# SamsungLabs/fcaf3d

Hardware: AMD Instinct MI355X
Metric: scenes/sec fwd+bwd, ScanNet 100k-pt 2cm voxels, 1/2/4/8 MI355X (higher is better)
Workload: dtype f32

## Files before the change

fcaf3d_amd/_lib.py:

```python
import ctypes
import os
import re
import threading
import time

import torch

_HERE = os.path.dirname(os.path.abspath(__file__))
LIB_PATH = os.environ.get('FC_LIB') or os.path.join(_HERE, 'libfcaf3d_hip.so')
HEADER = os.path.join(os.path.dirname(_HERE), 'include', 'fcaf3d_hip.h')

_SCALARS = {'int': ctypes.c_int, 'int64_t': ctypes.c_int64, 'float': ctypes.c_float,
            'hipStream_t': ctypes.c_void_p}


def parse_header(path=HEADER):
    txt = open(path).read()
    txt = re.sub(r'/\*.*?\*/', '', txt, flags=re.S)
    protos = {}
    for m in re.finditer(r'\b(int64_t|int)\s+(fc_\w+)\s*\(([^)]*)\)\s*;', txt):
        ret, name, args = m.group(1), m.group(2), m.group(3)
        argl = []
        for a in args.split(','):
            a = ' '.join(a.split())
            if not a or a == 'void':
                continue
            if '*' in a:
                argl.append((a.split('*')[-1].strip(), ctypes.c_void_p))
            else:
                ty, nm = a.rsplit(' ', 1)
                argl.append((nm, _SCALARS[ty.replace('const ', '')]))
        protos[name] = (_SCALARS[ret], argl)
    return protos


EXEC_OPS = os.path.join(_HERE, 'csrc', 'exec_ops.h')


def parse_enums(path=EXEC_OPS):
    txt = re.sub(r'//[^\n]*', '', open(path).read())
    known, blocks = {}, []
    for m in re.finditer(r'\benum\s*\{([^}]*)\}', txt):
        block, nxt = {}, 0
        for item in filter(None, (s.strip() for s in m.group(1).split(','))):
            name, _, expr = (s.strip() for s in item.partition('='))
            if expr:
                nxt = sum(known[t] if t in known else int(t, 0) for t in (s.strip() for s in expr.split('+')))
            assert re.fullmatch(r'[A-Z]\w*', name) and name not in known, item
            block[name] = known[name] = nxt
            nxt += 1
        blocks.append(block)
    return blocks


ABI_VERSION = 14
_lib = None
_protos = None


def lib():
    global _lib, _protos
    if _lib is None:
        if not os.path.exists(LIB_PATH):
            raise RuntimeError(
                f'{LIB_PATH} is missing: build it with `python -m fcaf3d_amd.build` '
                '(hipcc --offload-arch=gfx950).  There is no CPU fallback.')
        l = ctypes.CDLL(LIB_PATH)
        _protos = parse_header()
        for name, (ret, args) in _protos.items():
            fn = getattr(l, name)
            fn.restype = ret
            fn.argtypes = [t for _, t in args]
        if l.fc_abi_version() != ABI_VERSION:
            raise RuntimeError(f'{LIB_PATH} speaks ABI version {l.fc_abi_version()}, this host code was written for {ABI_VERSION}: rebuild '
                               'with `python -m fcaf3d_amd.build`')
        _lib = l
    return _lib


def ptr(t):
    if t is None:
        return None
    assert t.is_contiguous(), 'C ABI takes contiguous buffers'
    return t.data_ptr()


_raw_stream = getattr(torch._C, '_cuda_getCurrentRawStream', None)


def stream():
    if _raw_stream is not None:
        return _raw_stream(torch.cuda.current_device())
    return torch.cuda.current_stream().cuda_stream


_fns = {}


def call(name, *args):
    fn = _fns.get(name)
    if fn is None:
        fn = _fns[name] = getattr(lib(), name)
    rc = fn(*args)
    if rc != 0:
        kind = 'invalid argument' if rc == -1 else 'workspace too small' if rc == -2 else f'hipError {rc}'
        raise RuntimeError(f'{name} failed: {kind}')


_header_enums = {}


def header_enums():
    if not _header_enums:
        _header_enums.update({k: v for block in parse_enums(HEADER) for k, v in block.items()})
    return _header_enums


_ROUTE_FIELDS = {'fc_conv_fwd_route': 'FC_ROUTE_', 'fc_conv_wgrad_route': 'FC_WROUTE_', 'fc_bn_train_fwd_route': 'FC_NROUTE_',
                 'fc_bn_train_bwd_route': 'FC_NROUTE_'}


def route(name, *args):
    out = (ctypes.c_int * 16)()
    rc = getattr(lib(), name)(*args, out)
    prefix = _ROUTE_FIELDS[name]
    return rc, {k[len(prefix):].lower(): out[v] for k, v in header_enums().items() if k.startswith(prefix)}


_query_cache = {}


def query(name, *args):
    key = (name,) + args
    v = _query_cache.get(key)
    if v is None:
        if len(_query_cache) > 65536:
            _query_cache.clear()
        v = _query_cache[key] = int(getattr(lib(), name)(*args))
    return v


_ws_cache = {}


def workspace(nbytes, device):
    key = (device, stream())
    buf = _ws_cache.get(key)
    if buf is None or buf.numel() < nbytes:
        buf = torch.empty(max(int(nbytes), 1 << 20), dtype=torch.uint8, device=device)
        _ws_cache[key] = buf
    return buf


HOST_WAIT = [0.0]


class _PinnedRing:

    def __init__(self, n=16):
        self.bufs, self.evts, self.i = [None] * n, [None] * n, 0
        self.lock = threading.Lock()

    def upload(self, arr, device):
        with self.lock:
            i = self.i
            self.i = (i + 1) % len(self.bufs)
        if self.evts[i] is not None and not self.evts[i].query():
            t0 = time.perf_counter()
            self.evts[i].synchronize()
            HOST_WAIT[0] += time.perf_counter() - t0
        nb = max(int(arr.nbytes), 1)
        if self.bufs[i] is None or self.bufs[i].numel() < nb:
            self.bufs[i] = torch.empty(max(nb, 4096), dtype=torch.uint8).pin_memory()
        src = torch.from_numpy(arr)
        stage = self.bufs[i][:arr.nbytes].view(src.dtype).reshape(src.shape)
        stage.copy_(src)
        out = stage.to(device, non_blocking=True)
        e = torch.cuda.Event()
        e.record(torch.cuda.current_stream(out.device))
        self.evts[i] = e
        return out


_ring = _PinnedRing()


def upload(arr, device):
    return _ring.upload(arr, device)
```

fcaf3d_amd/csrc/exec.hip:

```cpp
#include "fc_common.h"
#include "../../include/fcaf3d_hip.h"
#include "exec_ops.h"
#include <vector>

namespace {

constexpr int MAX_EVENTS = 64;

constexpr int MAX_DEVICES = 16;
hipEvent_t g_events_dev[MAX_DEVICES][MAX_EVENTS];
bool g_events_ready[MAX_DEVICES] = {};
thread_local hipEvent_t* g_events = nullptr;

int ensure_events() {
  int dev = 0;
  FC_HIP(hipGetDevice(&dev));
  if (dev < 0 || dev >= MAX_DEVICES) return FC_EINVAL;
  if (!g_events_ready[dev]) {
    for (int i = 0; i < MAX_EVENTS; ++i) FC_HIP(hipEventCreateWithFlags(&g_events_dev[dev][i], hipEventDisableTiming));
    g_events_ready[dev] = true;
  }
  g_events = g_events_dev[dev];
  return 0;
}
// ... 94 lines not shown
  int64_t bn_small_elems;
  int flags;
};

int run_op_impl(Ctx& c, const int64_t* op);

int run_op(Ctx& c, const int64_t* op) {
  if (c.dry || !c.probe || (op[ROW_OP] != OP_CONV && op[ROW_OP] != OP_AMAX)) return run_op_impl(c, op);
  ProbeRec r;
  r.a = probe_event(); r.b = probe_event();
  if (!r.a || !r.b) return run_op_impl(c, op);
  hipStream_t st = c.streams[op[ROW_STREAM]];
  if (op[ROW_OP] == OP_AMAX) {
    const int64_t meta[8] = {-2, 0, c.dims[op[AMAX_N]], 0, 0, op[AMAX_C], 0, 0};
    __builtin_memcpy(r.meta, meta, sizeof meta);
  } else if (op[CONV_MAP] < 0) {
    const int64_t n = c.dims[op[CONV_N]];
    const int64_t meta[8] = {-1, op[CONV_DIR], n, n, 1, op[CONV_CIN], op[CONV_COUT], 0};
    __builtin_memcpy(r.meta, meta, sizeof meta);
  } else {
    const int64_t* mp = c.maps + op[CONV_MAP] * MAPW;
    const bool bwd = op[CONV_DIR] != 0;
    const int64_t meta[8] = {op[CONV_MAP], op[CONV_DIR], bwd ? mp[MAP_N_OUT] : mp[MAP_N_IN], bwd ? mp[MAP_N_IN] : mp[MAP_N_OUT], mp[MAP_K],
                             op[CONV_CIN], op[CONV_COUT], (mp[MAP_FLAGS] & (bwd ? MAP_ROUTE_BWD_PAIRS : MAP_ROUTE_FWD_PAIRS)) ? 1 : 0};
    __builtin_memcpy(r.meta, meta, sizeof meta);
  }
  FC_HIP(hipEventRecord(r.a, st));
  const int rc = run_op_impl(c, op);
  FC_HIP(hipEventRecord(r.b, st));
  g_probe.push_back(r);
  return rc;
}

template <class T>
inline T* P(const Ctx& c, int64_t idx) { return idx < 0 ? nullptr : reinterpret_cast<T*>(c.addr[idx]); }
template <class T>
inline T* P1(const Ctx& c, int64_t idx1) { return P<T>(c, idx1 - 1); }

int64_t stats_blocks_of(const Ctx& c, const int64_t* conv) {
  const int Cin = (int)conv[CONV_CIN], Cout = (int)conv[CONV_COUT];
  const int fl = c.flags | FC_CONV_SPLIT | FC_CONV_IMAGE;
  if (conv[CONV_MAP] < 0) return fc_conv_stats_blocks(c.dims[conv[CONV_N]], 1, Cin, Cout, fl, 0);
  const int64_t* m = c.maps + conv[CONV_MAP] * MAPW;
  const bool bwd = conv[CONV_DIR] != 0;
  return fc_conv_stats_blocks(bwd ? m[MAP_N_IN] : m[MAP_N_OUT], (int)m[MAP_K], Cin, Cout, fl,
                              (m[MAP_FLAGS] & (bwd ? MAP_ROUTE_BWD_PAIRS : MAP_ROUTE_FWD_PAIRS)) ? 1 : 0);
}

inline bool want_ws(Ctx& c, int s, int64_t bytes) {
  if (bytes > c.need[s]) c.need[s] = bytes;
  return !c.dry;
}

int run_op_impl(Ctx& c, const int64_t* op) {
  const int s = (int)op[ROW_STREAM];
  hipStream_t st = c.streams[s];
#ifdef FC_KO_EXEC
  {
    static const int ko = getenv("FC_KO_OPS") ? atoi(getenv("FC_KO_OPS")) : 0;
    const int64_t o = op[ROW_OP];
    if (!c.dry && (((ko & 1) && (o == OP_WGRAD || o == OP_STEM_WGRAD)) || ((ko & 2) && o == OP_CONV) ||
                   ((ko & 4) && (o == OP_BN_FWD || o == OP_BN_BWD || o == OP_COL_STATS || o == OP_NORM_POOL_FWD || o == OP_POOL_NORM_BWD))))
      return 0;
  }
#endif
  switch (op[ROW_OP]) {
    case OP_STEM_FWD: {
      const int64_t* m = c.maps + op[STEM_FWD_MAP] * MAPW;
      if (c.dry) return 0;
      return fc_stem_conv_fwd(P<const float>(c, op[STEM_FWD_X]), P<const float>(c, op[STEM_FWD_W]), reinterpret_cast<const int*>(m[MAP_NBR]),
                              P<float>(c, op[STEM_FWD_OUT]), P<float>(c, op[STEM_FWD_COL]), m[MAP_N_IN], m[MAP_N_OUT], (int)m[MAP_K], st);
    }
    case OP_COL_STATS: {
      const int64_t n = c.dims[op[COL_STATS_N]];
      const int C = (int)op[COL_STATS_C], nseg = (int)c.dims[op[COL_STATS_NSEG]];
      if (!want_ws(c, s, fc_col_stats_ws_bytes(n, C, nseg))) return 0;
      return fc_col_stats(P<const float>(c, op[COL_STATS_X]), P<const int>(c, op[COL_STATS_SEG]), op[COL_STATS_SEG] >= 0 ? 4 : 0, n, C, nseg,
                          P<float>(c, op[COL_STATS_MEAN]), P<float>(c, op[COL_STATS_VAR]), P<float>(c, op[COL_STATS_CNT]), c.ws[s],
                          c.ws_bytes[s], st);
    }
    case OP_CONV: {
      const int Cin = (int)op[CONV_CIN], Cout = (int)op[CONV_COUT];
      const int fl = c.flags | FC_CONV_SPLIT | FC_CONV_IMAGE;
      float* stats = (op[CONV_STATS_P1] > 0 && stats_blocks_of(c, op) > 0) ? P1<float>(c, op[CONV_STATS_P1]) : nullptr;
      const float* bnx = stats ? P1<const float>(c, op[CONV_BN_X_P1]) : nullptr;
      const float *bmean = P<const float>(c, op[CONV_BN_MEAN]), *bvar = P<const float>(c, op[CONV_BN_VAR]),
                  *bga = P<const float>(c, op[CONV_BN_GAMMA]), *bbe = P<const float>(c, op[CONV_BN_BETA]);
      const float beps = (float)as_double(op[CONV_BN_EPS]);
      const int bact = (int)op[CONV_BN_ACT];
      const float* badd = P1<const float>(c, op[CONV_BN_ADD_P1]);
      const float* bny = P1<const float>(c, op[CONV_BN_Y_P1]);
      const float* in = P<const float>(c, op[CONV_X]);
      const float* img = P<const float>(c, op[CONV_IMG]);
      float* out = P<float>(c, op[CONV_OUT]);
      if (!c.dry && op[CONV_AMAX_X_P1] > 0) fc_conv_amax_hint(P1<const unsigned>(c, op[CONV_AMAX_X_P1]), nullptr);
      if (op[CONV_MAP] < 0) {
        const int64_t n = c.dims[op[CONV_N]];
        if (!want_ws(c, s, fc_conv_fwd_ws_bytes(n, 1, Cin, Cout, fl))) return 0;
        if (bnx)
          return fc_conv_fwd_bn_bwd_stats(in, img, nullptr, nullptr, out, n, n, 1, Cin, Cout, fl, c.ws[s], c.ws_bytes[s], stats, bnx, bmean, bvar,
                                          bga, bbe, beps, bact, badd, bny, st);
        return fc_conv_fwd_stats(in, img, nullptr, nullptr, out, n, n, 1, Cin, Cout, fl, c.ws[s], c.ws_bytes[s], stats, st);
      }
      const int64_t* m = c.maps + op[CONV_MAP] * MAPW;
      const bool bwd = op[CONV_DIR] != 0;
      const int64_t n_in = bwd ? m[MAP_N_OUT] : m[MAP_N_IN], n_out = bwd ? m[MAP_N_IN] : m[MAP_N_OUT];
      const int K = (int)m[MAP_K];
      if (m[MAP_FLAGS] & (bwd ? MAP_ROUTE_BWD_PAIRS : MAP_ROUTE_FWD_PAIRS)) {
        const int64_t* pr = m + (bwd ? MAP_PAIRS_T : MAP_PAIRS);
        const int *pi = reinterpret_cast<const int*>(pr[PAIR_IN]), *pc = reinterpret_cast<const int*>(pr[PAIR_CNT]),
                  *pp = reinterpret_cast<const int*>(pr[PAIR_POS]);
        if (!want_ws(c, s, fc_conv_fwd_pairs_ws_bytes(n_out, K, Cout))) return 0;
        if (bnx)
          return fc_conv_fwd_pairs_tiles_bn_bwd_stats(in, img, pi, pc, pp, out, n_in, n_out, K, Cin, Cout, pr[PAIR_TILES], fl, c.ws[s],
                                                      c.ws_bytes[s], stats, bnx, bmean, bvar, bga, bbe, beps, bact, badd, bny, st);
        return fc_conv_fwd_pairs_tiles_stats(in, img, pi, pc, pp, out, n_in, n_out, K, Cin, Cout, pr[PAIR_TILES], fl, c.ws[s], c.ws_bytes[s],
                                             stats, st);
      }
      const int *tab = reinterpret_cast<const int*>(bwd ? m[MAP_BWD_TAB] : m[MAP_FWD_TAB]),
                *oidx = reinterpret_cast<const int*>(bwd ? m[MAP_BWD_IDX] : m[MAP_FWD_IDX]);
      if (!want_ws(c, s, fc_conv_fwd_ws_bytes(n_out, K, Cin, Cout, fl))) return 0;
      if (bnx)
        return fc_conv_fwd_bn_bwd_stats(in, img, tab, oidx, out, n_in, n_out, K, Cin, Cout, fl, c.ws[s], c.ws_bytes[s], stats, bnx, bmean, bvar,
                                        bga, bbe, beps, bact, badd, bny, st);
      return fc_conv_fwd_stats(in, img, tab, oidx, out, n_in, n_out, K, Cin, Cout, fl, c.ws[s], c.ws_bytes[s], stats, st);
    }
    case OP_BN_FWD: {
      const int64_t n = c.dims[op[BN_FWD_N]];
      const int C = (int)op[BN_FWD_C];
      const float eps = (float)as_double(op[BN_FWD_EPS]), mom = (float)as_double(op[BN_FWD_MOMENTUM]);
      const int* add_inv = P1<const int>(c, op[BN_FWD_ADD_INV_P1]);
      const float* add_src = op[BN_FWD_ADD_INV_P1] > 0 ? P1<const float>(c, op[BN_FWD_ADD_SRC_P1]) : nullptr;
      if (!op[BN_FWD_TRAIN]) {
        if (c.dry) return 0;
        if (op[BN_FWD_AMAX_Y_P1] > 0) fc_amax_out_hint(P1<unsigned>(c, op[BN_FWD_AMAX_Y_P1]));
        return fc_norm_act_add_fwd(P<const float>(c, op[BN_FWD_X]), nullptr, 0, n, C, P<const float>(c, op[BN_FWD_RMEAN]),
                                   P<const float>(c, op[BN_FWD_RVAR]), eps, P<const float>(c, op[BN_FWD_GAMMA]),
                                   P<const float>(c, op[BN_FWD_BETA]), P<const float>(c, op[BN_FWD_RES]), (int)op[BN_FWD_ACT], add_inv, add_src,
                                   P<float>(c, op[BN_FWD_Y]), st);
      }
      const float* part = nullptr;
      int64_t nbp = 0;
      if (op[BN_FWD_PRODUCER_P1] > 0) {
        const int64_t* conv = c.ops + (op[BN_FWD_PRODUCER_P1] - 1) * OPW;
        nbp = conv[CONV_STATS_P1] > 0 ? stats_blocks_of(c, conv) : 0;
        if (nbp > 0) part = P1<const float>(c, conv[CONV_STATS_P1]);
      }
      if (!want_ws(c, s, fc_bn_train_ws_bytes(n, C))) return 0;
      if (op[BN_FWD_AMAX_Y_P1] > 0) fc_amax_out_hint(P1<unsigned>(c, op[BN_FWD_AMAX_Y_P1]));
      return fc_bn_train_add_fwd(P<const float>(c, op[BN_FWD_X]), n, C, eps, P<const float>(c, op[BN_FWD_GAMMA]),
                                 P<const float>(c, op[BN_FWD_BETA]), P<const float>(c, op[BN_FWD_RES]), (int)op[BN_FWD_ACT], mom,
                                 P<float>(c, op[BN_FWD_Y]), P<float>(c, op[BN_FWD_MEAN]), P<float>(c, op[BN_FWD_VAR]),
                                 P<float>(c, op[BN_FWD_CNT]), P<float>(c, op[BN_FWD_RMEAN]), P<float>(c, op[BN_FWD_RVAR]),
                                 P<long long>(c, op[BN_FWD_NBT]), part, nbp, op[BN_FWD_GROUPS] > 0 ? (int)op[BN_FWD_GROUPS] : 1,
                                 c.bn_small_elems, add_inv, add_src, c.ws[s], c.ws_bytes[s], st);
    }
    case OP_HEAD_FWD: {
      if (c.dry) return 0;
      return fc_head_split_fwd(P<const float>(c, op[HEAD_FWD_Y]), (int)op[HEAD_FWD_LD], P<const float>(c, op[HEAD_FWD_BIAS]),
                               P<const float>(c, op[HEAD_FWD_SCALE]), c.dims[op[HEAD_FWD_N]], (int)op[HEAD_FWD_N_REG], (int)op[HEAD_FWD_N_CLS],
                               P<float>(c, op[HEAD_FWD_CENT]), P<float>(c, op[HEAD_FWD_BBOX]), P<float>(c, op[HEAD_FWD_CLS]),
                               P<float>(c, op[HEAD_FWD_CMAX]), st);
    }
    case OP_RECORD:
      if (c.dry) return 0;
      FC_HIP(hipEventRecord(g_events[op[RECORD_EVENT]], st));
      return 0;
    case OP_WAIT:
      if (c.dry) return 0;
      FC_HIP(hipStreamWaitEvent(st, g_events[op[WAIT_EVENT]], 0));
      return 0;
    case OP_HEAD_BWD: {
      const float *y = P<const float>(c, op[HEAD_BWD_Y]), *scale = P<const float>(c, op[HEAD_BWD_SCALE]),
                  *bbox = P<const float>(c, op[HEAD_BWD_BBOX]), *g_cent = P<const float>(c, op[HEAD_BWD_G_CENT]),
                  *g_bbox = P<const float>(c, op[HEAD_BWD_G_BBOX]), *g_cls = P<const float>(c, op[HEAD_BWD_G_CLS]);
      const int64_t n = c.dims[op[HEAD_BWD_N]];
      const int ld = (int)op[HEAD_BWD_LD], n_reg = (int)op[HEAD_BWD_N_REG], n_cls = (int)op[HEAD_BWD_N_CLS];
      if (op[HEAD_BWD_GS_ROW] < 0) {
        if (!want_ws(c, s, fc_head_split_bwd_sums_ws_bytes(n))) return 0;
        if (op[HEAD_BWD_AMAX_GY_P1] > 0) fc_amax_out_hint(P1<unsigned>(c, op[HEAD_BWD_AMAX_GY_P1]));
        return fc_head_split_bwd_sums(y, ld, scale, bbox, g_cent, g_bbox, g_cls, n, n_reg, n_cls, P<float>(c, op[HEAD_BWD_GY]),
                                      P<float>(c, op[HEAD_BWD_BIAS_PART]), P<float>(c, op[HEAD_BWD_G_SCALE]), c.ws[s], c.ws_bytes[s], st);
      }
      if (c.dry) return 0;
      return fc_head_split_bwd(y, ld, scale, bbox, g_cent, g_bbox, g_cls, n, n_reg, n_cls, P<float>(c, op[HEAD_BWD_GY]),
                               P<float>(c, op[HEAD_BWD_GS_ROW]), st);
    }
    case OP_WGRAD: {
      const int Cin = (int)op[WGRAD_CIN], Cout = (int)op[WGRAD_COUT];
      const int fl = c.flags | FC_CONV_SPLIT;
      const float *in = P<const float>(c, op[WGRAD_X]), *gout = P<const float>(c, op[WGRAD_GOUT]);
      float* gw = P<float>(c, op[WGRAD_GW]);
      if (!c.dry && (op[WGRAD_AMAX_X_P1] > 0 || op[WGRAD_AMAX_GOUT_P1] > 0))
        fc_conv_amax_hint(P1<const unsigned>(c, op[WGRAD_AMAX_X_P1]), P1<const unsigned>(c, op[WGRAD_AMAX_GOUT_P1]));
      if (op[WGRAD_MAP] < 0) {
        const int64_t n = c.dims[op[WGRAD_N]];
        if (!want_ws(c, s, fc_conv_wgrad_ws_bytes(n, 1, Cin, Cout, fl))) return 0;
        return fc_conv_wgrad(in, gout, nullptr, nullptr, gw, n, n, 1, Cin, Cout, fl, c.ws[s], c.ws_bytes[s], st);
      }
      const int64_t* m = c.maps + op[WGRAD_MAP] * MAPW;
      const int K = (int)m[MAP_K];
      if (!want_ws(c, s, fc_conv_wgrad_ws_bytes(m[MAP_N_OUT], K, Cin, Cout, fl))) return 0;
      if ((m[MAP_FLAGS] & MAP_ROUTE_WGRAD_PAIRS) && Cin % 64 == 0 && Cout % 64 == 0) {
        const int64_t* pr = m + MAP_PAIRS;
        return fc_conv_wgrad_pairs(in, gout, reinterpret_cast<const int*>(pr[PAIR_IN]), reinterpret_cast<const int*>(pr[PAIR_OUT]),
                                   reinterpret_cast<const int*>(pr[PAIR_CNT]), gw, m[MAP_N_IN], m[MAP_N_OUT], K, Cin, Cout, fl, c.ws[s],
                                   c.ws_bytes[s], st);
      }
      return fc_conv_wgrad(in, gout, reinterpret_cast<const int*>(m[MAP_NBR]), nullptr, gw, m[MAP_N_IN], m[MAP_N_OUT], K, Cin, Cout, fl,
                           c.ws[s], c.ws_bytes[s], st);
    }
    case OP_BN_BWD: {
      const int64_t n = c.dims[op[BN_BWD_N]];
      const int C = (int)op[BN_BWD_C];
      const float eps = (float)as_double(op[BN_BWD_EPS]);
      const float* part = nullptr;
      int64_t nbp = 0;
      if (op[BN_BWD_PRODUCER_P1] > 0) {
        const int64_t* conv = c.ops + (op[BN_BWD_PRODUCER_P1] - 1) * OPW;
        nbp = (conv[CONV_STATS_P1] > 0 && conv[CONV_BN_X_P1] > 0) ? stats_blocks_of(c, conv) : 0;
        if (nbp > 0) part = P1<const float>(c, conv[CONV_STATS_P1]);
      }
      if (!want_ws(c, s, fc_bn_train_ws_bytes(n, C))) return 0;
      if (op[BN_BWD_AMAX_GX_P1] > 0) fc_amax_out_hint(P1<unsigned>(c, op[BN_BWD_AMAX_GX_P1]));
      return fc_bn_train_bwd(P<const float>(c, op[BN_BWD_X]), P<const float>(c, op[BN_BWD_Y]), P<const float>(c, op[BN_BWD_GY]),
                             P1<const float>(c, op[BN_BWD_GY2_P1]), n, C, P<const float>(c, op[BN_BWD_MEAN]),
                             P<const float>(c, op[BN_BWD_VAR]), P<const float>(c, op[BN_BWD_CNT]), eps, P<const float>(c, op[BN_BWD_GAMMA]),
                             P<const float>(c, op[BN_BWD_BETA]), (int)op[BN_BWD_ACT], P<float>(c, op[BN_BWD_GX]),
                             P<float>(c, op[BN_BWD_GRES]), P<float>(c, op[BN_BWD_SUMS]), part, nbp, c.bn_small_elems, c.ws[s],
                             c.ws_bytes[s], st);
    }
    case OP_STEM_WGRAD: {
      const int64_t* m = c.maps + op[STEM_WGRAD_MAP] * MAPW;
      if (!want_ws(c, s, fc_stem_conv_wgrad_ws_bytes(m[MAP_N_OUT], (int)m[MAP_K]))) return 0;
      return fc_stem_conv_wgrad(P<const float>(c, op[STEM_WGRAD_COL]), P<const float>(c, op[STEM_WGRAD_GOUT]), P<float>(c, op[STEM_WGRAD_GW]),
                                m[MAP_N_OUT], (int)m[MAP_K], c.ws[s], c.ws_bytes[s], st);
    }
    case OP_GATHER: {
      if (c.dry) return 0;
      return fc_gather_rows(P<const float>(c, op[GATHER_SRC]), P<const int>(c, op[GATHER_IDX]), c.dims[op[GATHER_N]], (int)op[GATHER_C],
                            P<float>(c, op[GATHER_DST]), st);
    }
    case OP_ADD: {
      if (c.dry) return 0;
      const int64_t n4 = c.dims[op[ADD_N]] * op[ADD_C] / 4;
      if (n4 > 0) k_add_inplace<<<(unsigned)fc_cdiv(n4, 256), 256, 0, st>>>(P<float>(c, op[ADD_DST]), P<const float>(c, op[ADD_SRC]), n4);
      FC_CHECK_LAUNCH();
      return 0;
    }
    case OP_SMALL_GRADS: {
      if (c.dry) return 0;
      const int64_t cnt = op[SMALL_GRADS_COUNT];
      if (cnt > 0) k_small_grads<<<(unsigned)cnt, 128, 0, st>>>(P<const long long>(c, op[SMALL_GRADS_DESC]) + 8 * op[SMALL_GRADS_FIRST], (int)cnt);
      FC_CHECK_LAUNCH();
      return 0;
    }
    case OP_COL_SUM: {
      if (c.dry) return 0;
      k_col_sum<<<(unsigned)op[COL_SUM_C], 1024, 0, st>>>(P<const float>(c, op[COL_SUM_X]), c.dims[op[COL_SUM_N]], (int)op[COL_SUM_C],
                                                         P<float>(c, op[COL_SUM_DST]));
      FC_CHECK_LAUNCH();
      return 0;
    }
    case OP_ROW_SUM: {
      if (c.dry) return 0;
      k_col_sum<<<1, 1024, 0, st>>>(P<const float>(c, op[ROW_SUM_X]), c.dims[op[ROW_SUM_N]], 1, P<float>(c, op[ROW_SUM_DST]));
      FC_CHECK_LAUNCH();
      return 0;
    }
    case OP_PERMUTE_GENT: {
      if (c.dry) return 0;
      const int Cin = (int)op[PERMUTE_GENT_CIN], Cout = (int)op[PERMUTE_GENT_COUT];
      const int64_t total = (int64_t)8 * Cin * Cout;
      k_permute_gent<<<(unsigned)fc_cdiv(total, 256), 256, 0, st>>>(P<const float>(c, op[PERMUTE_GENT_SRC]), P<float>(c, op[PERMUTE_GENT_DST]),
                                                                    Cin, Cout);
      FC_CHECK_LAUNCH();
      return 0;
    }
    case OP_HEAD_WFIN: {
      if (c.dry) return 0;
      const int R = (int)op[HEAD_WFIN_R], n_reg = (int)op[HEAD_WFIN_N_REG], n_cls = (int)op[HEAD_WFIN_N_CLS];
      const int total = R * (1 + n_reg + n_cls);
      k_head_wfin<<<(unsigned)fc_cdiv(total, 256), 256, 0, st>>>(P<const float>(c, op[HEAD_WFIN_PART]), (int)op[HEAD_WFIN_NL], R,
                                                                 (int)op[HEAD_WFIN_LD], n_reg, n_cls, P<float>(c, op[HEAD_WFIN_G_CENT]),
                                                                 P<float>(c, op[HEAD_WFIN_G_REG]), P<float>(c, op[HEAD_WFIN_G_CLS]),
                                                                 P<const float>(c, op[HEAD_WFIN_BIAS_PART]), P<float>(c, op[HEAD_WFIN_G_BIAS]));
      FC_CHECK_LAUNCH();
      return 0;
    }
    case OP_AMAX: {
      if (c.dry) return 0;
      return fc_amax(P<const float>(c, op[AMAX_X]), c.dims[op[AMAX_N]] * op[AMAX_C], P<unsigned>(c, op[AMAX_SLOT]), st);
    }
    case OP_CLEAR: {
      if (c.dry) return 0;
      FC_HIP(hipMemsetAsync(P<void>(c, op[CLEAR_DST]), 0, (size_t)op[CLEAR_BYTES], st));
      return 0;
    }
    case OP_NORM_POOL_FWD: {
      const int64_t* m = c.maps + op[NORM_POOL_FWD_MAP] * MAPW;
      if (c.dry) return 0;
      if ((int)m[MAP_K] != 8) return FC_EINVAL;
      if (op[NORM_POOL_FWD_AMAX_OUT_P1] > 0) fc_amax_out_hint(P1<unsigned>(c, op[NORM_POOL_FWD_AMAX_OUT_P1]));
      return fc_norm_act_maxpool8_fwd(P<const float>(c, op[NORM_POOL_FWD_X]), P<const int>(c, op[NORM_POOL_FWD_SEG]),
                                      op[NORM_POOL_FWD_SEG] >= 0 ? 4 : 0, (int)op[NORM_POOL_FWD_C], P<const float>(c, op[NORM_POOL_FWD_MEAN]),
                                      P<const float>(c, op[NORM_POOL_FWD_VAR]), (float)as_double(op[NORM_POOL_FWD_EPS]),
                                      P<const float>(c, op[NORM_POOL_FWD_GAMMA]), P<const float>(c, op[NORM_POOL_FWD_BETA]),
                                      (int)op[NORM_POOL_FWD_ACT], reinterpret_cast<const int*>(m[MAP_NBR]), m[MAP_N_OUT],
                                      P<float>(c, op[NORM_POOL_FWD_OUT]), P<int>(c, op[NORM_POOL_FWD_ARG]), P<float>(c, op[NORM_POOL_FWD_Y]),
                                      P<int>(c, op[NORM_POOL_FWD_PARENT]), st);
    }
    case OP_POOL_NORM_BWD: {
      const int64_t n = c.dims[op[POOL_NORM_BWD_N]];
      const int C = (int)op[POOL_NORM_BWD_C], nseg = (int)c.dims[op[POOL_NORM_BWD_NSEG]];
      if (!want_ws(c, s, fc_maxpool8_norm_act_bwd_ws_bytes(n, C, nseg))) return 0;
      return fc_maxpool8_norm_act_bwd(P<const float>(c, op[POOL_NORM_BWD_X]), P<const float>(c, op[POOL_NORM_BWD_G_POOL]),
                                      P<const int>(c, op[POOL_NORM_BWD_ARG]), P<const int>(c, op[POOL_NORM_BWD_PARENT]),
                                      P<const int>(c, op[POOL_NORM_BWD_SEG]), op[POOL_NORM_BWD_SEG] >= 0 ? 4 : 0, n, C, nseg,
                                      P<const float>(c, op[POOL_NORM_BWD_MEAN]), P<const float>(c, op[POOL_NORM_BWD_VAR]),
                                      P<const float>(c, op[POOL_NORM_BWD_CNT]), (float)as_double(op[POOL_NORM_BWD_EPS]),
                                      P<const float>(c, op[POOL_NORM_BWD_GAMMA]), P<const float>(c, op[POOL_NORM_BWD_BETA]),
                                      (int)op[POOL_NORM_BWD_ACT], P<float>(c, op[POOL_NORM_BWD_GX]), P<float>(c, op[POOL_NORM_BWD_SUMS]),
                                      c.ws[s], c.ws_bytes[s], st);
    }
    case OP_INV_ROWS: {
      if (c.dry) return 0;
      return fc_inverse_rows(P<const int>(c, op[INV_ROWS_ROWS]), c.dims[op[INV_ROWS_N]], c.dims[op[INV_ROWS_N_INV]], P<int>(c, op[INV_ROWS_INV]), st);
    }
    case OP_COPY: {
      if (c.dry) return 0;
      FC_HIP(hipMemcpyAsync(P<float>(c, op[COPY_DST]), P<const float>(c, op[COPY_SRC]), sizeof(float) * c.dims[op[COPY_N]] * op[COPY_C],
                            hipMemcpyDeviceToDevice, st));
      return 0;
    }
    default:
      return FC_EINVAL;
  }
}

}

extern "C" {

int fc_exec_op_words(void) { return OPW; }
int fc_exec_map_words(void) { return MAPW; }

int fc_exec(const int64_t* ops, int64_t op_begin, int64_t op_end, const int64_t* addr, const int64_t* dims, const int64_t* maps,
            const int64_t* streams, const int64_t* ws, const int64_t* ws_bytes, int64_t* ws_need, const int64_t* cfg) {
  if (!ops || op_begin < 0 || op_end < op_begin) return FC_EINVAL;
  int rc = ensure_events();
  if (rc) return rc;
  Ctx c;
  c.ops = ops;
  c.addr = addr; c.dims = dims; c.maps = maps;
  for (int i = 0; i < NSTREAM; ++i) {
    c.streams[i] = reinterpret_cast<hipStream_t>(streams[i]);
    c.ws[i] = reinterpret_cast<void*>(ws[i]);
    c.ws_bytes[i] = ws_bytes[i];
    c.need[i] = 0;
  }
  c.bn_small_elems = cfg[0];
  c.flags = (int)cfg[1];
  c.probe = cfg[2] != 0;
  c.dry = true;
  for (int64_t i = op_begin; i < op_end; ++i) {
    rc = run_op(c, ops + i * OPW);
    if (rc) return rc;
  }
  bool ok = true;
  for (int i = 0; i < NSTREAM; ++i) {
    if (ws_need) ws_need[i] = c.need[i];
    if (c.need[i] > c.ws_bytes[i]) ok = false;
  }
  if (!ok) return FC_EWS;
  if (cfg[3]) return 0;
  c.dry = false;
  for (int64_t i = op_begin; i < op_end; ++i) {
    rc = run_op(c, ops + i * OPW);
    if (rc) return rc;
  }
  return 0;
}

int64_t fc_exec_probe_read(float* ms, int64_t* meta, int64_t cap) {
  const int64_t n = (int64_t)g_probe.size();
  for (int64_t i = 0; i < n; ++i) {
    ProbeRec& r = g_probe[i];
    if (i < cap) {
      float t = 0.f;
      if (hipEventElapsedTime(&t, r.a, r.b) != hipSuccess) t = -1.f;
      ms[i] = t;
      __builtin_memcpy(meta + 8 * i, r.meta, sizeof r.meta);
    }
    g_probe_pool.push_back(r.a);
    g_probe_pool.push_back(r.b);
  }
  g_probe.clear();
  return n;
}

}
```

fcaf3d_amd/csrc/exec_ops.h:

```cpp
#ifndef FCAF3D_EXEC_OPS_H
#define FCAF3D_EXEC_OPS_H

enum {
  OPW = 24,
  MAPW = 20,
  NSTREAM = 3
};
enum { ROW_OP, ROW_STREAM };

enum {
  OP_STEM_FWD = 1, OP_COL_STATS, OP_NORM_FWD, OP_MAXPOOL_FWD, OP_CONV, OP_BN_FWD, OP_UNION_FWD, OP_HEAD_FWD, OP_RECORD, OP_WAIT,
  OP_HEAD_BWD, OP_WGRAD, OP_BN_BWD, OP_NORM_BWD, OP_MAXPOOL_BWD, OP_STEM_WGRAD, OP_GATHER, OP_ADD, OP_SMALL_GRADS,
  OP_PERMUTE_GENT, OP_HEAD_WFIN, OP_COPY, OP_COL_SUM, OP_ROW_SUM, OP_AMAX, OP_CLEAR, OP_NORM_POOL_FWD, OP_POOL_NORM_BWD, OP_INV_ROWS
};

enum {
  STEM_FWD_X = 2,
  STEM_FWD_W,
  STEM_FWD_MAP,
  STEM_FWD_OUT,
  STEM_FWD_COL,
  STEM_FWD_END
};
enum {
  COL_STATS_X = 2,
  COL_STATS_SEG,
  COL_STATS_N,
  COL_STATS_C,
  COL_STATS_NSEG,
  COL_STATS_MEAN,
  COL_STATS_VAR,
  COL_STATS_CNT,
  COL_STATS_END
};
enum {
  CONV_X = 2,
  CONV_IMG,
  CONV_MAP,
  CONV_DIR,
  CONV_OUT,
  CONV_N,
  CONV_CIN,
  CONV_COUT,
  CONV_STATS_P1,
  CONV_BN_X_P1,
  CONV_BN_MEAN,
  CONV_BN_VAR,
  CONV_BN_GAMMA,
  CONV_BN_BETA,
  CONV_BN_EPS,
  CONV_BN_ACT,
  CONV_BN_ADD_P1,
  CONV_BN_Y_P1,
  CONV_AMAX_X_P1,
  CONV_END
};
enum {
  BN_FWD_X = 2,
  BN_FWD_N,
  BN_FWD_C,
  BN_FWD_EPS,
  BN_FWD_GAMMA,
  BN_FWD_BETA,
  BN_FWD_RES,
  BN_FWD_ACT,
  BN_FWD_MOMENTUM,
  BN_FWD_Y,
  BN_FWD_MEAN,
  BN_FWD_VAR,
  BN_FWD_CNT,
  BN_FWD_RMEAN,
  BN_FWD_RVAR,
  BN_FWD_NBT,
  BN_FWD_TRAIN,
  BN_FWD_PRODUCER_P1,
  BN_FWD_GROUPS,
  BN_FWD_AMAX_Y_P1,
  BN_FWD_ADD_INV_P1,
  BN_FWD_ADD_SRC_P1,
  BN_FWD_END
};
enum {
  HEAD_FWD_Y = 2,
  HEAD_FWD_LD,
  HEAD_FWD_BIAS,
  HEAD_FWD_SCALE,
  HEAD_FWD_N,
  HEAD_FWD_N_REG,
  HEAD_FWD_N_CLS,
  HEAD_FWD_CENT,
  HEAD_FWD_BBOX,
  HEAD_FWD_CLS,
  HEAD_FWD_CMAX,
  HEAD_FWD_END
};
enum { RECORD_EVENT = 2, RECORD_END };
enum { WAIT_EVENT = 2, WAIT_END };
enum {
  HEAD_BWD_Y = 2,
  HEAD_BWD_LD,
  HEAD_BWD_SCALE,
  HEAD_BWD_BBOX,
  HEAD_BWD_G_CENT,
  HEAD_BWD_G_BBOX,
  HEAD_BWD_G_CLS,
  HEAD_BWD_N,
  HEAD_BWD_N_REG,
  HEAD_BWD_N_CLS,
  HEAD_BWD_GY,
  HEAD_BWD_GS_ROW,
  HEAD_BWD_G_SCALE,
  HEAD_BWD_BIAS_PART,
  HEAD_BWD_AMAX_GY_P1,
  HEAD_BWD_END
};
enum {
  WGRAD_X = 2,
  WGRAD_GOUT,
  WGRAD_MAP,
  WGRAD_GW,
  WGRAD_N,
  WGRAD_CIN,
  WGRAD_COUT,
  WGRAD_AMAX_X_P1,
  WGRAD_AMAX_GOUT_P1,
  WGRAD_END
};
enum {
  BN_BWD_X = 2,
  BN_BWD_Y,
  BN_BWD_GY,
  BN_BWD_N,
  BN_BWD_C,
  BN_BWD_MEAN,
  BN_BWD_VAR,
  BN_BWD_CNT,
  BN_BWD_EPS,
  BN_BWD_GAMMA,
  BN_BWD_BETA,
  BN_BWD_ACT,
  BN_BWD_GX,
  BN_BWD_GRES,
  BN_BWD_SUMS,
  BN_BWD_GY2_P1,
  BN_BWD_PRODUCER_P1,
  BN_BWD_AMAX_GX_P1,
  BN_BWD_END
};
enum {
  STEM_WGRAD_COL = 2,
  STEM_WGRAD_GOUT,
  STEM_WGRAD_MAP,
  STEM_WGRAD_GW,
  STEM_WGRAD_END
};
enum {
  GATHER_SRC = 2,
  GATHER_IDX,
  GATHER_N,
  GATHER_C,
  GATHER_DST,
  GATHER_END
};
enum {
  ADD_DST = 2,
  ADD_SRC,
  ADD_N,
  ADD_C,
  ADD_END
};
enum {
  SMALL_GRADS_DESC = 2,
  SMALL_GRADS_FIRST,
  SMALL_GRADS_COUNT,
  SMALL_GRADS_END
};
enum {
  PERMUTE_GENT_SRC = 2,
  PERMUTE_GENT_DST,
  PERMUTE_GENT_CIN,
  PERMUTE_GENT_COUT,
  PERMUTE_GENT_END
};
enum {
  HEAD_WFIN_PART = 2,
  HEAD_WFIN_NL,
  HEAD_WFIN_R,
  HEAD_WFIN_LD,
  HEAD_WFIN_N_REG,
  HEAD_WFIN_N_CLS,
  HEAD_WFIN_G_CENT,
  HEAD_WFIN_G_REG,
  HEAD_WFIN_G_CLS,
  HEAD_WFIN_BIAS_PART,
  HEAD_WFIN_G_BIAS,
  HEAD_WFIN_END
};
enum {
  COPY_DST = 2,
  COPY_SRC,
  COPY_N,
  COPY_C,
  COPY_END
};
enum {
  COL_SUM_X = 2,
  COL_SUM_N,
  COL_SUM_C,
  COL_SUM_DST,
  COL_SUM_END
};
enum {
  ROW_SUM_X = 2,
  ROW_SUM_N,
  ROW_SUM_DST,
  ROW_SUM_END
};
enum {
  AMAX_X = 2,
  AMAX_N,
  AMAX_C,
  AMAX_SLOT,
  AMAX_END
};
enum {
  CLEAR_DST = 2,
  CLEAR_BYTES,
  CLEAR_END
};
enum {
  NORM_POOL_FWD_X = 2,
  NORM_POOL_FWD_SEG,
  NORM_POOL_FWD_C,
  NORM_POOL_FWD_MEAN,
  NORM_POOL_FWD_VAR,
  NORM_POOL_FWD_EPS,
  NORM_POOL_FWD_GAMMA,
  NORM_POOL_FWD_BETA,
  NORM_POOL_FWD_ACT,
  NORM_POOL_FWD_MAP,
  NORM_POOL_FWD_OUT,
  NORM_POOL_FWD_ARG,
  NORM_POOL_FWD_Y,
  NORM_POOL_FWD_AMAX_OUT_P1,
  NORM_POOL_FWD_PARENT,
  NORM_POOL_FWD_END
};
enum {
  POOL_NORM_BWD_X = 2,
  POOL_NORM_BWD_G_POOL,
  POOL_NORM_BWD_ARG,
  POOL_NORM_BWD_PARENT,
  POOL_NORM_BWD_SEG,
  POOL_NORM_BWD_N,
  POOL_NORM_BWD_C,
  POOL_NORM_BWD_NSEG,
  POOL_NORM_BWD_MEAN,
  POOL_NORM_BWD_VAR,
  POOL_NORM_BWD_CNT,
  POOL_NORM_BWD_EPS,
  POOL_NORM_BWD_GAMMA,
  POOL_NORM_BWD_BETA,
  POOL_NORM_BWD_ACT,
  POOL_NORM_BWD_GX,
  POOL_NORM_BWD_SUMS,
  POOL_NORM_BWD_END
};
enum {
  INV_ROWS_ROWS = 2,
  INV_ROWS_N,
  INV_ROWS_N_INV,
  INV_ROWS_INV,
  INV_ROWS_END
};

static_assert(STEM_FWD_END <= OPW && COL_STATS_END <= OPW && CONV_END <= OPW && BN_FWD_END <= OPW && HEAD_FWD_END <= OPW, "operator row");
static_assert(RECORD_END <= OPW && WAIT_END <= OPW && HEAD_BWD_END <= OPW && WGRAD_END <= OPW && BN_BWD_END <= OPW, "operator row");
static_assert(STEM_WGRAD_END <= OPW && GATHER_END <= OPW && ADD_END <= OPW && SMALL_GRADS_END <= OPW && PERMUTE_GENT_END <= OPW, "operator row");
static_assert(HEAD_WFIN_END <= OPW && COPY_END <= OPW && COL_SUM_END <= OPW && ROW_SUM_END <= OPW && AMAX_END <= OPW, "operator row");
static_assert(CLEAR_END <= OPW && NORM_POOL_FWD_END <= OPW && POOL_NORM_BWD_END <= OPW && INV_ROWS_END <= OPW, "operator row");

enum {
  PAIR_IN,
  PAIR_OUT,
  PAIR_POS,
  PAIR_CNT,
  PAIR_TILES,
  PAIR_END
};
enum {
  MAP_N_IN,
  MAP_N_OUT,
  MAP_K,
  MAP_NBR,
  MAP_NBR_T,
  MAP_FWD_TAB,
  MAP_FWD_IDX,
  MAP_BWD_TAB,
  MAP_BWD_IDX,
  MAP_PAIRS,
  MAP_PAIRS_T = MAP_PAIRS + PAIR_END,
  MAP_FLAGS = MAP_PAIRS_T + PAIR_END,
  MAP_END
};
enum {
  MAP_ROUTE_FWD_PAIRS = 1,
  MAP_ROUTE_BWD_PAIRS = 2,
  MAP_ROUTE_WGRAD_PAIRS = 4
};
static_assert(MAP_END <= MAPW, "kernel-map descriptor");

#endif
```

fcaf3d_amd/csrc/norm.hip:

```cpp
#include "fc_common.h"
#include "../../include/fcaf3d_hip.h"
#include "norm_route.h"
#include "norm_elem.h"
#include "norm_stats.h"
#include "norm_rows.h"
#include "norm_bn.h"
#include "pool_rows.h"

thread_local unsigned* t_fc_amax_out = nullptr;

#define FC_GRID(l, stream) dim3((l).grid_x, (l).grid_y), (l).threads, (l).lds, stream

static int bn_fwd(const float* x, int64_t n, int C, float eps, const float* gamma, const float* beta, const float* residual, int act, float momentum,
                  float* y, float* mean, float* var, float* cnt, float* rmean, float* rvar, long long* nbt, const float* table, int64_t nb_part, int groups,
                  int64_t small_elems, const int* add_inv, const float* add_src, void* ws, int64_t ws_bytes, hipStream_t stream, unsigned* amax,
                  bool apply = true) {
  if (act < 0 || act > 2 || (add_inv == nullptr) != (add_src == nullptr)) return FC_EINVAL;
  const NormRoute r = norm_fwd_route(n, C, table != nullptr, nb_part, groups, small_elems);
  if (int rc = route_check(r, ws_bytes)) return rc;
  float* part = (float*)ws;
  if (r.red.threads) { k_bn1_partial<<<FC_GRID(r.red, stream)>>>(x, n, C, r.red_rpb, part); FC_CHECK_LAUNCH(); }
  if (r.fin.threads) {
    if (r.sums == FC_NSTATS_PARTIAL) k_bn_finalize<<<FC_GRID(r.fin, stream)>>>(part, (int)r.np, C, n, x, momentum, mean, var, cnt, rmean, rvar, nbt);
    else k_bn2_finalize<<<FC_GRID(r.fin, stream)>>>(table, (int)r.np, C, groups, n, momentum, mean, var, cnt, rmean, rvar, nbt);
    FC_CHECK_LAUNCH();
  }
  if (!apply) return FC_OK;
  if (r.apply == FC_NAPPLY_BN1)
    k_bn1_apply<<<FC_GRID(r.ap, stream)>>>(x, n, C, r.rpb, part, (int)r.np, eps, gamma, beta, residual, act, momentum, y, mean, var, cnt, rmean, rvar, nbt, add_inv, add_src);
  else if (r.apply == FC_NAPPLY_BN2)
    k_bn2_apply<<<FC_GRID(r.ap, stream)>>>(x, n, C, r.rpb, table, (int)r.np, groups, eps, gamma, beta, residual, act, momentum, y, mean, var, cnt, rmean, rvar, nbt, r.cg,
                                   add_inv, add_src, amax);
  else
    k_norm_act_fwd<<<FC_GRID(r.ap, stream)>>>(x, nullptr, 0, n, C, mean, var, eps, gamma, beta, residual, act, add_inv, add_src, y, amax);
  FC_CHECK_LAUNCH();
  if (r.amax == FC_NAMAX_PASS && amax) return fc_amax(y, n * (int64_t)C, amax, stream);
  return FC_OK;
}

template <bool POOL>
static int norm_bwd(int form, const float* x, const float* y, const float* gy, const float* gy2, const int* parent, const int* argrow, const int* seg,
                    int seg_stride, int64_t n, int C, int nseg, const float* mean, const float* var, const float* cnt, float eps, const float* gamma,
                    const float* beta, int act, float* gx, float* gres, float* sums, const float* table, int64_t nb_part, int64_t small_elems, void* ws,
                    int64_t ws_bytes, hipStream_t stream, unsigned* amax, bool late_hint = false) {
  if (act < 0 || act > 2) return FC_EINVAL;
  const NormRoute r = norm_bwd_route(n, C, nseg, table != nullptr, nb_part, small_elems, form);
  if (int rc = route_check(r, ws_bytes)) return rc;
  if (late_hint) amax = take_amax_out();
  if (r.apply == FC_NBAPPLY_NONE) {
    FC_HIP(hipMemsetAsync(sums, 0, sizeof(float) * nseg * 2 * C, stream));
    return FC_OK;
  }
  if (r.sums == FC_NRED_PARTIAL) {
    k_norm_bwd_partial<POOL><<<FC_GRID(r.red, stream)>>>(x, y, gy, gy2, parent, argrow, seg, seg_stride, n, C, nseg, mean, var, eps, act, gamma, beta, r.red_rpb, (float*)ws);
    FC_CHECK_LAUNCH();
    table = (const float*)ws;
  }
  if (r.apply == FC_NBAPPLY_PROLOGUE) {
    k_bn1_bwd_apply<<<FC_GRID(r.ap, stream)>>>(x, y, gy, gy2, n, C, r.rpb, table, (int)r.np, mean, var, eps, gamma, beta, act, gx, gres, sums, r.cg, amax);
  } else {
    k_stats_final<<<FC_GRID(r.fin, stream)>>>(table, nullptr, r.np, nseg, 2 * C, 2, sums, nullptr);
    FC_CHECK_LAUNCH();
    k_norm_bwd_apply<POOL><<<FC_GRID(r.ap, stream)>>>(x, y, gy, gy2, parent, argrow, seg, seg_stride, n, C, mean, var, eps, gamma, beta, sums, cnt, act, gx, gres, amax);
  }
  FC_CHECK_LAUNCH();
  return FC_OK;
}

constexpr int ROUTE_OUT_INTS = 16;
static_assert(FC_NROUTE_LAUNCHES < ROUTE_OUT_INTS, "every FC_NROUTE_* field lies inside out[]");
static int route_out(const NormRoute& r, int* out) {
  const int f[ROUTE_OUT_INTS] = {r.sums, r.apply, r.amax, (int)r.np, (int)r.nb, (int)r.rpb, r.cg, r.ap.threads, (int)r.ap.lds, (int)r.ap.grid_x, (int)r.ap.grid_y,
                                 (int)r.ws_bytes, (r.red.threads != 0) + (r.fin.threads != 0) + (r.ap.threads != 0)};
  for (int i = 0; i < ROUTE_OUT_INTS; ++i) out[i] = f[i];
  return r.sums ? FC_OK : FC_EINVAL;
}

static int col_stats(bool stats, const float* x, const int* seg, int seg_stride, int64_t n, int C, int nseg, float* out, float* var, float* cnt, void* ws,
                     int64_t ws_bytes, hipStream_t stream) {
  if (n < 0 || nseg < 1 || nseg > MAXSEG) return FC_EINVAL;
  StatsGeometry g;
  if (!stats_geometry(C, &g)) return FC_EINVAL;
  if (ws_bytes < fc_col_stats_ws_bytes(n, C, nseg)) return FC_EWS;
  if (n == 0) {
    FC_HIP(hipMemsetAsync(out, 0, sizeof(float) * nseg * C, stream));
    if (stats) FC_HIP(hipMemsetAsync(var, 0, sizeof(float) * nseg * C, stream));
    if (stats) FC_HIP(hipMemsetAsync(cnt, 0, sizeof(float) * nseg, stream));
    return FC_OK;
  }
  const RowBlocks b = row_blocks(n, MAXBLOCKS);
  float* part = (float*)ws;
  float* part_cnt = stats ? part + b.nb * nseg * 2 * C : nullptr;
  k_stats_partial<<<(unsigned)b.nb, g.threads, g.lds_fwd, stream>>>(x, seg, seg_stride, n, C, nseg, nullptr, stats ? 2 : 0, b.rpb, part, part_cnt);
  FC_CHECK_LAUNCH();
  if (stats) k_seg_meanvar_final<<<FC_GRID(final_launch(nseg, C), stream)>>>(part, part_cnt, b.nb, nseg, C, out, var, cnt);
  else k_stats_final<<<FC_GRID(final_launch(nseg, C), stream)>>>(part, nullptr, b.nb, nseg, C, 2, out, nullptr);
  FC_CHECK_LAUNCH();
  return FC_OK;
}

extern "C" {

int64_t fc_col_stats_ws_bytes(int64_t n, int C, int nseg) {
  return row_blocks(n, MAXBLOCKS).nb * nseg * (2 * (int64_t)C + 1) * (int64_t)sizeof(float);
}

int fc_col_stats(const float* x, const int* seg, int seg_stride, int64_t n, int C, int nseg, float* mean, float* var,
                 float* cnt, void* ws, int64_t ws_bytes, hipStream_t stream) {
  return col_stats(true, x, seg, seg_stride, n, C, nseg, mean, var, cnt, ws, ws_bytes, stream);
}

int fc_seg_col_sums(const float* x, const int* seg, int seg_stride, int64_t n, int C, int nseg, float* out, void* ws,
                    int64_t ws_bytes, hipStream_t stream) {
  return col_stats(false, x, seg, seg_stride, n, C, nseg, out, nullptr, nullptr, ws, ws_bytes, stream);
}

int fc_bn_running_update(const float* mean, const float* var, const float* cnt, float momentum, int C, float* running_mean,
                         float* running_var, long long* num_batches_tracked, hipStream_t stream) {
  if (C < 1) return FC_EINVAL;
  k_bn_running<<<(unsigned)fc_cdiv(C, 256), 256, 0, stream>>>(mean, var, cnt, momentum, C, running_mean, running_var,
                                                             num_batches_tracked);
  FC_CHECK_LAUNCH();
  return FC_OK;
}

int fc_bn_train_fwd_route(int64_t n, int C, int has_part, int64_t nb_part, int groups, int64_t small_elems, int* out) {
  return out ? route_out(norm_fwd_route(n, C, has_part != 0, nb_part, groups, small_elems), out) : FC_EINVAL;
}
int fc_bn_train_bwd_route(int64_t n, int C, int nseg, int has_part, int64_t nb_part, int64_t small_elems, int form, int* out) {
  if (!out || form < FC_NFORM_TRAIN || form > FC_NFORM_SEG) return FC_EINVAL;
  return route_out(norm_bwd_route(n, C, nseg, has_part != 0, nb_part, small_elems, form), out);
}

int64_t fc_bn_small_ws_bytes(int C) { return small_ws_bytes(C); }
int64_t fc_bn_stats_ws_bytes(int64_t n, int C) { return reduce_ws_bytes(n, C, 1); }
int64_t fc_norm_act_bwd_ws_bytes(int64_t n, int C, int nseg) { return reduce_ws_bytes(n, C, nseg); }
int64_t fc_maxpool8_norm_act_bwd_ws_bytes(int64_t n_in, int C, int nseg) { return reduce_ws_bytes(n_in, C, nseg); }
int64_t fc_bn_train_ws_bytes(int64_t n, int C) { return reduce_ws_bytes(n, C, 1) > small_ws_bytes(C) ? reduce_ws_bytes(n, C, 1) : small_ws_bytes(C); }

int fc_bn_stats_train(const float* x, int64_t n, int C, float momentum, float* mean, float* var, float* cnt,
                      float* running_mean, float* running_var, long long* num_batches_tracked, void* ws,
                      int64_t ws_bytes, hipStream_t stream) {
  return bn_fwd(x, n, C, 0.f, nullptr, nullptr, nullptr, 0, momentum, nullptr, mean, var, cnt, running_mean, running_var, num_batches_tracked, nullptr, 0, 1,
                -1, nullptr, nullptr, ws, ws_bytes, stream, nullptr, false);
}

int fc_bn_act_train_fwd(const float* x, int64_t n, int C, float eps, const float* gamma, const float* beta,
                        const float* residual, int act, float momentum, float* y, float* mean, float* var, float* cnt,
                        float* running_mean, float* running_var, long long* num_batches_tracked, void* ws,
                        int64_t ws_bytes, hipStream_t stream) {
  return bn_fwd(x, n, C, eps, gamma, beta, residual, act, momentum, y, mean, var, cnt, running_mean, running_var, num_batches_tracked, nullptr, 0, 1,
                INT64_MAX, nullptr, nullptr, ws, ws_bytes, stream, nullptr);
}

int fc_bn_act_train_bwd(const float* x, const float* y, const float* gy, int64_t n, int C, const float* mean,
                        const float* var, float eps, const float* gamma, const float* beta, int act, float* gx, float* gres,
                        float* sums, void* ws, int64_t ws_bytes, hipStream_t stream) {
  return norm_bwd<false>(FC_NFORM_SMALL, x, y, gy, nullptr, nullptr, nullptr, nullptr, 0, n, C, 1, mean, var, nullptr, eps, gamma, beta, act, gx, gres, sums,
                         nullptr, 0, 0, ws, ws_bytes, stream, nullptr, true);
}

int fc_norm_act_add_fwd(const float* x, const int* seg, int seg_stride, int64_t n, int C, const float* mean, const float* var,
                        float eps, const float* gamma, const float* beta, const float* residual, int act, const int* add_inv,
                        const float* add_src, float* y, hipStream_t stream) {
  unsigned* ao = take_amax_out();
  if (n < 0 || C < 4 || C % 4 || act < 0 || act > 2 || (add_inv == nullptr) != (add_src == nullptr)) return FC_EINVAL;
  if (n == 0) return FC_OK;
  k_norm_act_fwd<<<FC_GRID(rows_launch(n, C), stream)>>>(x, seg, seg_stride, n, C, mean, var, eps, gamma, beta, residual, act, add_inv, add_src, y, ao);
  FC_CHECK_LAUNCH();
  return FC_OK;
}

int fc_norm_act_fwd(const float* x, const int* seg, int seg_stride, int64_t n, int C, const float* mean, const float* var,
                    float eps, const float* gamma, const float* beta, const float* residual, int act, float* y,
                    hipStream_t stream) {
  return fc_norm_act_add_fwd(x, seg, seg_stride, n, C, mean, var, eps, gamma, beta, residual, act, nullptr, nullptr, y, stream);
}

int fc_norm_act_bwd(const float* x, const float* y, const float* gy, const int* seg, int seg_stride, int64_t n, int C,
                    int nseg, const float* mean, const float* var, const float* cnt, float eps, const float* gamma,
                    const float* beta, int act, float* gx, float* gres, float* sums, void* ws, int64_t ws_bytes,
                    hipStream_t stream) {
  unsigned* ao = take_amax_out();
  return norm_bwd<false>(FC_NFORM_SEG, x, y, gy, nullptr, nullptr, nullptr, seg, seg_stride, n, C, nseg, mean, var, cnt, eps, gamma, beta, act, gx, gres, sums,
                         nullptr, 0, 0, ws, ws_bytes, stream, ao);
}

int fc_bn_train_add_fwd(const float* x, int64_t n, int C, float eps, const float* gamma, const float* beta, const float* residual,
                        int act, float momentum, float* y, float* mean, float* var, float* cnt, float* running_mean,
                        float* running_var, long long* num_batches_tracked, const float* part, int64_t nb_part, int groups,
                        int64_t small_elems, const int* add_inv, const float* add_src, void* ws, int64_t ws_bytes,
                        hipStream_t stream) {
  unsigned* ao = take_amax_out();
  return bn_fwd(x, n, C, eps, gamma, beta, residual, act, momentum, y, mean, var, cnt, running_mean, running_var, num_batches_tracked, part, nb_part, groups,
                small_elems, add_inv, add_src, ws, ws_bytes, stream, ao);
}

int fc_bn_train_fwd(const float* x, int64_t n, int C, float eps, const float* gamma, const float* beta, const float* residual,
                    int act, float momentum, float* y, float* mean, float* var, float* cnt, float* running_mean,
                    float* running_var, long long* num_batches_tracked, const float* part, int64_t nb_part, int groups,
                    int64_t small_elems, void* ws, int64_t ws_bytes, hipStream_t stream) {
  return fc_bn_train_add_fwd(x, n, C, eps, gamma, beta, residual, act, momentum, y, mean, var, cnt, running_mean, running_var, num_batches_tracked, part, nb_part,
                             groups, small_elems, nullptr, nullptr, ws, ws_bytes, stream);
}

int fc_bn_train_bwd(const float* x, const float* y, const float* gy, const float* gy2, int64_t n, int C, const float* mean,
                    const float* var, const float* cnt, float eps, const float* gamma, const float* beta, int act, float* gx,
                    float* gres, float* sums, const float* part, int64_t nb_part, int64_t small_elems, void* ws, int64_t ws_bytes,
                    hipStream_t stream) {
  unsigned* ao = take_amax_out();
  return norm_bwd<false>(FC_NFORM_TRAIN, x, y, gy, gy2, nullptr, nullptr, nullptr, 0, n, C, 1, mean, var, cnt, eps, gamma, beta, act, gx, gres, sums, part, nb_part,
                         small_elems, ws, ws_bytes, stream, ao);
}

int fc_amax_out_hint(unsigned* amax_word) {
  t_fc_amax_out = amax_word;
  return FC_OK;
}

int fc_maxpool_fwd(const float* in, const int* nbr, int64_t n_out, int K, int C, float* out, int* argrow,
                   hipStream_t stream) {
  unsigned* ao = take_amax_out();
  if (n_out < 0 || K < 1 || C < 1) return FC_EINVAL;
  if (n_out == 0) return FC_OK;
  if (K == 8 && C % 4 == 0) k_maxpool8_fwd<<<FC_GRID(rows_launch(n_out, C), stream)>>>(in, nbr, n_out, C, out, argrow, ao);
  else k_maxpool_fwd<<<(unsigned)fc_cdiv(n_out * C, 256), 256, 0, stream>>>(in, nbr, n_out, K, C, out, argrow);
  FC_CHECK_LAUNCH();
  if (ao && !(K == 8 && C % 4 == 0)) return fc_amax(out, n_out * (int64_t)C, ao, stream);
  return FC_OK;
}

int fc_maxpool_bwd(const float* gout, const int* argrow, int64_t n_out, int C, float* gin, hipStream_t stream) {
  if (n_out < 0 || C < 1) return FC_EINVAL;
  if (n_out == 0) return FC_OK;
  k_maxpool_bwd<<<(unsigned)fc_cdiv(n_out * C, 256), 256, 0, stream>>>(gout, argrow, n_out, C, gin);
  FC_CHECK_LAUNCH();
  return FC_OK;
}

int fc_gather_rows(const float* src, const int* idx, int64_t n, int C, float* dst, hipStream_t stream) {
  if (n < 0 || C < 1) return FC_EINVAL;
  if (n == 0) return FC_OK;
  k_gather_rows<<<(unsigned)fc_cdiv(n * C, 256), 256, 0, stream>>>(src, idx, n, C, dst);
  FC_CHECK_LAUNCH();
  return FC_OK;
}

int fc_scatter_rows_add(const float* src, const int* idx, int64_t n, int C, float* dst, hipStream_t stream) {
  if (n < 0 || C < 1) return FC_EINVAL;
  if (n == 0) return FC_OK;
  k_scatter_rows_add<<<(unsigned)fc_cdiv(n * C, 256), 256, 0, stream>>>(src, idx, n, C, dst);
  FC_CHECK_LAUNCH();
  return FC_OK;
}

int fc_norm_act_maxpool8_fwd(const float* x, const int* seg, int seg_stride, int C, const float* mean, const float* var, float eps,
                             const float* gamma, const float* beta, int act, const int* nbr, int64_t n_out, float* out,
                             int* argrow, float* y, int* parent, hipStream_t stream) {
  unsigned* ao = take_amax_out();
  if (n_out < 0 || C < 4 || C % 4 || act < 0 || act > 2) return FC_EINVAL;
  if (n_out == 0) return FC_OK;
  k_norm_act_maxpool8_fwd<<<FC_GRID(rows_launch(n_out, C), stream)>>>(x, seg, seg_stride, C, mean, var, eps, gamma, beta, act, nbr, n_out, out, argrow, y,
                                                                     parent, ao);
  FC_CHECK_LAUNCH();
  return FC_OK;
}

int fc_maxpool8_norm_act_bwd(const float* x, const float* gout, const int* argrow, const int* parent, const int* seg, int seg_stride,
                             int64_t n_in, int C, int nseg, const float* mean, const float* var, const float* cnt, float eps,
                             const float* gamma, const float* beta, int act, float* gx, float* sums, void* ws, int64_t ws_bytes,
                             hipStream_t stream) {
  if (!parent || !argrow) return FC_EINVAL;
  return norm_bwd<true>(FC_NFORM_SEG, x, nullptr, gout, nullptr, parent, argrow, seg, seg_stride, n_in, C, nseg, mean, var, cnt, eps, gamma, beta, act, gx, nullptr,
                        sums, nullptr, 0, 0, ws, ws_bytes, stream, nullptr);
}

int fc_inverse_rows(const int* rows, int64_t n, int64_t n_inv, int* inv, hipStream_t stream) {
  if (n < 0 || n_inv < 0) return FC_EINVAL;
  if (n_inv > 0) FC_HIP(hipMemsetAsync(inv, 0xff, sizeof(int) * n_inv, stream));
  if (n == 0) return FC_OK;
  k_inverse_rows<<<(unsigned)fc_cdiv(n, 256), 256, 0, stream>>>(rows, n, n_inv, inv);
  FC_CHECK_LAUNCH();
  return FC_OK;
}

}
```

fcaf3d_amd/csrc/norm_bn.h:

```cpp
#pragma once


__global__ void k_bn1_partial(const float* __restrict__ x, int64_t n, int C, int64_t rpb, float* __restrict__ part) {
  extern __shared__ float sm[];
  const auto [cl, rl, nrl] = lane_coord(C / 4);
  const auto [r0, r1] = row_span(rpb, n);
  const float4 sh = *reinterpret_cast<const float4*>(x + cl * 4);
  float4 a1 = make_float4(0.f, 0.f, 0.f, 0.f), a2 = a1;
  for (int64_t rb = r0 + rl; rb < r1; rb += 4 * (int64_t)nrl) {
    float4 v[4];
#pragma unroll
    for (int u = 0; u < 4; ++u) {
      const int64_t r = rb + (int64_t)u * nrl;
      v[u] = r < r1 ? *reinterpret_cast<const float4*>(x + r * C + cl * 4) : sh;
    }
#pragma unroll
    for (int u = 0; u < 4; ++u) {
      v[u].x -= sh.x; v[u].y -= sh.y; v[u].z -= sh.z; v[u].w -= sh.w;
      a1.x += v[u].x; a1.y += v[u].y; a1.z += v[u].z; a1.w += v[u].w;
      a2.x += v[u].x * v[u].x; a2.y += v[u].y * v[u].y; a2.z += v[u].z * v[u].z; a2.w += v[u].w * v[u].w;
    }
  }
  *reinterpret_cast<float4*>(&sm[(rl * 2 + 0) * C + cl * 4]) = a1;
  *reinterpret_cast<float4*>(&sm[(rl * 2 + 1) * C + cl * 4]) = a2;
  __syncthreads();
  if (rl == 0) {
    float4 t1 = make_float4(0.f, 0.f, 0.f, 0.f), t2 = t1;
    for (int j = 0; j < nrl; ++j) {
      float4 u = *reinterpret_cast<const float4*>(&sm[(j * 2 + 0) * C + cl * 4]);
      float4 w = *reinterpret_cast<const float4*>(&sm[(j * 2 + 1) * C + cl * 4]);
      t1.x += u.x; t1.y += u.y; t1.z += u.z; t1.w += u.w;
      t2.x += w.x; t2.y += w.y; t2.z += w.z; t2.w += w.w;
    }
    float* dst = part + ((int64_t)blockIdx.x * 2) * C;
    *reinterpret_cast<float4*>(dst + cl * 4) = t1;
    *reinterpret_cast<float4*>(dst + C + cl * 4) = t2;
  }
}

__device__ static inline void bn1_reduce_parts(const float* __restrict__ part, int nb, int C, int cl, int rl, int nrl,
                                               float* sm , float4* s1, float4* s2, int CG, int c0) {
  float4 a1 = make_float4(0.f, 0.f, 0.f, 0.f), a2 = a1;
  const bool past_l1 = (int64_t)nb * C * 8 <= 32768;
  for (int b = rl; b < nb; b += nrl) {
    const float* src = part + ((int64_t)b * 2) * C + c0;
    float4 u = past_l1 ? fc_ld4(src + cl * 4) : *reinterpret_cast<const float4*>(src + cl * 4);
    float4 w = past_l1 ? fc_ld4(src + C + cl * 4) : *reinterpret_cast<const float4*>(src + C + cl * 4);
    a1.x += u.x; a1.y += u.y; a1.z += u.z; a1.w += u.w;
    a2.x += w.x; a2.y += w.y; a2.z += w.z; a2.w += w.w;
  }
  *reinterpret_cast<float4*>(&sm[(rl * 2 + 0) * CG + cl * 4]) = a1;
  *reinterpret_cast<float4*>(&sm[(rl * 2 + 1) * CG + cl * 4]) = a2;
  __syncthreads();
  float4 t1 = make_float4(0.f, 0.f, 0.f, 0.f), t2 = t1;
  for (int j = 0; j < nrl; ++j) {
    float4 u = *reinterpret_cast<const float4*>(&sm[(j * 2 + 0) * CG + cl * 4]);
    float4 w = *reinterpret_cast<const float4*>(&sm[(j * 2 + 1) * CG + cl * 4]);
    t1.x += u.x; t1.y += u.y; t1.z += u.z; t1.w += u.w;
    t2.x += w.x; t2.y += w.y; t2.z += w.z; t2.w += w.w;
  }
  *s1 = t1; *s2 = t2;
}

__global__ void k_bn1_apply(const float* __restrict__ x, int64_t n, int C, int64_t rpb, const float* __restrict__ part, int nb,
                            float eps, const float* __restrict__ gamma, const float* __restrict__ beta,
                            const float* __restrict__ residual, int act, float momentum, float* __restrict__ y,
                            float* __restrict__ mean_out, float* __restrict__ var_out, float* __restrict__ cnt_out,
                            float* __restrict__ rmean, float* __restrict__ rvar, long long* __restrict__ nbt,
                            const int* __restrict__ add_inv, const float* __restrict__ add_src) {
  extern __shared__ float sm[];
  const int c4n = C / 4;
  const int cl = threadIdx.x % c4n, rl = threadIdx.x / c4n;
  const int nrl = blockDim.x / c4n;
  float4 s1, s2;
  bn1_reduce_parts(part, nb, C, cl, rl, nrl, sm, &s1, &s2, C, 0);
  const float4 sh = *reinterpret_cast<const float4*>(x + cl * 4);
  const float inv_n = 1.f / (float)n;
  float d[4] = {s1.x * inv_n, s1.y * inv_n, s1.z * inv_n, s1.w * inv_n};
  float q[4] = {s2.x * inv_n, s2.y * inv_n, s2.z * inv_n, s2.w * inv_n};
  float shv[4] = {sh.x, sh.y, sh.z, sh.w};
  float mu[4], va[4], is[4], g[4], bt[4];
#pragma unroll
  for (int j = 0; j < 4; ++j) {
    mu[j] = shv[j] + d[j];
    va[j] = fmaxf(q[j] - d[j] * d[j], 0.f);
    is[j] = 1.f / sqrtf(va[j] + eps);
    g[j] = gamma ? gamma[cl * 4 + j] : 1.f;
    bt[j] = beta ? beta[cl * 4 + j] : 0.f;
  }
  if (blockIdx.x == 0 && rl == 0) {
    *reinterpret_cast<float4*>(mean_out + cl * 4) = make_float4(mu[0], mu[1], mu[2], mu[3]);
    *reinterpret_cast<float4*>(var_out + cl * 4) = make_float4(va[0], va[1], va[2], va[3]);
    if (cl == 0) { cnt_out[0] = (float)n; if (nbt) nbt[0] += 1; }
    if (rmean) {
#pragma unroll
      for (int j = 0; j < 4; ++j) bn_running_update(rmean, rvar, cl * 4 + j, mu[j], va[j], (float)n, momentum);
    }
  }
  const auto [r0, r1] = row_span(rpb, n);
  for (int64_t rb = r0 + rl; rb < r1; rb += 4 * (int64_t)nrl) {
    float v[4][4], rs[4][4];
#pragma unroll
    for (int u = 0; u < 4; ++u) {
      const int64_t r = rb + (int64_t)u * nrl;
      const int64_t rc = r < r1 ? r : r0;
      *reinterpret_cast<float4*>(v[u]) = *reinterpret_cast<const float4*>(x + rc * C + cl * 4);
      if (residual) *reinterpret_cast<float4*>(rs[u]) = *reinterpret_cast<const float4*>(residual + rc * C + cl * 4);
    }
#pragma unroll
    for (int u = 0; u < 4; ++u) {
      const int64_t r = rb + (int64_t)u * nrl;
      if (r >= r1) continue;
      float o[4];
#pragma unroll
      for (int j = 0; j < 4; ++j) o[j] = norm_act_elem(v[u][j], mu[j], is[j], g[j], bt[j], residual ? &rs[u][j] : nullptr, act);
      const int q = add_inv ? add_inv[r] : -1;
      if (q >= 0) {
        const float4 f = *reinterpret_cast<const float4*>(add_src + (int64_t)q * C + cl * 4);
        o[0] += f.x; o[1] += f.y; o[2] += f.z; o[3] += f.w;
      }
      *reinterpret_cast<float4*>(y + r * C + cl * 4) = *reinterpret_cast<float4*>(o);
    }
  }
}

__global__ __launch_bounds__(1024) void k_bn_finalize(const float* __restrict__ part, int nb, int C, int64_t n,
                                                      const float* __restrict__ x, float momentum, float* __restrict__ mean,
                                                      float* __restrict__ var, float* __restrict__ cnt,
                                                      float* __restrict__ rmean, float* __restrict__ rvar,
                                                      long long* __restrict__ nbt) {
  __shared__ float r1[16][65], r2[16][65];
  const int c = blockIdx.x * 64 + (threadIdx.x & 63), j = threadIdx.x >> 6;
  float a1 = 0.f, a2 = 0.f;
  if (c < C) {
    float p1[4] = {0.f, 0.f, 0.f, 0.f}, p2[4] = {0.f, 0.f, 0.f, 0.f};
    int b = j;
    for (; b + 48 < nb; b += 64) {
      float u[4], w[4];
#pragma unroll
      for (int q = 0; q < 4; ++q) {
        u[q] = fc_ld(&part[((int64_t)(b + 16 * q) * 2) * C + c]);
        w[q] = fc_ld(&part[((int64_t)(b + 16 * q) * 2 + 1) * C + c]);
      }
#pragma unroll
      for (int q = 0; q < 4; ++q) { p1[q] += u[q]; p2[q] += w[q]; }
    }
    for (; b < nb; b += 16) {
      p1[0] += fc_ld(&part[((int64_t)b * 2) * C + c]);
      p2[0] += fc_ld(&part[((int64_t)b * 2 + 1) * C + c]);
    }
    a1 = (p1[0] + p1[1]) + (p1[2] + p1[3]);
    a2 = (p2[0] + p2[1]) + (p2[2] + p2[3]);
  }
  r1[j][threadIdx.x & 63] = a1;
  r2[j][threadIdx.x & 63] = a2;
  __syncthreads();
  if (j == 0 && c < C) {
    float s1 = 0.f, s2 = 0.f;
    for (int q = 0; q < 16; ++q) { s1 += r1[q][threadIdx.x & 63]; s2 += r2[q][threadIdx.x & 63]; }
    const float inv_n = 1.f / (float)n;
    float d = s1 * inv_n;
    float mu = x[c] + d;
    float va = fmaxf(s2 * inv_n - d * d, 0.f);
    mean[c] = mu;
    var[c] = va;
    if (c == 0) { cnt[0] = (float)n; if (nbt) nbt[0] += 1; }
    if (rmean) bn_running_update(rmean, rvar, c, mu, va, (float)n, momentum);
  }
}

__global__ void k_bn1_bwd_apply(const float* __restrict__ x, const float* __restrict__ y, const float* __restrict__ gy,
                                const float* __restrict__ gy2, int64_t n, int C, int64_t rpb, const float* __restrict__ part, int nb,
                                const float* __restrict__ mean, const float* __restrict__ var, float eps,
                                const float* __restrict__ gamma, const float* __restrict__ beta, int act,
                                float* __restrict__ gx, float* __restrict__ gres, float* __restrict__ sums , int CG,
                                unsigned* __restrict__ amax_out) {
  extern __shared__ float sm[];
  const int c0 = blockIdx.y * CG;
  x += c0; gy += c0; gx += c0; mean += c0; var += c0;
  if (y) y += c0;
  if (gy2) gy2 += c0;
  if (gres) gres += c0;
  if (gamma) gamma += c0;
  if (beta) beta += c0;
  const int c4n = CG / 4;
  const int cl = threadIdx.x % c4n, rl = threadIdx.x / c4n;
  const int nrl = blockDim.x / c4n;
  float4 t1, t2;
  bn1_reduce_parts(part, nb, C, cl, rl, nrl, sm, &t1, &t2, CG, c0);
  if (blockIdx.x == 0 && rl == 0) {
    *reinterpret_cast<float4*>(sums + c0 + cl * 4) = t1;
    *reinterpret_cast<float4*>(sums + C + c0 + cl * 4) = t2;
  }
  const float inv_n = 1.f / (float)n;
  float s1[4] = {t1.x * inv_n, t1.y * inv_n, t1.z * inv_n, t1.w * inv_n};
  float s2[4] = {t2.x * inv_n, t2.y * inv_n, t2.z * inv_n, t2.w * inv_n};
  float mu[4], is[4], g[4], bt[4];
#pragma unroll
  for (int j = 0; j < 4; ++j) {
    mu[j] = mean[cl * 4 + j];
    is[j] = 1.f / sqrtf(var[cl * 4 + j] + eps);
    g[j] = gamma ? gamma[cl * 4 + j] : 1.f;
    bt[j] = beta ? beta[cl * 4 + j] : 0.f;
  }
  const bool from_y = act && y;
  const auto [r0, r1] = row_span(rpb, n);
  unsigned am = 0u;
  for (int64_t rb = r0 + rl; rb < r1; rb += 4 * (int64_t)nrl) {
    float xv[4][4], gv[4][4], yv[4][4];
#pragma unroll
    for (int u = 0; u < 4; ++u) {
      const int64_t r = rb + (int64_t)u * nrl;
      const int64_t rc = r < r1 ? r : r0;
      *reinterpret_cast<float4*>(xv[u]) = *reinterpret_cast<const float4*>(x + rc * C + cl * 4);
      *reinterpret_cast<float4*>(gv[u]) = *reinterpret_cast<const float4*>(gy + rc * C + cl * 4);
      if (gy2) {
        const float4 t2 = *reinterpret_cast<const float4*>(gy2 + rc * C + cl * 4);
        gv[u][0] += t2.x; gv[u][1] += t2.y; gv[u][2] += t2.z; gv[u][3] += t2.w;
      }
      if (from_y) *reinterpret_cast<float4*>(yv[u]) = *reinterpret_cast<const float4*>(y + rc * C + cl * 4);
    }
#pragma unroll
    for (int u = 0; u < 4; ++u) {
      const int64_t r = rb + (int64_t)u * nrl;
      if (r >= r1) continue;
      float o[4], gr[4];
#pragma unroll
      for (int j = 0; j < 4; ++j) {
        float gg = gv[u][j];
        if (from_y) gg *= act_bwd_from_y(yv[u][j], act);
        else if (act) gg *= act_bwd_from_pre(bn_pre(xv[u][j], mu[j], is[j], g[j], bt[j]), act);
        float xh = (xv[u][j] - mu[j]) * is[j];
        gr[j] = gg;
        o[j] = g[j] * is[j] * (gg - s1[j] - xh * s2[j]);
      }
      *reinterpret_cast<float4*>(gx + r * C + cl * 4) = *reinterpret_cast<float4*>(o);
      if (gres) *reinterpret_cast<float4*>(gres + r * C + cl * 4) = *reinterpret_cast<float4*>(gr);
#pragma unroll
      for (int j = 0; j < 4; ++j) amax_fold(am, o[j]);
    }
  }
  if (amax_out) amax_commit(am, amax_out);
}

__global__ void k_bn2_apply(const float* __restrict__ x, int64_t n, int C, int64_t rpb, const float* __restrict__ part, int nb, int G,
                            float eps, const float* __restrict__ gamma, const float* __restrict__ beta,
                            const float* __restrict__ residual, int act, float momentum, float* __restrict__ y,
                            float* __restrict__ mean_out, float* __restrict__ var_out, float* __restrict__ cnt_out,
                            float* __restrict__ rmean, float* __restrict__ rvar, long long* __restrict__ nbt, int CG,
                            const int* __restrict__ add_inv, const float* __restrict__ add_src, unsigned* __restrict__ amax_out) {
  extern __shared__ double smd[];
  const int c0 = blockIdx.y * CG;
  x += c0; y += c0; part += c0; mean_out += c0; var_out += c0;
  if (add_src) add_src += c0;
  if (residual) residual += c0;
  if (gamma) gamma += c0;
  if (beta) beta += c0;
  if (rmean) { rmean += c0; rvar += c0; }
  const auto [cl, rl, nrl] = lane_coord(CG / 4);
  double a1[4] = {0., 0., 0., 0.}, a2[4] = {0., 0., 0., 0.};
  const int GC = G * C;
  for (int t = rl; t < nb * G; t += nrl) {
    const int b = t / G, g = t % G;
    const float* src = part + ((int64_t)b * 2) * GC + g * C + cl * 4;
    const float4 u = fc_ld4(src), w = fc_ld4(src + GC);
    a1[0] += u.x; a1[1] += u.y; a1[2] += u.z; a1[3] += u.w;
    a2[0] += w.x; a2[1] += w.y; a2[2] += w.z; a2[3] += w.w;
  }
#pragma unroll
  for (int j = 0; j < 4; ++j) {
    smd[(rl * 2 + 0) * CG + cl * 4 + j] = a1[j];
    smd[(rl * 2 + 1) * CG + cl * 4 + j] = a2[j];
  }
  __syncthreads();
  float mu[4], va[4], is[4], g[4], bt[4];
#pragma unroll
  for (int j = 0; j < 4; ++j) {
    double t1 = 0., t2 = 0.;
    for (int q = 0; q < nrl; ++q) { t1 += smd[(q * 2 + 0) * CG + cl * 4 + j]; t2 += smd[(q * 2 + 1) * CG + cl * 4 + j]; }
    bn2_stats(t1, t2, n, &mu[j], &va[j]);
    is[j] = 1.f / sqrtf(va[j] + eps);
    g[j] = gamma ? gamma[cl * 4 + j] : 1.f;
    bt[j] = beta ? beta[cl * 4 + j] : 0.f;
  }
  if (blockIdx.x == 0 && rl == 0) {
    *reinterpret_cast<float4*>(mean_out + cl * 4) = make_float4(mu[0], mu[1], mu[2], mu[3]);
    *reinterpret_cast<float4*>(var_out + cl * 4) = make_float4(va[0], va[1], va[2], va[3]);
    if (cl == 0 && blockIdx.y == 0) { cnt_out[0] = (float)n; if (nbt) nbt[0] += 1; }
    if (rmean) {
#pragma unroll
      for (int j = 0; j < 4; ++j) bn_running_update(rmean, rvar, cl * 4 + j, mu[j], va[j], (float)n, momentum);
    }
  }
  const auto [r0, r1] = row_span(rpb, n);
  unsigned am = 0u;
  for (int64_t rb = r0 + rl; rb < r1; rb += 4 * (int64_t)nrl) {
    float v[4][4], rs[4][4];
    int q[4];
#pragma unroll
    for (int u = 0; u < 4; ++u) {
      const int64_t r = rb + (int64_t)u * nrl;
      const int64_t rc = r < r1 ? r : r0;
      *reinterpret_cast<float4*>(v[u]) = *reinterpret_cast<const float4*>(x + rc * C + cl * 4);
      if (residual) *reinterpret_cast<float4*>(rs[u]) = *reinterpret_cast<const float4*>(residual + rc * C + cl * 4);
      q[u] = add_inv ? add_inv[rc] : -1;
    }
#pragma unroll
    for (int u = 0; u < 4; ++u) {
      const int64_t r = rb + (int64_t)u * nrl;
      if (r >= r1) continue;
      float o[4];
#pragma unroll
      for (int j = 0; j < 4; ++j) o[j] = norm_act_elem(v[u][j], mu[j], is[j], g[j], bt[j], residual ? &rs[u][j] : nullptr, act);
      if (q[u] >= 0) {
        const float4 f = *reinterpret_cast<const float4*>(add_src + (int64_t)q[u] * C + cl * 4);
        o[0] += f.x; o[1] += f.y; o[2] += f.z; o[3] += f.w;
      }
// ... 67 lines not shown
```

fcaf3d_amd/csrc/norm_rows.h:

```cpp
#pragma once

__global__ void k_norm_act_fwd(const float* __restrict__ x, const int* __restrict__ seg, int seg_stride, int64_t n, int C,
                               const float* __restrict__ mean, const float* __restrict__ var, float eps,
                               const float* __restrict__ gamma, const float* __restrict__ beta,
                               const float* __restrict__ residual, int act, const int* __restrict__ add_inv,
                               const float* __restrict__ add_src, float* __restrict__ y, unsigned* __restrict__ amax_out) {
  int64_t t = (int64_t)blockIdx.x * blockDim.x + threadIdx.x;
  const int c4n = C / 4;
  unsigned am = 0u;
  if (t < n * c4n) {
  int64_t r = t / c4n;
  int c = (int)(t % c4n) * 4;
  int s = seg_of(seg, seg_stride, r);
  const int q = add_inv ? add_inv[r] : -1;
  float4 v = *reinterpret_cast<const float4*>(x + r * C + c);
  float4 mu = *reinterpret_cast<const float4*>(mean + (int64_t)s * C + c);
  float4 va = *reinterpret_cast<const float4*>(var + (int64_t)s * C + c);
  float4 g = gamma ? *reinterpret_cast<const float4*>(gamma + c) : make_float4(1.f, 1.f, 1.f, 1.f);
  float4 b = beta ? *reinterpret_cast<const float4*>(beta + c) : make_float4(0.f, 0.f, 0.f, 0.f);
  float4 o;
  o.x = bn_pre(v.x, mu.x, 1.f / sqrtf(va.x + eps), g.x, b.x);
  o.y = bn_pre(v.y, mu.y, 1.f / sqrtf(va.y + eps), g.y, b.y);
  o.z = bn_pre(v.z, mu.z, 1.f / sqrtf(va.z + eps), g.z, b.z);
  o.w = bn_pre(v.w, mu.w, 1.f / sqrtf(va.w + eps), g.w, b.w);
  if (residual) {
    float4 rs = *reinterpret_cast<const float4*>(residual + r * C + c);
    o.x += rs.x; o.y += rs.y; o.z += rs.z; o.w += rs.w;
  }
  o.x = act_fwd(o.x, act); o.y = act_fwd(o.y, act); o.z = act_fwd(o.z, act); o.w = act_fwd(o.w, act);
  if (q >= 0) {
    const float4 f = *reinterpret_cast<const float4*>(add_src + (int64_t)q * C + c);
    o.x += f.x; o.y += f.y; o.z += f.z; o.w += f.w;
  }
  *reinterpret_cast<float4*>(y + r * C + c) = o;
  amax_fold(am, o.x); amax_fold(am, o.y); amax_fold(am, o.z); amax_fold(am, o.w);
  }
  if (amax_out) amax_commit(am, amax_out);
}

template <bool POOL>
__global__ void k_norm_bwd_partial(const float* __restrict__ x, const float* __restrict__ y, const float* __restrict__ gy,
                                   const float* __restrict__ gy2, const int* __restrict__ pool_parent,
                                   const int* __restrict__ pool_arg, const int* __restrict__ seg, int seg_stride, int64_t n, int C, int nseg,
                                   const float* __restrict__ mean, const float* __restrict__ var, float eps, int act,
                                   const float* __restrict__ gamma, const float* __restrict__ beta,
                                   int64_t rpb, float* __restrict__ part) {
  extern __shared__ float sm[];
  __shared__ int srange[2];
  const auto [cl, rl, nrl] = lane_coord(C / 4);
  const int64_t r0 = (int64_t)blockIdx.x * rpb;
  int64_t r1 = r0 + rpb;
  if (r1 > n) r1 = n;
  int s_lo, s_hi;
  seg_range(seg, seg_stride, r0, r1, &s_lo, &s_hi, srange);
  const bool chk = seg && s_lo != s_hi;
  for (int s = 0; s < nseg; ++s) {
    float4 a1[4], a2[4];
#pragma unroll
    for (int u = 0; u < 4; ++u) { a1[u] = make_float4(0.f, 0.f, 0.f, 0.f); a2[u] = a1[u]; }
    if (s >= s_lo && s <= s_hi) {
      float4 mu = *reinterpret_cast<const float4*>(mean + (int64_t)s * C + cl * 4);
      float4 va = *reinterpret_cast<const float4*>(var + (int64_t)s * C + cl * 4);
      float4 is = make_float4(1.f / sqrtf(va.x + eps), 1.f / sqrtf(va.y + eps), 1.f / sqrtf(va.z + eps),
                              1.f / sqrtf(va.w + eps));
      const float4 gm = gamma ? *reinterpret_cast<const float4*>(gamma + cl * 4) : make_float4(1.f, 1.f, 1.f, 1.f);
      const float4 bt = beta ? *reinterpret_cast<const float4*>(beta + cl * 4) : make_float4(0.f, 0.f, 0.f, 0.f);
      const bool from_y = act && y;
      for (int64_t rb = r0 + rl; rb < r1; rb += 4 * nrl) {
        float4 xv[4], gv[4], yv[4], g2[4];
        bool ok[4];
#pragma unroll
        for (int u = 0; u < 4; ++u) {
          const int64_t r = rb + (int64_t)u * nrl;
          ok[u] = r < r1;
          const int64_t rc = ok[u] ? r : r0;
          if (chk) ok[u] = ok[u] && seg[rc * seg_stride] == s;
          xv[u] = *reinterpret_cast<const float4*>(x + rc * C + cl * 4);
          if (POOL) {
            const int64_t o = pool_parent[rc];
            const int4 a = *reinterpret_cast<const int4*>(pool_arg + o * C + cl * 4);
            gv[u] = *reinterpret_cast<const float4*>(gy + o * C + cl * 4);
            gv[u].x = a.x == rc ? gv[u].x : 0.f; gv[u].y = a.y == rc ? gv[u].y : 0.f;
            gv[u].z = a.z == rc ? gv[u].z : 0.f; gv[u].w = a.w == rc ? gv[u].w : 0.f;
          } else {
            gv[u] = *reinterpret_cast<const float4*>(gy + rc * C + cl * 4);
          }
          if (gy2) g2[u] = *reinterpret_cast<const float4*>(gy2 + rc * C + cl * 4);
          if (from_y) yv[u] = *reinterpret_cast<const float4*>(y + rc * C + cl * 4);
        }
#pragma unroll
        for (int u = 0; u < 4; ++u) {
          if (!ok[u]) continue;
          float4 g = gv[u];
          if (gy2) { g.x += g2[u].x; g.y += g2[u].y; g.z += g2[u].z; g.w += g2[u].w; }
          if (from_y) {
            g.x *= act_bwd_from_y(yv[u].x, act); g.y *= act_bwd_from_y(yv[u].y, act);
            g.z *= act_bwd_from_y(yv[u].z, act); g.w *= act_bwd_from_y(yv[u].w, act);
          } else if (act) {
            g.x *= act_bwd_from_pre(bn_pre(xv[u].x, mu.x, is.x, gm.x, bt.x), act);
            g.y *= act_bwd_from_pre(bn_pre(xv[u].y, mu.y, is.y, gm.y, bt.y), act);
            g.z *= act_bwd_from_pre(bn_pre(xv[u].z, mu.z, is.z, gm.z, bt.z), act);
            g.w *= act_bwd_from_pre(bn_pre(xv[u].w, mu.w, is.w, gm.w, bt.w), act);
          }
          a1[u].x += g.x; a1[u].y += g.y; a1[u].z += g.z; a1[u].w += g.w;
          a2[u].x += g.x * (xv[u].x - mu.x) * is.x; a2[u].y += g.y * (xv[u].y - mu.y) * is.y;
          a2[u].z += g.z * (xv[u].z - mu.z) * is.z; a2[u].w += g.w * (xv[u].w - mu.w) * is.w;
        }
      }
    }
    float4 b1 = make_float4((a1[0].x + a1[1].x) + (a1[2].x + a1[3].x), (a1[0].y + a1[1].y) + (a1[2].y + a1[3].y),
                            (a1[0].z + a1[1].z) + (a1[2].z + a1[3].z), (a1[0].w + a1[1].w) + (a1[2].w + a1[3].w));
    float4 b2 = make_float4((a2[0].x + a2[1].x) + (a2[2].x + a2[3].x), (a2[0].y + a2[1].y) + (a2[2].y + a2[3].y),
                            (a2[0].z + a2[1].z) + (a2[2].z + a2[3].z), (a2[0].w + a2[1].w) + (a2[2].w + a2[3].w));
    __syncthreads();
    *reinterpret_cast<float4*>(&sm[(rl * 2 + 0) * C + cl * 4]) = b1;
    *reinterpret_cast<float4*>(&sm[(rl * 2 + 1) * C + cl * 4]) = b2;
    __syncthreads();
    if (rl == 0) {
      float4 t1 = make_float4(0.f, 0.f, 0.f, 0.f), t2 = t1;
      for (int j = 0; j < nrl; ++j) {
        float4 u = *reinterpret_cast<const float4*>(&sm[(j * 2 + 0) * C + cl * 4]);
        float4 w = *reinterpret_cast<const float4*>(&sm[(j * 2 + 1) * C + cl * 4]);
        t1.x += u.x; t1.y += u.y; t1.z += u.z; t1.w += u.w;
        t2.x += w.x; t2.y += w.y; t2.z += w.z; t2.w += w.w;
      }
      float* dst = part + (((int64_t)blockIdx.x * nseg + s) * 2) * C;
      *reinterpret_cast<float4*>(dst + cl * 4) = t1;
      *reinterpret_cast<float4*>(dst + C + cl * 4) = t2;
    }
  }
}

template <bool POOL>
__global__ void k_norm_bwd_apply(const float* __restrict__ x, const float* __restrict__ y, const float* __restrict__ gy,
                                 const float* __restrict__ gy2, const int* __restrict__ pool_parent,
                                 const int* __restrict__ pool_arg, const int* __restrict__ seg, int seg_stride, int64_t n, int C,
                                 const float* __restrict__ mean, const float* __restrict__ var, float eps,
                                 const float* __restrict__ gamma, const float* __restrict__ beta,
                                 const float* __restrict__ sums ,
                                 const float* __restrict__ cnt, int act, float* __restrict__ gx, float* __restrict__ gres,
                                 unsigned* __restrict__ amax_out) {
  int64_t t = (int64_t)blockIdx.x * blockDim.x + threadIdx.x;
  const int c4n = C / 4;
  unsigned am = 0u;
  if (t < n * c4n) {
  int64_t r = t / c4n;
  int c = (int)(t % c4n) * 4;
  int s = seg_of(seg, seg_stride, r);
  float inv_n = 1.f / cnt[s];
  float xv[4], gv[4], muv[4], vav[4], gam[4], bet[4] = {0.f, 0.f, 0.f, 0.f}, s1[4], s2[4], yv[4], o[4], gr[4];
  *reinterpret_cast<float4*>(xv) = *reinterpret_cast<const float4*>(x + r * C + c);
  if (POOL) {
    const int64_t o = pool_parent[r];
    const int4 a = *reinterpret_cast<const int4*>(pool_arg + o * C + c);
    *reinterpret_cast<float4*>(gv) = *reinterpret_cast<const float4*>(gy + o * C + c);
    gv[0] = a.x == r ? gv[0] : 0.f; gv[1] = a.y == r ? gv[1] : 0.f; gv[2] = a.z == r ? gv[2] : 0.f; gv[3] = a.w == r ? gv[3] : 0.f;
  } else {
    *reinterpret_cast<float4*>(gv) = *reinterpret_cast<const float4*>(gy + r * C + c);
  }
  if (gy2) {
    const float4 t2 = *reinterpret_cast<const float4*>(gy2 + r * C + c);
    gv[0] += t2.x; gv[1] += t2.y; gv[2] += t2.z; gv[3] += t2.w;
  }
  *reinterpret_cast<float4*>(muv) = *reinterpret_cast<const float4*>(mean + (int64_t)s * C + c);
  *reinterpret_cast<float4*>(vav) = *reinterpret_cast<const float4*>(var + (int64_t)s * C + c);
  *reinterpret_cast<float4*>(s1) = *reinterpret_cast<const float4*>(sums + ((int64_t)s * 2) * C + c);
  *reinterpret_cast<float4*>(s2) = *reinterpret_cast<const float4*>(sums + ((int64_t)s * 2 + 1) * C + c);
  if (gamma) *reinterpret_cast<float4*>(gam) = *reinterpret_cast<const float4*>(gamma + c);
  else gam[0] = gam[1] = gam[2] = gam[3] = 1.f;
  const bool from_y = act && y;
  if (from_y) *reinterpret_cast<float4*>(yv) = *reinterpret_cast<const float4*>(y + r * C + c);
  if (beta) *reinterpret_cast<float4*>(bet) = *reinterpret_cast<const float4*>(beta + c);
#pragma unroll
  for (int j = 0; j < 4; ++j) {
    float g = gv[j];
    float is = 1.f / sqrtf(vav[j] + eps);
    if (from_y) g *= act_bwd_from_y(yv[j], act);
    else if (act) g *= act_bwd_from_pre(bn_pre(xv[j], muv[j], is, gam[j], bet[j]), act);
    float xh = (xv[j] - muv[j]) * is;
    gr[j] = g;
    o[j] = gam[j] * is * (g - s1[j] * inv_n - xh * s2[j] * inv_n);
  }
  *reinterpret_cast<float4*>(gx + r * C + c) = *reinterpret_cast<float4*>(o);
  if (gres) *reinterpret_cast<float4*>(gres + r * C + c) = *reinterpret_cast<float4*>(gr);
#pragma unroll
  for (int j = 0; j < 4; ++j) amax_fold(am, o[j]);
  }
  if (amax_out) amax_commit(am, amax_out);
}
```

fcaf3d_amd/csrc/norm_stats.h:

```cpp
#pragma once

__global__ void k_stats_partial(const float* __restrict__ x, const int* __restrict__ seg, int seg_stride, int64_t n, int C,
                                int nseg, const float* __restrict__ mean, int mode, int64_t rpb, float* __restrict__ part,
                                float* __restrict__ part_cnt) {
  extern __shared__ float sm[];
  __shared__ int srange[2];
  const int c4n = C / 4;
  const auto [cl, rl, nrl] = lane_coord(c4n);
  const auto [r0, r1] = row_span(rpb, n);
  int s_lo, s_hi;
  seg_range(seg, seg_stride, r0, r1, &s_lo, &s_hi, srange);
  const bool chk = seg && s_lo != s_hi;
  for (int s = 0; s < nseg; ++s) {
    float4 acc[4];
    float4 sq = make_float4(0.f, 0.f, 0.f, 0.f);
    float cnt = 0.f;
#pragma unroll
    for (int u = 0; u < 4; ++u) acc[u] = make_float4(0.f, 0.f, 0.f, 0.f);
    if (s >= s_lo && s <= s_hi) {
      float4 mu = make_float4(0.f, 0.f, 0.f, 0.f);
      if (mode == 1) mu = *reinterpret_cast<const float4*>(mean + (int64_t)s * C + cl * 4);
      for (int64_t rb = r0 + rl; rb < r1; rb += 4 * nrl) {
        float4 vv[4];
        bool ok[4];
#pragma unroll
        for (int u = 0; u < 4; ++u) {
          const int64_t r = rb + (int64_t)u * nrl;
          ok[u] = r < r1;
          const int64_t rc = ok[u] ? r : r0;
          if (chk) ok[u] = ok[u] && seg[rc * seg_stride] == s;
          vv[u] = *reinterpret_cast<const float4*>(x + rc * C + cl * 4);
        }
#pragma unroll
        for (int u = 0; u < 4; ++u) {
          if (!ok[u]) continue;
          float4 v = vv[u];
          if (mode == 1) {
            v.x -= mu.x; v.y -= mu.y; v.z -= mu.z; v.w -= mu.w;
            v.x *= v.x; v.y *= v.y; v.z *= v.z; v.w *= v.w;
          }
          if (mode == 2) { sq.x += v.x * v.x; sq.y += v.y * v.y; sq.z += v.z * v.z; sq.w += v.w * v.w; }
          acc[u].x += v.x; acc[u].y += v.y; acc[u].z += v.z; acc[u].w += v.w;
          cnt += 1.f;
        }
      }
    }
    float4 a;
    a.x = (acc[0].x + acc[1].x) + (acc[2].x + acc[3].x);
    a.y = (acc[0].y + acc[1].y) + (acc[2].y + acc[3].y);
    a.z = (acc[0].z + acc[1].z) + (acc[2].z + acc[3].z);
    a.w = (acc[0].w + acc[1].w) + (acc[2].w + acc[3].w);
    __syncthreads();
    *reinterpret_cast<float4*>(&sm[(rl * c4n + cl) * 4]) = a;
    float* smc = sm + nrl * C;
    if (cl == 0) smc[rl] = cnt;
    __syncthreads();
    const int64_t slot = (int64_t)blockIdx.x * nseg + s;
    float* dst = mode == 2 ? part + slot * 2 * C : part + slot * C;
    if (rl == 0) {
      float4 t = make_float4(0.f, 0.f, 0.f, 0.f);
      for (int j = 0; j < nrl; ++j) {
        float4 u = *reinterpret_cast<const float4*>(&sm[(j * c4n + cl) * 4]);
        t.x += u.x; t.y += u.y; t.z += u.z; t.w += u.w;
      }
      *reinterpret_cast<float4*>(dst + cl * 4) = t;
      if (cl == 0 && part_cnt) {
        float c = 0.f;
        for (int j = 0; j < nrl; ++j) c += smc[j];
        part_cnt[slot] = c;
      }
    }
    if (mode == 2) {
      __syncthreads();
      *reinterpret_cast<float4*>(&sm[(rl * c4n + cl) * 4]) = sq;
      __syncthreads();
      if (rl == 0) {
        float4 t = make_float4(0.f, 0.f, 0.f, 0.f);
        for (int j = 0; j < nrl; ++j) {
          float4 u = *reinterpret_cast<const float4*>(&sm[(j * c4n + cl) * 4]);
          t.x += u.x; t.y += u.y; t.z += u.z; t.w += u.w;
        }
        *reinterpret_cast<float4*>(dst + C + cl * 4) = t;
      }
    }
  }
}

static_assert(FIN_CB == 4 && FIN_SL == 64, "k_seg_meanvar_final spells out the 4 channels x 64 slices its launch (final_launch) gives it");
__global__ __launch_bounds__(256) void k_seg_meanvar_final(const float* __restrict__ part, const float* __restrict__ part_cnt,
                                                           int64_t nblocks, int nseg, int C, float* __restrict__ mean,
                                                           float* __restrict__ var, float* __restrict__ cnt_out) {
  __shared__ double r1[64][5], r2[64][5], rc[64];
  const int cgroups = (C + 3) / 4;
  const int s = blockIdx.x / cgroups, cg = blockIdx.x % cgroups;
  const int cl = threadIdx.x & 3, j = threadIdx.x >> 2;
  const int c = cg * 4 + cl;
  double a1 = 0., a2 = 0., ac = 0.;
  if (c < C) {
    for (int64_t b = j; b < nblocks; b += 64) {
      const float* src = part + ((b * nseg + s) * 2) * C;
      a1 += fc_ld(&src[c]);
      a2 += fc_ld(&src[C + c]);
      if (cl == 0) ac += fc_ld(&part_cnt[b * nseg + s]);
    }
  }
  r1[j][cl] = a1; r2[j][cl] = a2;
  if (cl == 0) rc[j] = ac;
  __syncthreads();
  if (j == 0 && c < C) {
    double s1 = 0., s2 = 0., n = 0.;
    for (int q = 0; q < 64; ++q) { s1 += r1[q][cl]; s2 += r2[q][cl]; n += rc[q]; }
    double m = 0., v = 0.;
    if (n > 0.) {
      m = s1 / n;
      v = s2 / n - m * m;
      if (v < 0.) v = 0.;
    }
    mean[(int64_t)s * C + c] = (float)m;
    var[(int64_t)s * C + c] = (float)v;
    if (c == 0) cnt_out[s] = (float)n;
  }
}

__global__ __launch_bounds__(256) void k_stats_final(const float* __restrict__ part, const float* __restrict__ part_cnt,
                                                      int64_t nblocks, int nseg, int C, int mode, float* __restrict__ out,
                                                      float* __restrict__ cnt_io) {
  __shared__ float red[FIN_SL][FIN_CB + 1];
  __shared__ float redc[FIN_SL];
  const int cgroups = (C + FIN_CB - 1) / FIN_CB;
  const int s = blockIdx.x / cgroups, cg = blockIdx.x % cgroups;
  const int cl = threadIdx.x & (FIN_CB - 1), j = threadIdx.x / FIN_CB;
  const int c = cg * FIN_CB + cl;
  float a0 = 0.f, a1 = 0.f, a2 = 0.f, a3 = 0.f;
  if (c < C) {
    int64_t b = j;
    for (; b + 3 * FIN_SL < nblocks; b += 4 * FIN_SL) {
      const float v0 = fc_ld(&part[(b * nseg + s) * C + c]), v1 = fc_ld(&part[((b + FIN_SL) * nseg + s) * C + c]);
      const float v2 = fc_ld(&part[((b + 2 * FIN_SL) * nseg + s) * C + c]), v3 = fc_ld(&part[((b + 3 * FIN_SL) * nseg + s) * C + c]);
      a0 += v0; a1 += v1; a2 += v2; a3 += v3;
    }
    for (; b < nblocks; b += FIN_SL) a0 += fc_ld(&part[(b * nseg + s) * C + c]);
  }
  float acc = (a0 + a1) + (a2 + a3);
  red[j][cl] = acc;
  if (mode == 0 && cl == 0) {
    float cc = 0.f;
    for (int64_t b = j; b < nblocks; b += FIN_SL) cc += fc_ld(&part_cnt[b * nseg + s]);
    redc[j] = cc;
  }
  __syncthreads();
  if (j == 0 && c < C) {
    float t = 0.f;
    for (int q = 0; q < FIN_SL; ++q) t += red[q][cl];
    float cnt = 1.f;
    if (mode == 0) {
      float cc = 0.f;
      for (int q = 0; q < FIN_SL; ++q) cc += redc[q];
      if (c == 0) cnt_io[s] = cc;
      cnt = cc;
    } else if (mode == 1) {
      cnt = cnt_io[s];
    }
    out[(int64_t)s * C + c] = (mode == 2) ? t : (cnt > 0.f ? t / cnt : 0.f);
  }
}
```

fcaf3d_amd/csrc/pool_rows.h:

```cpp
#pragma once

__global__ void k_maxpool_fwd(const float* __restrict__ in, const int* __restrict__ nbr, int64_t n_out, int K, int C,
                              float* __restrict__ out, int* __restrict__ argrow) {
  int64_t t = (int64_t)blockIdx.x * blockDim.x + threadIdx.x;
  if (t >= n_out * C) return;
  int64_t o = t / C;
  int c = (int)(t % C);
  float best = -INFINITY;
  int arg = -1;
  for (int k = 0; k < K; ++k) {
    int i = nbr[(int64_t)k * n_out + o];
    if (i < 0) continue;
    float v = in[(int64_t)i * C + c];
    if (arg < 0 || v > best) { best = v; arg = i; }
  }
  out[t] = arg < 0 ? 0.f : best;
  argrow[t] = arg;
}

__global__ void k_maxpool8_fwd(const float* __restrict__ in, const int* __restrict__ nbr, int64_t n_out, int C,
                               float* __restrict__ out, int* __restrict__ argrow, unsigned* __restrict__ amax_out) {
  const int c4n = C / 4;
  int64_t t = (int64_t)blockIdx.x * blockDim.x + threadIdx.x;
  unsigned am = 0u;
  if (t < n_out * c4n) {
  const int64_t o = t / c4n;
  const int c = (int)(t % c4n) * 4;
  int idx[8];
#pragma unroll
  for (int k = 0; k < 8; ++k) idx[k] = nbr[(int64_t)k * n_out + o];
  float4 v[8];
#pragma unroll
  for (int k = 0; k < 8; ++k) {
    const int i = idx[k] < 0 ? 0 : idx[k];
    v[k] = *reinterpret_cast<const float4*>(in + (int64_t)i * C + c);
  }
  float best[4] = {-INFINITY, -INFINITY, -INFINITY, -INFINITY};
  int arg[4] = {-1, -1, -1, -1};
#pragma unroll
  for (int k = 0; k < 8; ++k) {
    if (idx[k] < 0) continue;
    const float e[4] = {v[k].x, v[k].y, v[k].z, v[k].w};
#pragma unroll
    for (int j = 0; j < 4; ++j)
      if (arg[j] < 0 || e[j] > best[j]) { best[j] = e[j]; arg[j] = idx[k]; }
  }
  float4 ob = make_float4(arg[0] < 0 ? 0.f : best[0], arg[1] < 0 ? 0.f : best[1], arg[2] < 0 ? 0.f : best[2], arg[3] < 0 ? 0.f : best[3]);
  *reinterpret_cast<float4*>(out + o * C + c) = ob;
  *reinterpret_cast<int4*>(argrow + o * C + c) = make_int4(arg[0], arg[1], arg[2], arg[3]);
  amax_fold(am, ob.x); amax_fold(am, ob.y); amax_fold(am, ob.z); amax_fold(am, ob.w);
  }
  if (amax_out) amax_commit(am, amax_out);
}

__global__ void k_maxpool_bwd(const float* __restrict__ gout, const int* __restrict__ argrow, int64_t n_out, int C,
                              float* __restrict__ gin) {
  int64_t t = (int64_t)blockIdx.x * blockDim.x + threadIdx.x;
  if (t >= n_out * C) return;
  int i = argrow[t];
  if (i >= 0) gin[(int64_t)i * C + (t % C)] = gout[t];
}

__global__ void k_norm_act_maxpool8_fwd(const float* __restrict__ x, const int* __restrict__ seg, int seg_stride, int C,
                                        const float* __restrict__ mean, const float* __restrict__ var, float eps,
                                        const float* __restrict__ gamma, const float* __restrict__ beta, int act,
                                        const int* __restrict__ nbr, int64_t n_out, float* __restrict__ out, int* __restrict__ argrow,
                                        float* __restrict__ y, int* __restrict__ parent, unsigned* __restrict__ amax_out) {
  const int c4n = C / 4;
  int64_t t = (int64_t)blockIdx.x * blockDim.x + threadIdx.x;
  unsigned am = 0u;
  if (t < n_out * c4n) {
  const int64_t o = t / c4n;
  const int c = (int)(t % c4n) * 4;
  int idx[8];
#pragma unroll
  for (int k = 0; k < 8; ++k) idx[k] = nbr[(int64_t)k * n_out + o];
  if (parent) {
    int mine = -1;
#pragma unroll
    for (int k = 0; k < 8; ++k) mine = (c == 4 * k) ? idx[k] : mine;
    if (mine >= 0) parent[mine] = (int)o;
  }
  float4 v[8];
  int first = -1;
#pragma unroll
  for (int k = 0; k < 8; ++k) {
    const int i = idx[k] < 0 ? 0 : idx[k];
    if (first < 0 && idx[k] >= 0) first = idx[k];
    v[k] = *reinterpret_cast<const float4*>(x + (int64_t)i * C + c);
  }
  float best[4] = {-INFINITY, -INFINITY, -INFINITY, -INFINITY};
  int arg[4] = {-1, -1, -1, -1};
  if (first >= 0) {
    const int s = seg_of(seg, seg_stride, first);
    float mu[4], va[4], is[4], g[4] = {1.f, 1.f, 1.f, 1.f}, b[4] = {0.f, 0.f, 0.f, 0.f};
    *reinterpret_cast<float4*>(mu) = *reinterpret_cast<const float4*>(mean + (int64_t)s * C + c);
    *reinterpret_cast<float4*>(va) = *reinterpret_cast<const float4*>(var + (int64_t)s * C + c);
    if (gamma) *reinterpret_cast<float4*>(g) = *reinterpret_cast<const float4*>(gamma + c);
    if (beta) *reinterpret_cast<float4*>(b) = *reinterpret_cast<const float4*>(beta + c);
#pragma unroll
    for (int j = 0; j < 4; ++j) is[j] = 1.f / sqrtf(va[j] + eps);
#pragma unroll
    for (int k = 0; k < 8; ++k) {
      if (idx[k] < 0) continue;
      float e[4] = {v[k].x, v[k].y, v[k].z, v[k].w};
#pragma unroll
      for (int j = 0; j < 4; ++j) {
        e[j] = act_fwd(bn_pre(e[j], mu[j], is[j], g[j], b[j]), act);
        if (arg[j] < 0 || e[j] > best[j]) { best[j] = e[j]; arg[j] = idx[k]; }
      }
      if (y) *reinterpret_cast<float4*>(y + (int64_t)idx[k] * C + c) = make_float4(e[0], e[1], e[2], e[3]);
    }
  }
  float4 ob = make_float4(arg[0] < 0 ? 0.f : best[0], arg[1] < 0 ? 0.f : best[1], arg[2] < 0 ? 0.f : best[2], arg[3] < 0 ? 0.f : best[3]);
  *reinterpret_cast<float4*>(out + o * C + c) = ob;
  *reinterpret_cast<int4*>(argrow + o * C + c) = make_int4(arg[0], arg[1], arg[2], arg[3]);
  amax_fold(am, ob.x); amax_fold(am, ob.y); amax_fold(am, ob.z); amax_fold(am, ob.w);
  }
  if (amax_out) amax_commit(am, amax_out);
}

__global__ void k_inverse_rows(const int* __restrict__ rows, int64_t n, int64_t n_inv, int* __restrict__ inv) {
  const int64_t i = (int64_t)blockIdx.x * blockDim.x + threadIdx.x;
  if (i >= n) return;
  const int r = rows[i];
  if (r >= 0 && r < n_inv) inv[r] = (int)i;
}

__global__ void k_gather_rows(const float* __restrict__ src, const int* __restrict__ idx, int64_t n, int C,
                              float* __restrict__ dst) {
  int64_t t = (int64_t)blockIdx.x * blockDim.x + threadIdx.x;
  if (t >= n * C) return;
  int64_t r = t / C;
  int i = idx[r];
  dst[t] = i >= 0 ? src[(int64_t)i * C + (t % C)] : 0.f;
}

__global__ void k_scatter_rows_add(const float* __restrict__ src, const int* __restrict__ idx, int64_t n, int C,
                                   float* __restrict__ dst) {
  int64_t t = (int64_t)blockIdx.x * blockDim.x + threadIdx.x;
  if (t >= n * C) return;
  int64_t r = t / C;
  int i = idx[r];
  if (i >= 0) dst[(int64_t)i * C + (t % C)] += src[t];
}
```

fcaf3d_amd/executor.py:

```python
import os
import struct

import numpy as np
import torch

from . import _lib as L
from . import functional as Fn
from . import nn as MEnn
from .weight_images import ImageSet

ENABLED = os.environ.get('FC_EXEC', '1') != '0'
PROBE = None
KEEP_STATE = False


def _layouts():
    names, fields = {}, {}
    for block in L.parse_enums():
        names.update(block)
        *members, end = block
        op = names.get('OP_' + end[:-len('_END')]) if end.endswith('_END') else None
        if op is not None:
            fields[op] = {n[len(end) - 3:].lower().removesuffix('_p1'): (block[n], n.endswith('_P1')) for n in members}
    return {k: v for k, v in names.items() if k.startswith('OP_') or k in ('OPW', 'MAPW', 'ROW_OP', 'ROW_STREAM')}, fields


_NAMES, FIELDS = _layouts()
globals().update(_NAMES)


def word(op, field):
    return FIELDS[op][field][0]


ALIGN = 256
S_MAIN, S_HEAD, S_WGRAD = 0, 1, 2
EV_FORK, EV_HEAD_DONE, EV_W0, EV_W1, EV_WEND, EV_BWD0, EV_HB = 0, 8, 9, 10, 11, 12, 16


def _f(x):
    return struct.unpack('<q', struct.pack('<d', float(x)))[0]


def supported(det):
    bb, nh = det.backbone, det.neck_with_head
    if not (ENABLED and Fn.X6 and not (Fn.FLAGS & Fn.CONV_FMA) and Fn.STEM_COL and Fn.DGRAD_WT):
        return False
    if getattr(bb.BLOCK, 'expansion', 1) != 1 or det.spatial_sort:
        return False
    if 1 + nh.n_reg_outs + nh.n_classes > 64 or bb.conv1[0].in_channels != 3:
        return False
    return type(nh).forward_single is _FORWARD_SINGLE and type(nh).forward is _NECK_FORWARD


_FORWARD_SINGLE = _NECK_FORWARD = None


class NetProgram:
    def __init__(self, det, training, wgrad_async, head_overlap, tail0=False, keep_state=None):
        self.det = det
        self.tail0 = tail0
        self.keep_state = bool(KEEP_STATE if keep_state is None else keep_state)
        self.training = training
        self.wgrad_async = wgrad_async and training
        bb, nh = det.backbone, det.neck_with_head
        self.nl = min(bb.n_outs, 4)
        self.head_overlap = head_overlap and self.nl > 1
        self.dev = next(det.parameters()).device
        self.ops_f, self.ops_b = [], []
        self.n_addr = 0
        self.static = []
        self.arena = {'f': [], 'b': []}
        self.alias = []
        self.dyn = {}
        self.dim_names = {}
        self.map_names = {}
        self.grad_refs = []
        self.keep = []
        self.relu_outs = []
        self.pool_arg = None
        self.out_idx = None
        self.gout_idx = self.x0_idx = ()
        self.in_sums = None
        self.small = []
        self._pready = {}
        self._params = [p for p in det.parameters() if p.requires_grad]
        self._goff, off = {}, 0
        flat = getattr(self._params[0], '_fc_flat', None)
        self.flat = flat[0] if flat is not None else None
        for p in self._params:
            if self.flat is not None:
                assert p._fc_flat[0] is self.flat
                self._goff[id(p)] = p._fc_flat[1]
            else:
                self._goff[id(p)] = off
                off += -(-p.numel() // 64) * 64
        self._gtotal = self.flat.n if self.flat is not None else off
        self._sig = self.signature(det)
        self._build_weights()
        self._build(_Emitter(self))
        self._finalise()

    @staticmethod
    def signature(det):
        from .flat import GENERATION
        return GENERATION[0]

    def _new(self):
        self.n_addr += 1
        return self.n_addr - 1

    def D(self, name):
        if name not in self.dim_names:
            self.dim_names[name] = len(self.dim_names)
        return self.dim_names[name]

    def M(self, name):
        if name not in self.map_names:
            self.map_names[name] = len(self.map_names)
        return self.map_names[name]

    def T(self, rows, cols, arena='f', elem=4, extra=0):
        i = self._new()
        self.arena[arena].append((i, self.D(rows), cols * elem, extra))
        return i

    def S(self, tensor):
        i = self._new()
        self.static.append((i, tensor.data_ptr()))
        self.keep.append(tensor)
        return i

    def SA(self, address):
        i = self._new()
        self.static.append((i, int(address)))
        return i

    def DY(self, name):
        if name not in self.dyn:
            self.dyn[name] = self._new()
        return self.dyn[name]

    def AL(self, parent, off_dim, cols, elem=4):
        i = self._new()
        self.alias.append((i, parent, self.D(off_dim), cols * elem))
        return i

    def G(self, p):
        i = self._new()
        self.grad_refs.append((i, self._goff[id(p)]))
        return i

    def emit(self, lst, op, stream, **fields):
        row = [0] * OPW
        row[ROW_OP], row[ROW_STREAM] = op, stream
        self.patch(row, **fields)
        lst.append(row)

    @staticmethod
    def patch(row, **fields):
        layout = FIELDS[row[ROW_OP]]
        for k, v in fields.items():
            if k not in layout:
                raise KeyError(f'operator {row[ROW_OP]} has no field {k!r}')
            w, p1 = layout[k]
            row[w] = v + 1 if p1 else v

    def _build_weights(self):
        holder = self.det.__dict__.get('_exec_weights')
        if holder is None or holder.sig != self._sig:
            holder = self.det.__dict__['_exec_weights'] = _Weights(self.det, self.dev, self._sig)
        self.w = holder
        self.packed, self.gent_w, self.gents, self.ncol = holder.packed, holder.gent_w, holder.gents, holder.ncol

    def IMG(self, w, transposed):
        v = self.w.images.table.get((w.data_ptr(), 1 if w.dim() == 2 else w.shape[0], w.shape[-2], w.shape[-1]))
        assert v is not None and v[1 if transposed else 0] is not None, 'no split-bf16 image for this kernel shape'
        return self.S(v[1 if transposed else 0])

    def _build(self, em):
        bb, nh = self.det.backbone, self.det.neck_with_head
        x = em.stem(bb.conv1[0], bb.conv1[1])
        levels = []
        for li in range(1, self.nl + 1):
            x = em.level(li, getattr(bb, f'layer{li}'), x)
            levels.append(x)
        self.out_idx = (self.T('Nall', 1), self.T('Nall', nh.n_reg_outs), self.T('Nall', nh.n_classes), self.T('Nall', 1))
        if self.training:
            em.tape.append(lambda: em.flush_small(S_MAIN))
            self.gout_idx = (self.DY('g_cent'), self.DY('g_bbox'), self.DY('g_cls'))
        for i in range(self.nl - 1, -1, -1):
            if i < self.nl - 1:
                x = em.up(i, getattr(nh, f'up_block_{i + 1}'), x, levels[i])
            if i == 0 and self.tail0:
                self.x0_idx = x
                if self.training:
                    em.grads.arrive(x[0], self.DY('g_x0'), *x[1:], S_MAIN)
            else:
                em.head(i, getattr(nh, f'out_block_{i}'), x)
        if self.head_overlap:
            em.sync(self.ops_f, S_HEAD, S_MAIN, EV_HEAD_DONE)
        em.backward()

    def _finalise(self):
        self.ops_f = np.ascontiguousarray(np.asarray(self.ops_f, dtype=np.int64).reshape(-1, OPW))
        self.ops_b = np.ascontiguousarray(np.asarray(self.ops_b, dtype=np.int64).reshape(-1, OPW)) if self.ops_b else np.zeros((0, OPW), np.int64)
        self.addr0 = np.zeros(self.n_addr, dtype=np.int64)
        for i, a in self.static:
            self.addr0[i] = a

        def columns(table, width):
            return tuple(np.ascontiguousarray(np.array(table, dtype=np.int64).reshape(-1, width).T))
        self._ar = {k: columns(a, 4) for k, a in self.arena.items()}
        self._al = columns(self.alias, 4)
        self._gr = columns([(i, 4 * off) for i, off in self.grad_refs], 2)
        self.n_dims, self.n_maps = len(self.dim_names), len(self.map_names)
        self._ws = [None, None, None]
        self._need = np.zeros(3, dtype=np.int64)
        self._cfg = np.array([Fn.BN_SMALL_ELEMS, Fn.FLAGS, 0, 0], dtype=np.int64)
        self.n_conv_f = int((self.ops_f[:, ROW_OP] == OP_CONV).sum())
        self.n_conv_b = int((self.ops_b[:, ROW_OP] == OP_CONV).sum()) if len(self.ops_b) else 0
        self.n_amax = int((self.ops_f[:, ROW_OP] == OP_AMAX).sum()) + (int((self.ops_b[:, ROW_OP] == OP_AMAX).sum()) if len(self.ops_b) else 0)
        self._anchor = torch.zeros(1, device=self.dev, requires_grad=True)
        if self.training:
            n = len(self.small)
            self._small = np.zeros((2 * n, 8), dtype=np.int64)
            self._small_goff = np.zeros(2 * n, dtype=np.int64)
            self._small_in = None
            for k, (src, nseg, C, w, b) in enumerate(self.small):
                for h, p in ((0, b), (1, w)):
                    r = 2 * k + h
                    self._small[r, 2], self._small[r, 3], self._small[r, 4] = C, 1, 2 * C
                    self._small_goff[r] = self._goff[id(p)] * 4
                    if src is not None:
                        self._small[r, 0] = src + 4 * C * h
                    else:
                        self._small_in = (2 * k, C)

    def _fill_arena(self, addr, dims, which, base):
        idx, di, bpr, ext = self._ar[which]
        if len(idx) == 0:
            return
        sizes = (dims[di] * bpr + ext + (ALIGN - 1)) // ALIGN * ALIGN
        offs = np.cumsum(sizes) - sizes
        addr[idx] = base + offs

    def _arena_bytes(self, dims, which):
        idx, di, bpr, ext = self._ar[which]
        return int(((dims[di] * bpr + ext + (ALIGN - 1)) // ALIGN * ALIGN).sum()) + ALIGN

    def bind(self, x, batch_size, backward):
        nl = self.nl
        cm0 = x.cmap
        dims = np.zeros(self.n_dims, dtype=np.int64)
        maps = np.zeros((self.n_maps, MAPW), dtype=np.int64)
        dn, mn, N = self.dim_names, self.map_names, _Names

        def setd(k, v):
            if k in dn:
                dims[dn[k]] = v
        m1 = cm0.strided(2)
        m2 = m1.strided(2)
        maps[mn['stem']] = cm0.kernel_map(m1, 3).desc(conv=False)
        maps[mn['pool']] = m1.kernel_map(m2, 2).desc(conv=False)
        kms = {}
        setd('n0', cm0.n); setd('n1', m1.n); setd('n2', m2.n); setd('B', batch_size); setd('one', 1)
        prev, lv = m2, []
        for li in range(1, nl + 1):
            mi = prev.strided(2)
            kms[N.down(li)], kms[N.ds(li)], kms[N.same(li)] = prev.kernel_map(mi, 3), prev.kernel_map(mi, 1), mi.kernel_map(mi, 3)
            for k in (N.down(li), N.ds(li), N.same(li)):
                maps[mn[k]] = kms[k].desc(True, backward)
            setd(N.rows(li), mi.n)
            lv.append(mi)
            prev = mi
        xm = lv[-1]
        head_maps = [xm]
        dyn = {}
        for i in range(nl - 2, -1, -1):
            g = xm.generate()
            u, rows, swapped = lv[i].union(g)
            if not swapped or u is not g:
                return None
            kms[N.gsame(i)] = g.kernel_map(g, 3)
            maps[mn[N.gsame(i)]] = kms[N.gsame(i)].desc(True, backward)
            setd(N.gen(i), g.n)
            dyn[N.union(i)] = rows
            xm = g
            head_maps.append(g)
        head_maps = head_maps[::-1]
        off = 0
        for i, cm in enumerate(head_maps):
            if i == 0 and self.tail0:
                continue
            setd(N.off(i), off)
            off += cm.n
        setd('Nall', off)
        st = dict(dims=dims, maps=maps, dyn=dyn, head_maps=head_maps, x=x, seg1=m1.coords, n_all=off)
        if PROBE is not None:
            from .sparse import _rec
            st['pairs'] = {mn[k]: _rec(km._pairs[3].sum() if km._pairs is not None else (km.nbr >= 0).sum()) for k, km in kms.items()}
            PROBE.append(dict(pairs=st['pairs'], nf=self.n_conv_f, nb=self.n_conv_b, na=self.n_amax))
        return st

    def _streams(self):
        dev = self.dev
        nh = self.det.neck_with_head
        main = L.stream()
        head = nh._head_stream(dev).cuda_stream if self.head_overlap else main
        wg = Fn.wgrad_stream(dev).cuda_stream if self.wgrad_async else main
        return np.array([main, head, wg], dtype=np.int64)

    def _run(self, ops, addr, st, begin=0, end=None, size_only=False):
        streams = self._streams()
        self._cfg[2] = 1 if 'pairs' in st else 0
        self._cfg[3] = 1 if size_only else 0
        end = len(ops) if end is None else end
        while True:
            ws = np.array([w.data_ptr() if w is not None else 0 for w in self._ws], dtype=np.int64)
            wsb = np.array([w.numel() if w is not None else 0 for w in self._ws], dtype=np.int64)
            rc = L.lib().fc_exec(ops.ctypes.data, begin, end, addr.ctypes.data, st['dims'].ctypes.data, st['maps'].ctypes.data,
                                 streams.ctypes.data, ws.ctypes.data, wsb.ctypes.data, self._need.ctypes.data, self._cfg.ctypes.data)
            if rc == -2:
                for i in range(3):
                    if self._need[i] > wsb[i]:
                        self._ws[i] = torch.empty(int(self._need[i] * 5 // 4) + (1 << 20), dtype=torch.uint8, device=self.dev)
                continue
            if rc != 0:
                raise RuntimeError(f'fc_exec failed: {"invalid argument" if rc == -1 else "hipError %d" % rc}')
            return

    def decisions(self, st):
        assert self.keep_state, 'this program does not store the stem\'s normalised output: build it under executor.KEEP_STATE'
        relu = [(self._view(st, *t) > 0).cpu() for t in self.relu_outs]
        return relu, self._view(st, *self.pool_arg, torch.int32).cpu()

    def _view(self, st, idx, rows, C, dtype=torch.float32):
        fa, n = st['fa'], int(st['dims'][self.dim_names[rows]])
        o = int(st['addr'][idx] - fa.data_ptr())
        return fa[o:o + n * C * 4].view(dtype).view(n, C)

    def forward(self, st):
        self.w.ensure(trusted=ImageSet.held is self.w or (not self.training and getattr(self.det, 'static_weights', False)))
        self.w.wait()
        if self.training:
            return _NetFn.apply(self._anchor, self, st)
        return self._forward(st)

    def _forward(self, st):
        dims = st['dims']
        fa = torch.empty(self._arena_bytes(dims, 'f'), dtype=torch.uint8, device=self.dev)
        addr = self.addr0.copy()
        base = (fa.data_ptr() + ALIGN - 1) // ALIGN * ALIGN
        self._fill_arena(addr, dims, 'f', base)
        addr[self.dyn['x0']] = st['x'].F.data_ptr()
        addr[self.dyn['seg1']] = st['seg1'].data_ptr()
        for k, t in st['dyn'].items():
            addr[self.dyn[k]] = t.data_ptr()
        ai, ap, ad, ab = self._al
        fwd_alias = addr[ap] != 0
        addr[ai[fwd_alias]] = addr[ap[fwd_alias]] + dims[ad[fwd_alias]] * ab[fwd_alias]
        st['fa'], st['addr'] = fa, addr
        self._run(self.ops_f, addr, st)
        nh = self.det.neck_with_head
        outs = [self._view(st, idx, 'Nall', c) for idx, c in zip(self.out_idx, (1, nh.n_reg_outs, nh.n_classes, 1))]
        if self.tail0:
            outs.append(self._view(st, *self.x0_idx))
        return tuple(outs)

    def _backward(self, st, g_cent, g_bbox, g_cls, g_x0=None):
        dims, addr = st['dims'], st['addr']
        n = st['n_all']
        nh = self.det.neck_with_head
        gs = []
        for g, c in zip((g_cent, g_bbox, g_cls), (1, nh.n_reg_outs, nh.n_classes)):
            gs.append(g.contiguous() if g is not None else torch.zeros((n, c), dtype=torch.float32, device=self.dev))
        if self.tail0:
            t, rows, C = self.x0_idx
            n0 = int(dims[self.dim_names[rows]])
            g_x0 = g_x0.contiguous() if g_x0 is not None else torch.zeros((n0, C), dtype=torch.float32, device=self.dev)
            gs.append(g_x0)
        ba = torch.empty(self._arena_bytes(dims, 'b'), dtype=torch.uint8, device=self.dev)
        base = (ba.data_ptr() + ALIGN - 1) // ALIGN * ALIGN
        self._fill_arena(addr, dims, 'b', base)
        for k, g in zip(('g_cent', 'g_bbox', 'g_cls', 'g_x0'), gs):
            addr[self.dyn[k]] = g.data_ptr()
        ai, ap, ad, ab = self._al
        addr[ai] = addr[ap] + dims[ad] * ab
        own = self._own_params()
        pre = [(p, p.grad) for p in own if p.grad is not None]
        aliased = self.flat is not None and any(g.data_ptr() == self.flat.grad_view(p).data_ptr() for p, g in pre)
        accum = bool(pre) and (self.flat is None or aliased or len(pre) > 16)
        if self.flat is not None and not accum:
            gbuf = self.flat.grad
        else:
            gbuf = torch.zeros(self._gtotal, dtype=torch.float32, device=self.dev)
        gi, go = self._gr
        addr[gi] = gbuf.data_ptr() + go
        desc = self._small.copy()
        desc[:, 1] = gbuf.data_ptr() + self._small_goff
        r, C = self._small_in
        B = int(dims[self.dim_names['B']])
        desc[r, 0], desc[r + 1, 0] = addr[self.in_sums], addr[self.in_sums] + 4 * C
        desc[r:r + 2, 3] = B
        desc_dev = L.upload(desc, self.dev)
        addr[self.dyn['small_desc']] = desc_dev.data_ptr()
        gv = self._grad_views(gbuf)
        if not accum:
            for p in own:
                p.grad = gv[id(p)]
        from . import dist as D
        av = D.ACTIVE
        if av is not None and av.buckets and av.flat is self.flat and self.flat is not None and not accum and not self.tail0:
            pos = 0
            self._run(self.ops_b, addr, st, size_only=True)
            for upto in self._bucket_ready(av):
                if upto > pos:
                    self._run(self.ops_b, addr, st, pos, upto)
                    pos = upto
                av.launch_next()
            if pos < len(self.ops_b):
                self._run(self.ops_b, addr, st, pos, len(self.ops_b))
        else:
            self._run(self.ops_b, addr, st)
        if accum:
            for p in own:
                if p.grad is None:
                    p.grad = gv[id(p)]
                else:
                    p.grad.add_(gv[id(p)])
        else:
            for p, g0 in pre:
                gv[id(p)].add_(g0)
            if self.flat is not None and not self.tail0:
                self.flat.complete = True
        st['ba'] = ba

    def _own_params(self):
        c = getattr(self, '_own', None)
        if c is None:
            c = self._own = [p for p in self._params if id(p) in self._pready]
        return c

    def _bucket_ready(self, av):
        key = id(av)
        c = getattr(self, '_br', None)
        if c is None or c[0] != key:
            out, run = [], 0
            for b in av.buckets:
                run = max(run, max(self._pready[id(p)] for p in b))
                out.append(run)
            c = self._br = (key, out)
        return c[1]

    def _grad_views(self, gbuf):
        key = gbuf.data_ptr()
        cache = getattr(self, '_gv', None)
        if cache is None or cache[0] != key:
            views = {id(p): gbuf[self._goff[id(p)]:self._goff[id(p)] + p.numel()].view(p.shape) for p in self._params}
            cache = self._gv = (key, views, gbuf)
        return cache[1]


class _Names:
    rows, down, ds, same = 'L{}'.format, 'down{}'.format, 'ds{}'.format, 'same{}'.format
    gen, gsame, off, union = 'g{}'.format, 'gsame{}'.format, 'off{}'.format, 'rows{}'.format


class _Grads:

    def __init__(self, em):
        self.em = em
        self.full = {}
        self.second = {}
        self.behind = {}
        self.src = {}

    def _add(self, t, g, rows, cols, stream):
        em, dst = self.em, self.full[t]
        em.p.emit(em.Bk, OP_ADD, stream, dst=dst, src=g, n=em.p.D(rows), c=cols)
        self.src.pop(dst, None)
        em.amax_of.pop(dst, None)

    def arrive(self, t, g, rows, cols, stream):
        if t not in self.full:
            self.full[t] = g
        elif Fn.BN_FUSE and t not in self.second:
            self.second[t] = (g, rows, cols, stream)
        else:
            self.own(t)
            self._add(t, g, rows, cols, stream)

    def take(self, t, rows, cols, pair=False):
        if t in self.behind:
            g, lvl = self.behind.pop(t)
            self.em.join(lvl)
            self.arrive(t, g, rows, cols, S_MAIN)
        if pair:
            return self.full[t], (self.second.pop(t)[0] if t in self.second else None)
        return self.own(t)

    def own(self, t):
        if t in self.second:
            self._add(t, *self.second.pop(t))
        return self.full[t]

    def deliver(self, t, lvl):
        self.behind[t] = (self.own(t), lvl)
        del self.full[t]


class _Emitter:

    AMAX_SLOTS = 1024
    AMAX_SLOT_BYTES = 2048

    def __init__(self, p):
        self.p, self.F, self.Bk, self.tr = p, p.ops_f, p.ops_b, p.training
        nh = p.det.neck_with_head
        self.grads = _Grads(self)
        self.main = []
        self.branches = {}
        self.tape = self.main
        self.branch = None
        self.branch_params = {}
        self.flushed = 0
        self.producer = {}
        self.n_reg, self.n_cls, self.Cn = nh.n_reg_outs, nh.n_classes, nh.centerness_conv.in_channels
        self.n_heads = p.nl - (1 if p.tail0 else 0)
        self.head_partials = 0
        if self.tr:
            self.head_part = torch.zeros((p.nl, self.Cn, 64), dtype=torch.float32, device=p.dev)
            self.bias_part = torch.zeros((p.nl, self.n_cls), dtype=torch.float32, device=p.dev)
            p.keep += [self.head_part, self.bias_part]
        self.amax = Fn.X6 and Fn.split_mode() == 2
        self.amax_f = {}
        self.amax_of = {}
        self.amax_used = 0
        if self.amax:
            self.amax_buf = torch.zeros(self.AMAX_SLOTS * self.AMAX_SLOT_BYTES // 4, dtype=torch.int32, device=p.dev)
            p.keep.append(self.amax_buf)
            self.amax_slot()
            p.emit(self.F, OP_CLEAR, S_MAIN, dst=p.SA(self.amax_buf.data_ptr()), bytes=0)

    def amax_slot(self):
        assert self.amax_used < self.AMAX_SLOTS
        self.amax_used += 1
        return self.p.SA(self.amax_buf.data_ptr() + self.AMAX_SLOT_BYTES * (self.amax_used - 1))

    def amax_op(self, lst, stream, x, rows, cols):
        slot = self.amax_slot()
        self.p.emit(lst, OP_AMAX, stream, x=x, n=self.p.D(rows), c=cols, slot=slot)
        return slot

    def amax_fwd(self, x, rows, cols, stream):
        if not self.amax:
            return -1
        if x in self.amax_of:
            return self.amax_of[x]
        if (x, stream) not in self.amax_f:
            self.amax_f[(x, stream)] = self.amax_op(self.F, stream, x, rows, cols)
        return self.amax_f[(x, stream)]

    def folded(self, t):
        if self.amax:
            self.amax_of[t] = self.amax_slot()
        return self.amax_of.get(t, -1)

    def sync(self, lst, src, dst, event):
        self.p.emit(lst, OP_RECORD, src, event=event)
        self.p.emit(lst, OP_WAIT, dst, event=event)

    def wgrad(self, cur, op, **fields):
        if self.p.wgrad_async:
            self.sync(self.Bk, cur, S_WGRAD, EV_W0 if cur == S_MAIN else EV_W1)
        self.p.emit(self.Bk, op, S_WGRAD if self.p.wgrad_async else cur, **fields)

    def wrote(self, *params):
        for prm in params:
            self.p._pready[id(prm)] = len(self.Bk)
        if self.branch is not None:
            self.branch_params.setdefault(self.branch, []).extend(params)

    def join(self, lvl):
        self.p.emit(self.Bk, OP_WAIT, S_MAIN, event=EV_HB + lvl)
        for prm in self.branch_params.pop(lvl, ()):
            self.p._pready[id(prm)] = max(self.p._pready[id(prm)], len(self.Bk))

    def flush_small(self, stream):
        p, n = self.p, len(self.p.small) - self.flushed
        if n:
            p.emit(self.Bk, OP_SMALL_GRADS, stream, desc=p.DY('small_desc'), first=2 * self.flushed, count=2 * n)
            for _, _, _, w_, b_ in p.small[self.flushed:]:
                self.wrote(w_, b_)
            self.flushed = len(p.small)

    def head_wfin(self, stream):
        p, nh, lo = self.p, self.p.det.neck_with_head, self.p.nl - self.n_heads
        p.emit(self.Bk, OP_HEAD_WFIN, stream, part=p.SA(self.head_part[lo].data_ptr()), nl=self.n_heads, r=self.Cn, ld=64, n_reg=self.n_reg,
               n_cls=self.n_cls, g_cent=p.G(nh.centerness_conv.kernel), g_reg=p.G(nh.reg_conv.kernel), g_cls=p.G(nh.cls_conv.kernel),
               bias_part=p.SA(self.bias_part[lo].data_ptr()), g_bias=p.G(nh.cls_conv.bias))
        self.wrote(nh.centerness_conv.kernel, nh.reg_conv.kernel, nh.cls_conv.kernel, nh.cls_conv.bias)

    def conv(self, x, rows_in, rows_out, mod=None, mname=None, dense=None, stream=S_MAIN):
        p, F, Bk, G = self.p, self.F, self.Bk, self.grads
        if dense is None:
            w, gw, Cin, Cout, m, n = mod.kernel, None, mod.in_channels, mod.out_channels, p.M(mname), -1
        else:
            (w, gw), m, n = dense, -1, p.D(rows_in)
            Cin, Cout = w.shape[-2:]
        y = p.T(rows_out, Cout)
        ax = self.amax_fwd(x, rows_in, Cin, stream)
        p.emit(F, OP_CONV, stream, x=x, img=p.IMG(w, False), map=m, dir=0, out=y, n=n, cin=Cin, cout=Cout, amax_x=ax)
        self.producer[y] = (len(F) - 1, rows_out, Cout)

        def bwd():
            gy = G.take(y, rows_out, Cout) if stream == S_MAIN else G.own(y)
            gx = p.T(rows_in, Cin, 'b')
            ag = (self.amax_of[gy] if gy in self.amax_of else self.amax_op(Bk, stream, gy, rows_out, Cout)) if self.amax else -1
            p.emit(Bk, OP_CONV, stream, x=gy, img=p.IMG(w, True), map=m, dir=1, out=gx, n=n, cin=Cout, cout=Cin, amax_x=ag)
            G.src[gx] = (len(Bk) - 1, rows_in, Cin, stream)
            self.wgrad(stream, OP_WGRAD, x=x, gout=gy, map=m, gw=p.G(w) if gw is None else gw, n=n, cin=Cin, cout=Cout, amax_x=ax, amax_gout=ag)
            if gw is None:
                self.wrote(w)
            G.arrive(x, gx, rows_in, Cin, stream)
        if self.tr:
            self.tape.append(bwd)
        return y

    def bn(self, x, mod, act, rows, res=None, stream=S_MAIN, add=None):
        assert add is None or res is None
        p, F, Bk, G, tr = self.p, self.F, self.Bk, self.grads, self.tr
        b, C = mod.bn, mod.bn.num_features
        y = p.T(rows, C)
        mean, var, cnt = (p.T('one', C), p.T('one', C), p.T('one', 1)) if tr else (-1, -1, -1)
        if act == Fn.ACT['relu']:
            p.relu_outs.append((y, rows, C))
        prod, groups = -1, 1
        if tr and Fn.BN_FUSE and x in self.producer:
            prod, prows, pcols = self.producer[x]
            groups = pcols // C
            assert pcols == groups * C and groups in (1, 8)
            p.patch(F[prod], stats=p.T(prows, pcols // 8, extra=8 * pcols + 256))
        ay = self.folded(y)
        add_inv, add_src = add if add is not None else (-1, -1)
        p.emit(F, OP_BN_FWD, stream, x=x, n=p.D(rows), c=C, eps=_f(b.eps), gamma=p.S(b.weight), beta=p.S(b.bias),
               res=-1 if res is None else res, act=act, momentum=_f(b.momentum), y=y, mean=mean, var=var, cnt=cnt,
               rmean=p.S(b.running_mean), rvar=p.S(b.running_var), nbt=p.S(b.num_batches_tracked), train=1 if tr else 0,
               producer=prod, groups=groups, amax_y=ay, add_inv=add_inv, add_src=add_src)
        if not tr:
            return y
        sums = torch.zeros((2, C), dtype=torch.float32, device=p.dev)
        si = p.S(sums)

        def bwd():
            p.small.append((sums.data_ptr(), None, C, b.weight, b.bias))
            gy, gy2 = G.take(y, rows, C, pair=True) if stream == S_MAIN else (G.own(y), None)
            gx = p.T(rows, C, 'b')
            gres = p.T(rows, C, 'b') if res is not None else -1
            prod = -1
            last, first = (gy, None) if gy2 is None else (gy2, gy)
            src = G.src.get(last)
            if Fn.BN_FUSE and src is not None and src[3] == stream and src[1:3] == (rows, C):
                prod = src[0]
                p.patch(Bk[prod], stats=p.T(rows, C // 8, 'b', extra=8 * C + 256), bn_x=x, bn_mean=mean, bn_var=var,
                        bn_gamma=p.S(b.weight), bn_beta=p.S(b.bias), bn_eps=_f(b.eps), bn_act=act,
                        bn_add=-1 if first is None else first, bn_y=-1 if res is None else y)
            agx = self.folded(gx)
            p.emit(Bk, OP_BN_BWD, stream, x=x, y=y if res is not None else -1, gy=gy, n=p.D(rows), c=C, mean=mean, var=var,
                   cnt=cnt, eps=_f(b.eps), gamma=p.S(b.weight), beta=p.S(b.bias), act=act, gx=gx, gres=gres, sums=si,
                   gy2=-1 if gy2 is None else gy2, producer=prod, amax_gx=agx)
            G.arrive(x, gx, rows, C, stream)
            if res is not None:
                G.arrive(res, gres, rows, C, stream)
        self.tape.append(bwd)
        return y

    def stem(self, stem, inorm):
        p, F, tr, relu = self.p, self.F, self.tr, Fn.ACT['relu']
        x0, seg1 = p.DY('x0'), p.DY('seg1')
        t_stem = p.T('n1', 64)
        col = p.T('n1', 84) if tr else -1
        p.emit(F, OP_STEM_FWD, S_MAIN, x=x0, w=p.S(stem.kernel), map=p.M('stem'), out=t_stem, col=col)
        mean_in, var_in, cnt_in = p.T('B', 64), p.T('B', 64), p.T('B', 1)
        p.emit(F, OP_COL_STATS, S_MAIN, x=t_stem, seg=seg1, n=p.D('n1'), c=64, nseg=p.D('B'), mean=mean_in, var=var_in, cnt=cnt_in)
        t_in = p.T('n1', 64) if p.keep_state else -1
        if p.keep_state:
            p.relu_outs.append((t_in, 'n1', 64))
        t_pool, arg = p.T('n2', 64), p.T('n2', 64)
        p.pool_arg = (arg, 'n2', 64)
        ap = self.folded(t_pool)
        pool_parent = p.T('n1', 1) if tr else -1
        p.emit(F, OP_NORM_POOL_FWD, S_MAIN, x=t_stem, seg=seg1, c=64, mean=mean_in, var=var_in, eps=_f(inorm.eps), gamma=p.S(inorm.weight),
               beta=p.S(inorm.bias), act=relu, map=p.M('pool'), out=t_pool, arg=arg, y=t_in, amax_out=ap, parent=pool_parent)
        if tr:
            p.in_sums = p.T('B', 2 * 64, 'b')

            def bwd():
                p.small.append((None, 'B', 64, inorm.weight, inorm.bias))
                g_pool = self.grads.take(t_pool, 'n2', 64)
                g_stem = p.T('n1', 64, 'b')
                p.emit(self.Bk, OP_POOL_NORM_BWD, S_MAIN, x=t_stem, g_pool=g_pool, arg=arg, parent=pool_parent, seg=seg1, n=p.D('n1'), c=64,
                       nseg=p.D('B'), mean=mean_in, var=var_in, cnt=cnt_in, eps=_f(inorm.eps), gamma=p.S(inorm.weight),
                       beta=p.S(inorm.bias), act=relu, gx=g_stem, sums=p.in_sums)
                self.wgrad(S_MAIN, OP_STEM_WGRAD, col=col, gout=g_stem, map=p.M('stem'), gw=p.G(stem.kernel))
                self.wrote(stem.kernel)
            self.tape.append(bwd)
        return t_pool, 'n2', 64

    def level(self, li, layer, x):
        relu, none, N = Fn.ACT['relu'], Fn.ACT['none'], _Names
        (cur, cur_rows, _), rows = x, N.rows(li)
        if self.tr:
            self.tape.append(lambda: self.flush_small(S_MAIN))
        for j, blk in enumerate(layer):
            if j == 0:
                assert blk.downsample is not None and blk.conv1.stride == 2
                t_ds = self.conv(cur, cur_rows, rows, blk.downsample[0], N.ds(li))
                res = self.bn(t_ds, blk.downsample[1], none, rows)
                t1 = self.conv(cur, cur_rows, rows, blk.conv1, N.down(li))
            else:
                assert blk.downsample is None
                res = cur
                t1 = self.conv(cur, rows, rows, blk.conv1, N.same(li))
            t1 = self.bn(t1, blk.norm1, relu, rows)
            t2 = self.conv(t1, rows, rows, blk.conv2, N.same(li))
            cur = self.bn(t2, blk.norm2, relu, rows, res=res)
        return cur, rows, blk.conv1.out_channels

    def up(self, i, up, x, fb):
        p, F, Bk, G, tr, elu = self.p, self.F, self.Bk, self.grads, self.tr, Fn.ACT['elu']
        (x, x_rows, x_C), (fb, fb_rows, _) = x, fb
        g_rows, Ci = _Names.gen(i), up[0].out_channels
        gw_tmp = torch.zeros((x_C, 8 * Ci), dtype=torch.float32, device=p.dev)
        gw_i = p.S(gw_tmp)

        def bwd_perm():
            p.emit(Bk, OP_PERMUTE_GENT, S_WGRAD if p.wgrad_async else S_MAIN, src=gw_i, dst=p.G(up[0].kernel), cin=x_C, cout=Ci)
            self.wrote(up[0].kernel)
            self.flush_small(S_MAIN)
        if tr:
            self.tape.append(bwd_perm)
        t = self.conv(x, x_rows, x_rows, dense=(p.gent_w[p.gents.index(up[0])], gw_i))
        t = self.bn(t, up[1], elu, g_rows)
        t = self.conv(t, g_rows, g_rows, up[3], _Names.gsame(i))
        rows_i = p.DY(_Names.union(i))
        inv_i = p.T(g_rows, 1)
        p.emit(F, OP_INV_ROWS, S_MAIN, rows=rows_i, n=p.D(fb_rows), n_inv=p.D(g_rows), inv=inv_i)
        u = self.bn(t, up[4], elu, g_rows, add=(inv_i, fb))

        def bwd_union():
            gu = G.take(u, g_rows, Ci)
            gfb = p.T(fb_rows, Ci, 'b')
            p.emit(Bk, OP_GATHER, S_MAIN, src=gu, idx=rows_i, n=p.D(fb_rows), c=Ci, dst=gfb)
            G.arrive(fb, gfb, fb_rows, Ci, S_MAIN)
        if tr:
            self.tape.append(bwd_union)
        return u, g_rows, Ci

    def head(self, i, ob, x):
        p, F, Bk, tr = self.p, self.F, self.Bk, self.tr
        nh, n_reg, n_cls = p.det.neck_with_head, self.n_reg, self.n_cls
        x, rows, _ = x
        hs = S_HEAD if (p.head_overlap and i > 0) else S_MAIN
        if hs == S_HEAD:
            self.sync(F, S_MAIN, S_HEAD, EV_FORK + i)
            self.tape = []
            self.branches[i] = (x, self.tape)
        o = self.conv(x, rows, rows, ob[0], _Names.same(p.nl) if i == p.nl - 1 else _Names.gsame(i), stream=hs)
        o = self.bn(o, ob[1], Fn.ACT['elu'], rows, stream=hs)
        gw_head = p.SA(self.head_part[i].data_ptr()) if tr else -1

        def partial_done():
            self.head_partials += 1
            if self.head_partials == self.n_heads and p.wgrad_async:
                self.head_wfin(S_WGRAD)
        if tr:
            self.tape.append(partial_done)
        y = self.conv(o, rows, rows, dense=(p.packed, gw_head), stream=hs)
        off = _Names.off(i)
        outs = [p.AL(t, off, c) for t, c in zip(p.out_idx, (1, n_reg, n_cls, 1))]
        p.emit(F, OP_HEAD_FWD, hs, y=y, ld=64, bias=p.S(nh.cls_conv.bias), scale=p.S(nh.scales[i].scale), n=p.D(rows), n_reg=n_reg,
               n_cls=n_cls, cent=outs[0], bbox=outs[1], cls=outs[2], cmax=outs[3])

        def bwd():
            gy = p.T(rows, 64, 'b')
            gin = [p.AL(g, off, c) for g, c in zip(p.gout_idx, (1, n_reg, n_cls))]
            agy = self.folded(gy)
            p.emit(Bk, OP_HEAD_BWD, hs, y=y, ld=64, scale=p.S(nh.scales[i].scale), bbox=outs[1], g_cent=gin[0], g_bbox=gin[1],
                   g_cls=gin[2], n=p.D(rows), n_reg=n_reg, n_cls=n_cls, gy=gy, gs_row=-1, g_scale=p.G(nh.scales[i].scale),
                   bias_part=p.SA(self.bias_part[i].data_ptr()), amax_gy=agy)
            self.wrote(nh.scales[i].scale)
            self.grads.arrive(y, gy, rows, 64, hs)
        if tr:
            self.tape.append(bwd)
        self.tape = self.main

    def backward(self):
        p, Bk, tr = self.p, self.Bk, self.tr
        if self.amax:
            n_fwd_slots = self.amax_used
            p.patch(self.F[0], bytes=self.AMAX_SLOT_BYTES * n_fwd_slots)
            if tr:
                p.emit(Bk, OP_CLEAR, S_MAIN, dst=p.SA(self.amax_buf.data_ptr() + self.AMAX_SLOT_BYTES * n_fwd_slots), bytes=0)
        if not tr:
            return
        if p.head_overlap:
            self.sync(Bk, S_MAIN, S_HEAD, EV_BWD0)
            for lvl in sorted(self.branches):
                xt, tape = self.branches[lvl]
                assert xt not in self.grads.full
                self.branch = lvl
                for e in reversed(tape):
                    e()
                self.flush_small(S_HEAD)
                self.branch = None
                p.emit(Bk, OP_RECORD, S_HEAD, event=EV_HB + lvl)
                self.grads.deliver(xt, lvl)
        for e in reversed(self.main):
            e()
        assert not self.grads.behind and not self.branch_params, 'a head branch was never joined'
        if not p.wgrad_async:
            self.head_wfin(S_MAIN)
        self.flush_small(S_MAIN)
        assert self.head_partials == self.n_heads
        missing = [n for n, prm in p.det.named_parameters() if prm.requires_grad and id(prm) not in p._pready]
        if p.tail0:
            missing = [n for n in missing if not (n.startswith('neck_with_head.out_block_0.') or n == 'neck_with_head.scales.0.scale')]
        assert not missing, missing
        if p.wgrad_async:
            self.sync(Bk, S_WGRAD, S_MAIN, EV_WEND)
        if self.amax:
            p.patch(Bk[0], bytes=self.AMAX_SLOT_BYTES * (self.amax_used - n_fwd_slots))


class _Weights(ImageSet):

    def __init__(self, det, dev, sig):
        nh = det.neck_with_head
        self.det, self.sig = det, sig
        head = (nh.centerness_conv, nh.reg_conv, nh.cls_conv)
        convs = [m for m in det.modules() if isinstance(m, MEnn.MinkowskiConvolution) and m not in head]
        self.gents = [m for m in det.modules() if isinstance(m, MEnn.MinkowskiGenerativeConvolutionTranspose)]
        C = nh.centerness_conv.in_channels
        self.ncol = 1 + nh.n_reg_outs + nh.n_classes
        self.packed = torch.zeros((1, C, 64), dtype=torch.float32, device=dev)
        self.gent_w = [torch.empty((1, m.in_channels, 8 * m.out_channels), dtype=torch.float32, device=dev) for m in self.gents]
        ws = [m.kernel for m in convs] + [self.packed] + self.gent_w
        super().__init__([m.kernel for m in convs + list(head) + self.gents], weights=ws)

    def lookup(self, weight, transposed):
        return None

    @torch.no_grad()
    def prepare(self):
        nh = self.det.neck_with_head
        torch.cat((nh.centerness_conv.kernel, nh.reg_conv.kernel, nh.cls_conv.kernel), dim=1, out=self.packed[0][:, :self.ncol])
        for m, w in zip(self.gents, self.gent_w):
            w.view(m.in_channels, 8, m.out_channels).copy_(m.kernel.permute(1, 0, 2))


class _NetFn(torch.autograd.Function):

    @staticmethod
    def forward(ctx, anchor, prog, st):
        ctx.prog, ctx.st = prog, st
        outs = prog._forward(st)
        ctx.mark_non_differentiable(outs[3])
        return outs

    @staticmethod
    def backward(ctx, g_cent, g_bbox, g_cls, _g_max, g_x0=None):
        ctx.prog._backward(ctx.st, g_cent, g_bbox, g_cls, g_x0)
        return None, None, None


def program_for(det, training, tail0=False):
    if not supported(det):
        return None
    nh = det.neck_with_head
    if tail0 and min(det.backbone.n_outs, 4) < 2:
        return None
    key = (bool(training), bool(Fn.WGRAD_ASYNC), bool(nh.head_overlap), bool(tail0))
    keep = bool(KEEP_STATE)
    fuse = bool(Fn.BN_FUSE)
    mode = Fn.split_mode() if Fn.X6 else -1
    cache = det.__dict__.setdefault('_programs', {})
    sig = NetProgram.signature(det)
    prog = cache.get(key + (fuse, mode, keep))
    if prog is None or prog._sig != sig:
        prog = cache[key + (fuse, mode, keep)] = NetProgram(det, *key, keep_state=keep)
    return prog
```

include/fcaf3d_hip.h:

```cpp
#ifndef FCAF3D_HIP_H
#define FCAF3D_HIP_H
#include <stdint.h>

#ifndef __HIP_PLATFORM_AMD__
typedef struct ihipStream_t* hipStream_t;
#endif

#ifdef __cplusplus
extern "C" {
#endif

#define FC_ABI_VERSION 14
#ifndef FC_AMAX_SLOT_BYTES
#define FC_AMAX_SLOT_BYTES 2048
#endif
int fc_abi_version(void);


int fc_voxelize(const float* points, int64_t n, int pt_stride, int batch_idx, float voxel_size, float feat_div,
                int nfeat, int* coords, float* feats, hipStream_t stream);

int fc_augment_voxelize(const float* points, int64_t n_src, int pt_stride, const int* sample_idx, int64_t n_out,
                        const float* xform_host, int batch_idx, float voxel_size, float feat_div, int nfeat, int* coords,
                        float* feats, float* points_out, hipStream_t stream);

#define FC_BATCH_DESC_WORDS 18
int fc_batch_augment_voxelize(const float* arena, int64_t arena_rows, int pt_stride, const int64_t* desc, int B, int64_t total_out,
                              int64_t out_rows, const int* sample_idx, int64_t n_idx, float voxel_size, float feat_div, int nfeat,
                              int* coords, float* feats, int* sample_out, float* points_out, hipStream_t stream);

int fc_morton_keys(const int* coords, int64_t n, long long* keys, hipStream_t stream);

int fc_scan_flags(const unsigned char* flags, int64_t n, int* pos, int* total_dev, void* ws, int64_t ws_bytes,
                  hipStream_t stream);
int fc_compact_rows(const unsigned char* flags, const int* pos, int64_t n, int* kept, int64_t m, hipStream_t stream);

int64_t fc_hash_unique_ws_bytes(int64_t n);
int fc_hash_unique(const int* coords, int64_t n, int q, unsigned long long* table_keys, int* table_vals, int64_t cap,
                   int* out_coords, int* first_idx, int* inverse, int* n_out_dev, void* ws, int64_t ws_bytes,
                   hipStream_t stream);

int fc_kernel_map(const int* out_coords, int64_t n_out, const unsigned long long* table_keys, const int* table_vals,
                  int64_t cap, const int* offsets, int K, int* nbr, hipStream_t stream);
int fc_nbr_row_masks(const int* nbr, int64_t n_out, int K, int* masks, hipStream_t stream);
int fc_permute_nbr(const int* nbr, const int* order, int64_t n_out, int K, int* nbr_sorted, hipStream_t stream);
int64_t fc_kernel_map_pairs_ws_bytes(int64_t n_out, int K);
int fc_kernel_map_pairs(const int* nbr, int64_t n_out, int K, int* pair_in, int* pair_out, int* pair_pos, int* cnt,
                        void* ws, int64_t ws_bytes, hipStream_t stream);
int fc_kernel_map_transpose(const int* nbr, int64_t n_out, int64_t n_in, int K, int* nbr_t, hipStream_t stream);

int fc_gen_coords(const int* coords, int64_t n, int half_stride, int* out_coords, hipStream_t stream);

int fc_kernel_map_children(const int* parent_nbr, int64_t n_parent, int* nbr, hipStream_t stream);
int fc_child_rows(const int* query_coords, int64_t n, const unsigned long long* parent_keys, const int* parent_vals,
                  int64_t cap, int child_stride, int* rows, int* n_found_dev, hipStream_t stream);

int64_t fc_union_map_ws_bytes(int64_t n_b);
int fc_union_map(const int* coords_b, int64_t n_b, const unsigned long long* table_keys_a, const int* table_vals_a,
                 int64_t cap_a, int64_t n_a, int* row_b, int* new_coords, int* n_new_dev, void* ws, int64_t ws_bytes,
                 hipStream_t stream);

int fc_interp(const int* query_coords, int64_t n, const unsigned long long* table_keys, const int* table_vals, int64_t cap,
              const float* feats, int C, int tensor_stride, float* out, hipStream_t stream);

int fc_gather_coords(const int* src, const int* idx, int64_t n, int* dst, hipStream_t stream);


int fc_plan_cfg_words(void);
int fc_plan_out_words(int B, int nl);
int64_t fc_plan_stage1_bytes(int64_t total_points, int B, int nl, int nfeat);
int fc_plan_levels(const int64_t* cfg, const int64_t* scenes, void* arena1, int64_t arena1_bytes, int64_t* out, int* counts_host,
                   hipStream_t stream);
int64_t fc_plan_stage2_bytes(const int64_t* cfg, int64_t* out, const int* counts_host);
int fc_plan_maps(const int64_t* cfg, int64_t* out, const int* counts_host, void* arena2, int64_t arena2_bytes, int* cnt_host,
                 hipStream_t stream);
int64_t fc_plan_probe_read(float* ms, double* bytes, int* kind, int64_t cap);
int64_t fc_argsort27_ws_bytes(int64_t n);
int fc_argsort27(const int* keys, int64_t n, int* order, void* ws, int64_t ws_bytes, hipStream_t stream);


#define FC_CONV_FMA (1 << 0)
#define FC_CONV_BM_SHIFT 4
#define FC_CONV_BN_SHIFT 6
#define FC_CONV_TILE_MASK 3
#define FC_CONV_S_SHIFT 8
#define FC_CONV_S_MASK 255
#define FC_CONV_WGRAD_PIPE_OFF (1 << 16)
#define FC_CONV_PIPE_OFF (1 << 17)
#define FC_CONV_PIPE_ON (1 << 18)
#define FC_CONV_WGRAD_DEEP (1 << 19)
#define FC_CONV_WGRAD_PIPE_ON (1 << 20)
#define FC_CONV_GLDS (1 << 21)
#define FC_CONV_GLDS_OFF (1 << 22)
#define FC_CONV_WT (1 << 23)
#define FC_CONV_SPLIT (1 << 24)
#define FC_CONV_IMAGE (1 << 26)
#define FC_CONV_FLAT (1 << 27)
#define FC_CONV_WGRAD_MULTI_OFF (1 << 29)
#define FC_CONV_WGRAD_MULTI_FIRST (1 << 30)

int64_t fc_x6_weight_image_bytes(int K, int R, int C);
int fc_x6_weight_image(const float* W, void* img, int K, int R, int C, int transposed, hipStream_t stream);
int fc_x6_weight_images(const int64_t* desc, int n, int64_t total_blocks, hipStream_t stream);

int64_t fc_conv_fwd_ws_bytes(int64_t n_out, int K, int Cin, int Cout, int flags);
int fc_conv_fwd(const float* in, const float* W, const int* nbr, const int* out_index, float* out, int64_t n_in,
                int64_t n_out, int K, int Cin, int Cout, int flags, void* ws, int64_t ws_bytes, hipStream_t stream);

int64_t fc_conv_fwd_pairs_ws_bytes(int64_t n_out, int K, int Cout);
int fc_conv_fwd_pairs(const float* in, const float* W, const int* pair_in, const int* pair_cnt, const int* pair_pos,
                      float* out, int64_t n_in, int64_t n_out, int K, int Cin, int Cout, int flags, void* ws,
                      int64_t ws_bytes, hipStream_t stream);

int fc_conv_fwd_pairs_tiles(const float* in, const float* W, const int* pair_in, const int* pair_cnt, const int* pair_pos,
                            float* out, int64_t n_in, int64_t n_out, int K, int Cin, int Cout, int64_t live_tiles, int flags,
                            void* ws, int64_t ws_bytes, hipStream_t stream);

int64_t fc_conv_stats_blocks(int64_t n_out, int K, int Cin, int Cout, int flags, int pairs);
int fc_conv_fwd_stats(const float* in, const float* W, const int* nbr, const int* out_index, float* out, int64_t n_in,
                      int64_t n_out, int K, int Cin, int Cout, int flags, void* ws, int64_t ws_bytes, float* stats,
                      hipStream_t stream);
int fc_conv_fwd_pairs_tiles_stats(const float* in, const float* W, const int* pair_in, const int* pair_cnt, const int* pair_pos,
                                  float* out, int64_t n_in, int64_t n_out, int K, int Cin, int Cout, int64_t live_tiles, int flags,
                                  void* ws, int64_t ws_bytes, float* stats, hipStream_t stream);
int fc_conv_fwd_bn_bwd_stats(const float* in, const float* W, const int* nbr, const int* out_index, float* out, int64_t n_in,
                             int64_t n_out, int K, int Cin, int Cout, int flags, void* ws, int64_t ws_bytes, float* stats,
                             const float* bn_x, const float* mean, const float* var, const float* gamma, const float* beta, float eps,
                             int act, const float* add, const float* bn_y, hipStream_t stream);
int fc_conv_fwd_pairs_tiles_bn_bwd_stats(const float* in, const float* W, const int* pair_in, const int* pair_cnt, const int* pair_pos,
                                         float* out, int64_t n_in, int64_t n_out, int K, int Cin, int Cout, int64_t live_tiles, int flags,
                                         void* ws, int64_t ws_bytes, float* stats, const float* bn_x, const float* mean,
                                         const float* var, const float* gamma, const float* beta, float eps, int act,
                                         const float* add, const float* bn_y, hipStream_t stream);

int64_t fc_conv_wgrad_ws_bytes(int64_t n_out, int K, int Cin, int Cout, int flags);
int fc_conv_wgrad(const float* in, const float* gout, const int* nbr, const int* row_index, float* gW, int64_t n_in,
                  int64_t n_out, int K, int Cin, int Cout, int flags, void* ws, int64_t ws_bytes, hipStream_t stream);
int fc_conv_wgrad_pairs(const float* in, const float* gout, const int* pair_in, const int* pair_out, const int* pair_cnt,
                        float* gW, int64_t n_in, int64_t n_out, int K, int Cin, int Cout, int flags, void* ws,
                        int64_t ws_bytes, hipStream_t stream);

int fc_stem_conv_fwd(const float* in, const float* W, const int* nbr, float* out, float* col, int64_t n_in, int64_t n_out,
                     int K, hipStream_t stream);
int64_t fc_stem_conv_wgrad_ws_bytes(int64_t n_out, int K);
int fc_stem_conv_wgrad(const float* col, const float* gout, float* gW, int64_t n_out, int K, void* ws, int64_t ws_bytes,
                       hipStream_t stream);

int fc_transpose_weight(const float* W, float* Wt, int K, int Cin, int Cout, hipStream_t stream);

enum { FC_TABLE_NONE, FC_TABLE_DENSE, FC_TABLE_SORTED, FC_TABLE_PAIRS, FC_TABLE_STATS = 8 };
enum { FC_FAM_INVALID, FC_FAM_STEM, FC_FAM_FMA, FC_FAM_MFMA, FC_FAM_MFMA_P, FC_FAM_GLDS, FC_FAM_X6, FC_FAM_H3R };
enum { FC_WFAM_INVALID, FC_WFAM_STEM, FC_WFAM_FMA, FC_WFAM_MFMA, FC_WFAM_MFMA_P, FC_WFAM_MULTI, FC_WFAM_X6T };
enum { FC_WSRC_FP32, FC_WSRC_FP32_T, FC_WSRC_IMAGE };
enum { FC_MODE_FP32, FC_MODE_SIX, FC_MODE_BF16, FC_MODE_H3 };
enum { FC_EPI_NONE, FC_EPI_KERNEL, FC_EPI_SUM };
enum { FC_ROUTE_FAMILY, FC_ROUTE_BM, FC_ROUTE_BN, FC_ROUTE_WM, FC_ROUTE_S, FC_ROUTE_WSRC, FC_ROUTE_MODE, FC_ROUTE_BUF, FC_ROUTE_EPI,
       FC_ROUTE_GRID_X, FC_ROUTE_GRID_Y, FC_ROUTE_GRID_Z };
enum { FC_WROUTE_FAMILY, FC_WROUTE_BM, FC_WROUTE_BN, FC_WROUTE_KO, FC_WROUTE_BKR, FC_WROUTE_TABLE, FC_WROUTE_MODE, FC_WROUTE_S,
       FC_WROUTE_RPS, FC_WROUTE_WBUF, FC_WROUTE_GRID_Y };
int fc_conv_fwd_route(int64_t n_in, int64_t n_out, int K, int Cin, int Cout, int flags, int table_kind, int64_t live_tiles,
                      int* out);
int fc_conv_wgrad_route(int64_t n_in, int64_t n_out, int K, int Cin, int Cout, int flags, int table_kind, int* out);


int64_t fc_col_stats_ws_bytes(int64_t n, int C, int nseg);
int fc_col_stats(const float* x, const int* seg, int seg_stride, int64_t n, int C, int nseg, float* mean, float* var,
                 float* cnt, void* ws, int64_t ws_bytes, hipStream_t stream);

int fc_seg_col_sums(const float* x, const int* seg, int seg_stride, int64_t n, int C, int nseg, float* out, void* ws,
                    int64_t ws_bytes, hipStream_t stream);
int fc_bn_running_update(const float* mean, const float* var, const float* cnt, float momentum, int C, float* running_mean,
                         float* running_var, long long* num_batches_tracked, hipStream_t stream);

int fc_norm_act_fwd(const float* x, const int* seg, int seg_stride, int64_t n, int C, const float* mean, const float* var,
                    float eps, const float* gamma, const float* beta, const float* residual, int act, float* y,
                    hipStream_t stream);
int64_t fc_norm_act_bwd_ws_bytes(int64_t n, int C, int nseg);
int fc_norm_act_bwd(const float* x, const float* y, const float* gy, const int* seg, int seg_stride, int64_t n, int C,
                    int nseg, const float* mean, const float* var, const float* cnt, float eps, const float* gamma,
                    const float* beta, int act, float* gx, float* gres, float* sums, void* ws, int64_t ws_bytes,
                    hipStream_t stream);

int64_t fc_bn_stats_ws_bytes(int64_t n, int C);
int fc_bn_stats_train(const float* x, int64_t n, int C, float momentum, float* mean, float* var, float* cnt,
                      float* running_mean, float* running_var, long long* num_batches_tracked, void* ws,
                      int64_t ws_bytes, hipStream_t stream);
int64_t fc_bn_small_ws_bytes(int C);
int fc_bn_act_train_fwd(const float* x, int64_t n, int C, float eps, const float* gamma, const float* beta,
                        const float* residual, int act, float momentum, float* y, float* mean, float* var, float* cnt,
                        float* running_mean, float* running_var, long long* num_batches_tracked, void* ws,
                        int64_t ws_bytes, hipStream_t stream);
int fc_bn_act_train_bwd(const float* x, const float* y, const float* gy, int64_t n, int C, const float* mean,
                        const float* var, float eps, const float* gamma, const float* beta, int act, float* gx, float* gres,
                        float* sums, void* ws, int64_t ws_bytes, hipStream_t stream);

int64_t fc_bn_train_ws_bytes(int64_t n, int C);
int fc_bn_train_fwd(const float* x, int64_t n, int C, float eps, const float* gamma, const float* beta, const float* residual,
                    int act, float momentum, float* y, float* mean, float* var, float* cnt, float* running_mean,
                    float* running_var, long long* num_batches_tracked, const float* part, int64_t nb_part, int groups,
                    int64_t small_elems, void* ws, int64_t ws_bytes, hipStream_t stream);
int fc_bn_train_bwd(const float* x, const float* y, const float* gy, const float* gy2, int64_t n, int C, const float* mean,
                    const float* var, const float* cnt, float eps, const float* gamma, const float* beta, int act, float* gx,
                    float* gres, float* sums, const float* part, int64_t nb_part, int64_t small_elems, void* ws, int64_t ws_bytes,
                    hipStream_t stream);

enum { FC_NFORM_TRAIN, FC_NFORM_SMALL, FC_NFORM_SEG };
enum { FC_NSTATS_INVALID, FC_NSTATS_PROLOGUE, FC_NSTATS_PARTIAL_SMALL, FC_NSTATS_PARTIAL, FC_NSTATS_TABLE };
enum { FC_NAPPLY_NONE, FC_NAPPLY_BN1, FC_NAPPLY_BN2, FC_NAPPLY_ROWS };
enum { FC_NAMAX_NONE, FC_NAMAX_FOLDED, FC_NAMAX_PASS };
enum { FC_NRED_INVALID, FC_NRED_TABLE, FC_NRED_PARTIAL };
enum { FC_NBAPPLY_NONE, FC_NBAPPLY_PROLOGUE, FC_NBAPPLY_FINAL };
enum { FC_NROUTE_SUMS, FC_NROUTE_APPLY, FC_NROUTE_AMAX, FC_NROUTE_NP, FC_NROUTE_NB, FC_NROUTE_RPB, FC_NROUTE_CG, FC_NROUTE_THREADS, FC_NROUTE_LDS,
       FC_NROUTE_GRID_X, FC_NROUTE_GRID_Y, FC_NROUTE_WS_BYTES, FC_NROUTE_LAUNCHES };
int fc_bn_train_fwd_route(int64_t n, int C, int has_part, int64_t nb_part, int groups, int64_t small_elems, int* out);
int fc_bn_train_bwd_route(int64_t n, int C, int nseg, int has_part, int64_t nb_part, int64_t small_elems, int form, int* out);

int fc_maxpool_fwd(const float* in, const int* nbr, int64_t n_out, int K, int C, float* out, int* argrow,
                   hipStream_t stream);
int fc_maxpool_bwd(const float* gout, const int* argrow, int64_t n_out, int C, float* gin, hipStream_t stream);

int fc_norm_act_maxpool8_fwd(const float* x, const int* seg, int seg_stride, int C, const float* mean, const float* var, float eps,
                             const float* gamma, const float* beta, int act, const int* nbr, int64_t n_out, float* out,
                             int* argrow, float* y, int* parent, hipStream_t stream);
int64_t fc_maxpool8_norm_act_bwd_ws_bytes(int64_t n_in, int C, int nseg);
int fc_maxpool8_norm_act_bwd(const float* x, const float* gout, const int* argrow, const int* parent, const int* seg, int seg_stride,
                             int64_t n_in, int C, int nseg, const float* mean, const float* var, const float* cnt, float eps,
                             const float* gamma, const float* beta, int act, float* gx, float* sums, void* ws, int64_t ws_bytes,
                             hipStream_t stream);

int fc_inverse_rows(const int* rows, int64_t n, int64_t n_inv, int* inv, hipStream_t stream);
int fc_norm_act_add_fwd(const float* x, const int* seg, int seg_stride, int64_t n, int C, const float* mean, const float* var,
                        float eps, const float* gamma, const float* beta, const float* residual, int act, const int* add_inv,
                        const float* add_src, float* y, hipStream_t stream);
int fc_bn_train_add_fwd(const float* x, int64_t n, int C, float eps, const float* gamma, const float* beta, const float* residual,
                        int act, float momentum, float* y, float* mean, float* var, float* cnt, float* running_mean,
                        float* running_var, long long* num_batches_tracked, const float* part, int64_t nb_part, int groups,
                        int64_t small_elems, const int* add_inv, const float* add_src, void* ws, int64_t ws_bytes,
                        hipStream_t stream);

int fc_gather_rows(const float* src, const int* idx, int64_t n, int C, float* dst, hipStream_t stream);
int fc_scatter_rows_add(const float* src, const int* idx, int64_t n, int C, float* dst, hipStream_t stream);


int fc_focal_loss_fwd(const float* logits, const long long* labels, const float* row_weight, int64_t n, int C, float gamma,
                      float alpha, float* loss_rows, hipStream_t stream);
int fc_focal_loss_bwd(const float* logits, const long long* labels, const float* row_weight, int64_t n, int C, float gamma,
                      float alpha, const float* gscale_dev, float* glogits, hipStream_t stream);

int fc_aiou3d_fwd_bwd(const float* pred, const float* target, int target_stride, int64_t n, float eps, float* iou,
                      float* dpred, hipStream_t stream);

int64_t fc_fcaf3d_loss_ws_bytes(int64_t n);
int fc_fcaf3d_loss_fwd(const float* points, const float* bbox_pred, const float* centerness, const float* cls_score,
                       const float* centerness_t, const float* bbox_t, const long long* labels, const int* scene,
                       const float* inv_pos, const float* inv_den, int64_t n, int n_classes, float gamma, float alpha,
                       float lw_cls, float lw_centerness, float lw_bbox, float* loss_cls, float* loss_centerness,
                       float* loss_bbox, void* ws, int64_t ws_bytes, hipStream_t stream);
int fc_fcaf3d_loss_bwd(const float* points, const float* bbox_pred, const float* centerness, const float* cls_score,
                       const float* centerness_t, const float* bbox_t, const long long* labels, const int* scene,
                       const float* inv_pos, const float* inv_den, int64_t n, int n_classes, float gamma, float alpha,
                       float lw_cls, float lw_centerness, float lw_bbox, const float* g_cls, const float* g_centerness,
                       const float* g_bbox, float* grad_cls_score, float* grad_centerness, float* grad_bbox_pred,
                       hipStream_t stream);

int fc_riou3d_fwd_bwd(const float* pred, const float* target, const float* weight, int64_t n, float* iou, float* dpred,
                      hipStream_t stream);

enum { FC_EIOU_GIOU = 0, FC_EIOU_DIOU = 1 };
int fc_eiou3d_fwd_bwd(const float* pred, const float* target, int target_stride, const float* weight, int64_t n, int box_dim,
                      int kind, float* loss, float* iou, float* dpred, hipStream_t stream);

int fc_head_split_fwd(const float* y, int ld, const float* bias, const float* scale_dev, int64_t n, int n_reg, int n_cls,
                      float* centerness, float* bbox_pred, float* cls_score, float* cls_max, hipStream_t stream);
int fc_head_split_bwd(const float* y, int ld, const float* scale_dev, const float* bbox_pred, const float* g_centerness,
                      const float* g_bbox, const float* g_cls, int64_t n, int n_reg, int n_cls, float* gy,
                      float* gscale_row, hipStream_t stream);
int64_t fc_head_split_bwd_sums_ws_bytes(int64_t n);
int fc_head_split_bwd_sums(const float* y, int ld, const float* scale_dev, const float* bbox_pred, const float* g_centerness,
                           const float* g_bbox, const float* g_cls, int64_t n, int n_reg, int n_cls, float* gy, float* gbias,
                           float* gscale, void* ws, int64_t ws_bytes, hipStream_t stream);

int fc_sort_v(const float* vertices, const unsigned char* mask, const int* num_valid, int64_t n_pairs, int* idx,
              hipStream_t stream);

int64_t fc_assign_ws_bytes(int B, int M, int L);
int fc_assign_targets(const float* points, const int* scene, const int* level, int64_t N, const float* boxes,
                      const long long* labels, const int* box_count, int B, int M, int L, const int* order,
                      const int* seg_start, int limit, int topk, float* centerness_t, float* bbox_t, long long* labels_out,
                      void* ws, int64_t ws_bytes, hipStream_t stream);


int64_t fc_nms_bev_ws_bytes(int nseg, int stride);
int fc_nms_bev(const float* boxes, const int* counts_dev, int nseg, int stride, float thresh, int rotated,
               unsigned long long* mask_ws, int64_t ws_bytes, int* keep, int* keep_count, hipStream_t stream);
int fc_boxes_iou_bev(const float* boxes_a, int n, const float* boxes_b, int m, int rotated, float* out,
                     hipStream_t stream);


#define FC_MERGE_TO_BOTTOM 1
#define FC_MERGE_WITH_YAW 2
#define FC_MERGE_XF_FLIP_H (1ull << 32)
#define FC_MERGE_XF_FLIP_V (1ull << 33)
int64_t fc_merge_sorted_segments_ws_bytes(int nseg_out, int max_total);
int fc_merge_sorted_segments(const int64_t* desc, int nseg_out, int K, const int* counts_dev, const int* keep, int keep_stride,
                             const int64_t* ord, int ord_stride, const float* scores, int score_stride, const float* boxes,
                             int flags, int max_total, int cap, float* out_boxes, float* out_scores, int* out_src,
                             int* out_count, int stride_out, void* ws, int64_t ws_bytes, hipStream_t stream);


#define FC_EVAL_DET_BOTTOM 1
int64_t fc_eval_match_ws_bytes(int64_t n_det, int64_t n_gt, int n_thr);
int fc_eval_match(const float* det_boxes, int det_dim , const float* det_scores, const int64_t* det_labels,
                  const float* gt_boxes , const int* gt_labels,
                  const int64_t* seg , int n_scenes,
                  int64_t n_det, int64_t n_gt, const double* thr , int n_thr, int flags,
                  float* best_iou, int* best_gt, unsigned char* tp_bits, void* ws, int64_t ws_bytes, hipStream_t stream);


int64_t fc_grad_norm_ws_bytes(int64_t n);
int fc_grad_norm(const float* g, int64_t n, float max_norm, float* out, void* ws, int64_t ws_bytes, hipStream_t stream);
int fc_adamw_step(float* p, const float* g, float* m, float* v, int64_t n, float lr, float beta1, float beta2, float eps,
                  float weight_decay, float bias_correction1, float bias_correction2, const float* norm_and_clip,
                  hipStream_t stream);

int fc_set_bf16_fast(int on);

int fc_set_split_mode(int mode);
int fc_get_split_mode(void);
int fc_amax(const float* x, int64_t n, unsigned* slot, hipStream_t stream);
int fc_conv_amax_hint(const unsigned* amax_in, const unsigned* amax_gout);
int fc_amax_out_hint(unsigned* amax_word);
int fc_debug_set_h3r(int mode);


int fc_exec_op_words(void);
int64_t fc_exec_probe_read(float* ms, int64_t* meta, int64_t cap);
int fc_exec_map_words(void);
int fc_exec(const int64_t* ops, int64_t op_begin, int64_t op_end, const int64_t* addr, const int64_t* dims, const int64_t* maps,
            const int64_t* streams, const int64_t* ws, const int64_t* ws_bytes, int64_t* ws_need, const int64_t* cfg);

#ifdef __cplusplus
}
#endif
#endif
```

Before: 514.1.

## Replace stem maxpool argrow with per-input-row 64-bit winner bitmask in training

In training, the stem maxpool forward now writes a compact 64-bit mask per input row saying which channels won the max, in place of a full n2×64 int argrow tensor. The fused pool+norm backward reads that mask to gate the pooled gradient, so it no longer needs a 256-byte argrow row per output. The backward partial kernel is also specialised at compile time on from_y/gy2, and k_stats_final is simplified to a sum-only form. The mask path only supports C=64 and adds shuffle work in the forward kernel.

```diff
diff --git a/fcaf3d_amd/_lib.py b/fcaf3d_amd/_lib.py
--- a/fcaf3d_amd/_lib.py
+++ b/fcaf3d_amd/_lib.py
@@ -53,7 +53,7 @@
     return blocks
 
 
-ABI_VERSION = 14
+ABI_VERSION = 15
 _lib = None
 _protos = None
 
diff --git a/fcaf3d_amd/csrc/exec.hip b/fcaf3d_amd/csrc/exec.hip
--- a/fcaf3d_amd/csrc/exec.hip
+++ b/fcaf3d_amd/csrc/exec.hip
@@ -420,6 +420,14 @@
       if (c.dry) return 0;
       if ((int)m[MAP_K] != 8) return FC_EINVAL;
       if (op[NORM_POOL_FWD_AMAX_OUT_P1] > 0) fc_amax_out_hint(P1<unsigned>(c, op[NORM_POOL_FWD_AMAX_OUT_P1]));
+      if (op[NORM_POOL_FWD_MASK_P1] > 0)
+        return fc_norm_act_maxpool8_mask_fwd(P<const float>(c, op[NORM_POOL_FWD_X]), P<const int>(c, op[NORM_POOL_FWD_SEG]),
+                                             op[NORM_POOL_FWD_SEG] >= 0 ? 4 : 0, (int)op[NORM_POOL_FWD_C], P<const float>(c, op[NORM_POOL_FWD_MEAN]),
+                                             P<const float>(c, op[NORM_POOL_FWD_VAR]), (float)as_double(op[NORM_POOL_FWD_EPS]),
+                                             P<const float>(c, op[NORM_POOL_FWD_GAMMA]), P<const float>(c, op[NORM_POOL_FWD_BETA]),
+                                             (int)op[NORM_POOL_FWD_ACT], reinterpret_cast<const int*>(m[MAP_NBR]), m[MAP_N_OUT],
+                                             P<float>(c, op[NORM_POOL_FWD_OUT]), P<int>(c, op[NORM_POOL_FWD_ARG]), P<float>(c, op[NORM_POOL_FWD_Y]),
+                                             P<int>(c, op[NORM_POOL_FWD_PARENT]), P1<unsigned long long>(c, op[NORM_POOL_FWD_MASK_P1]), st);
       return fc_norm_act_maxpool8_fwd(P<const float>(c, op[NORM_POOL_FWD_X]), P<const int>(c, op[NORM_POOL_FWD_SEG]),
                                       op[NORM_POOL_FWD_SEG] >= 0 ? 4 : 0, (int)op[NORM_POOL_FWD_C], P<const float>(c, op[NORM_POOL_FWD_MEAN]),
                                       P<const float>(c, op[NORM_POOL_FWD_VAR]), (float)as_double(op[NORM_POOL_FWD_EPS]),
@@ -432,6 +440,15 @@
       const int64_t n = c.dims[op[POOL_NORM_BWD_N]];
       const int C = (int)op[POOL_NORM_BWD_C], nseg = (int)c.dims[op[POOL_NORM_BWD_NSEG]];
       if (!want_ws(c, s, fc_maxpool8_norm_act_bwd_ws_bytes(n, C, nseg))) return 0;
+      if (op[POOL_NORM_BWD_MASK_P1] > 0)
+        return fc_maxpool8_mask_norm_act_bwd(P<const float>(c, op[POOL_NORM_BWD_X]), P<const float>(c, op[POOL_NORM_BWD_G_POOL]),
+                                             P1<const unsigned long long>(c, op[POOL_NORM_BWD_MASK_P1]), P<const int>(c, op[POOL_NORM_BWD_PARENT]),
+                                             P<const int>(c, op[POOL_NORM_BWD_SEG]), op[POOL_NORM_BWD_SEG] >= 0 ? 4 : 0, n, C, nseg,
+                                             P<const float>(c, op[POOL_NORM_BWD_MEAN]), P<const float>(c, op[POOL_NORM_BWD_VAR]),
+                                             P<const float>(c, op[POOL_NORM_BWD_CNT]), (float)as_double(op[POOL_NORM_BWD_EPS]),
+                                             P<const float>(c, op[POOL_NORM_BWD_GAMMA]), P<const float>(c, op[POOL_NORM_BWD_BETA]),
+                                             (int)op[POOL_NORM_BWD_ACT], P<float>(c, op[POOL_NORM_BWD_GX]), P<float>(c, op[POOL_NORM_BWD_SUMS]),
+                                             c.ws[s], c.ws_bytes[s], st);
       return fc_maxpool8_norm_act_bwd(P<const float>(c, op[POOL_NORM_BWD_X]), P<const float>(c, op[POOL_NORM_BWD_G_POOL]),
                                       P<const int>(c, op[POOL_NORM_BWD_ARG]), P<const int>(c, op[POOL_NORM_BWD_PARENT]),
                                       P<const int>(c, op[POOL_NORM_BWD_SEG]), op[POOL_NORM_BWD_SEG] >= 0 ? 4 : 0, n, C, nseg,
diff --git a/fcaf3d_amd/csrc/exec_ops.h b/fcaf3d_amd/csrc/exec_ops.h
--- a/fcaf3d_amd/csrc/exec_ops.h
+++ b/fcaf3d_amd/csrc/exec_ops.h
@@ -244,6 +244,7 @@
   NORM_POOL_FWD_Y,
   NORM_POOL_FWD_AMAX_OUT_P1,
   NORM_POOL_FWD_PARENT,
+  NORM_POOL_FWD_MASK_P1,
   NORM_POOL_FWD_END
 };
 enum {
@@ -264,6 +265,7 @@
   POOL_NORM_BWD_ACT,
   POOL_NORM_BWD_GX,
   POOL_NORM_BWD_SUMS,
+  POOL_NORM_BWD_MASK_P1,
   POOL_NORM_BWD_END
 };
 enum {
diff --git a/fcaf3d_amd/csrc/norm.hip b/fcaf3d_amd/csrc/norm.hip
--- a/fcaf3d_amd/csrc/norm.hip
+++ b/fcaf3d_amd/csrc/norm.hip
@@ -38,7 +38,7 @@
   return FC_OK;
 }
 
-template <bool POOL>
+template <int POOL>
 static int norm_bwd(int form, const float* x, const float* y, const float* gy, const float* gy2, const int* parent, const int* argrow, const int* seg,
                     int seg_stride, int64_t n, int C, int nseg, const float* mean, const float* var, const float* cnt, float eps, const float* gamma,
                     const float* beta, int act, float* gx, float* gres, float* sums, const float* table, int64_t nb_part, int64_t small_elems, void* ws,
@@ -52,14 +52,25 @@
     return FC_OK;
   }
   if (r.sums == FC_NRED_PARTIAL) {
-    k_norm_bwd_partial<POOL><<<FC_GRID(r.red, stream)>>>(x, y, gy, gy2, parent, argrow, seg, seg_stride, n, C, nseg, mean, var, eps, act, gamma, beta, r.red_rpb, (float*)ws);
+    const bool from_y = act && y;
+#define FC_PARTIAL(P, Y, G2) \
+  k_norm_bwd_partial<P, Y, G2><<<FC_GRID(r.red, stream)>>>(x, y, gy, gy2, parent, argrow, seg, seg_stride, n, C, nseg, mean, var, eps, act, gamma, beta, r.red_rpb, (float*)ws)
+    if constexpr (POOL != POOL_NONE) {
+      if (from_y || gy2) return FC_EINVAL;
+      FC_PARTIAL(POOL, false, false);
+    } else if (from_y) {
+      if (gy2) FC_PARTIAL(POOL_NONE, true, true); else FC_PARTIAL(POOL_NONE, true, false);
+    } else {
+      if (gy2) FC_PARTIAL(POOL_NONE, false, true); else FC_PARTIAL(POOL_NONE, false, false);
+    }
+#undef FC_PARTIAL
     FC_CHECK_LAUNCH();
     table = (const float*)ws;
   }
   if (r.apply == FC_NBAPPLY_PROLOGUE) {
     k_bn1_bwd_apply<<<FC_GRID(r.ap, stream)>>>(x, y, gy, gy2, n, C, r.rpb, table, (int)r.np, mean, var, eps, gamma, beta, act, gx, gres, sums, r.cg, amax);
   } else {
-    k_stats_final<<<FC_GRID(r.fin, stream)>>>(table, nullptr, r.np, nseg, 2 * C, 2, sums, nullptr);
+    k_stats_final<<<FC_GRID(r.fin, stream)>>>(table, r.np, nseg, 2 * C, sums);
     FC_CHECK_LAUNCH();
     k_norm_bwd_apply<POOL><<<FC_GRID(r.ap, stream)>>>(x, y, gy, gy2, parent, argrow, seg, seg_stride, n, C, mean, var, eps, gamma, beta, sums, cnt, act, gx, gres, amax);
   }
@@ -91,10 +102,10 @@
   const RowBlocks b = row_blocks(n, MAXBLOCKS);
   float* part = (float*)ws;
   float* part_cnt = stats ? part + b.nb * nseg * 2 * C : nullptr;
-  k_stats_partial<<<(unsigned)b.nb, g.threads, g.lds_fwd, stream>>>(x, seg, seg_stride, n, C, nseg, nullptr, stats ? 2 : 0, b.rpb, part, part_cnt);
+  k_stats_partial<<<(unsigned)b.nb, g.threads, g.lds_fwd, stream>>>(x, seg, seg_stride, n, C, nseg, stats, b.rpb, part, part_cnt);
   FC_CHECK_LAUNCH();
   if (stats) k_seg_meanvar_final<<<FC_GRID(final_launch(nseg, C), stream)>>>(part, part_cnt, b.nb, nseg, C, out, var, cnt);
-  else k_stats_final<<<FC_GRID(final_launch(nseg, C), stream)>>>(part, nullptr, b.nb, nseg, C, 2, out, nullptr);
+  else k_stats_final<<<FC_GRID(final_launch(nseg, C), stream)>>>(part, b.nb, nseg, C, out);
   FC_CHECK_LAUNCH();
   return FC_OK;
 }
@@ -156,7 +167,7 @@
 int fc_bn_act_train_bwd(const float* x, const float* y, const float* gy, int64_t n, int C, const float* mean,
                         const float* var, float eps, const float* gamma, const float* beta, int act, float* gx, float* gres,
                         float* sums, void* ws, int64_t ws_bytes, hipStream_t stream) {
-  return norm_bwd<false>(FC_NFORM_SMALL, x, y, gy, nullptr, nullptr, nullptr, nullptr, 0, n, C, 1, mean, var, nullptr, eps, gamma, beta, act, gx, gres, sums,
+  return norm_bwd<POOL_NONE>(FC_NFORM_SMALL, x, y, gy, nullptr, nullptr, nullptr, nullptr, 0, n, C, 1, mean, var, nullptr, eps, gamma, beta, act, gx, gres, sums,
                          nullptr, 0, 0, ws, ws_bytes, stream, nullptr, true);
 }
 
@@ -182,7 +193,7 @@
                     const float* beta, int act, float* gx, float* gres, float* sums, void* ws, int64_t ws_bytes,
                     hipStream_t stream) {
   unsigned* ao = take_amax_out();
-  return norm_bwd<false>(FC_NFORM_SEG, x, y, gy, nullptr, nullptr, nullptr, seg, seg_stride, n, C, nseg, mean, var, cnt, eps, gamma, beta, act, gx, gres, sums,
+  return norm_bwd<POOL_NONE>(FC_NFORM_SEG, x, y, gy, nullptr, nullptr, nullptr, seg, seg_stride, n, C, nseg, mean, var, cnt, eps, gamma, beta, act, gx, gres, sums,
                          nullptr, 0, 0, ws, ws_bytes, stream, ao);
 }
 
@@ -209,7 +220,7 @@
                     float* gres, float* sums, const float* part, int64_t nb_part, int64_t small_elems, void* ws, int64_t ws_bytes,
                     hipStream_t stream) {
   unsigned* ao = take_amax_out();
-  return norm_bwd<false>(FC_NFORM_TRAIN, x, y, gy, gy2, nullptr, nullptr, nullptr, 0, n, C, 1, mean, var, cnt, eps, gamma, beta, act, gx, gres, sums, part, nb_part,
+  return norm_bwd<POOL_NONE>(FC_NFORM_TRAIN, x, y, gy, gy2, nullptr, nullptr, nullptr, 0, n, C, 1, mean, var, cnt, eps, gamma, beta, act, gx, gres, sums, part, nb_part,
                          small_elems, ws, ws_bytes, stream, ao);
 }
 
@@ -260,8 +271,20 @@
   unsigned* ao = take_amax_out();
   if (n_out < 0 || C < 4 || C % 4 || act < 0 || act > 2) return FC_EINVAL;
   if (n_out == 0) return FC_OK;
-  k_norm_act_maxpool8_fwd<<<FC_GRID(rows_launch(n_out, C), stream)>>>(x, seg, seg_stride, C, mean, var, eps, gamma, beta, act, nbr, n_out, out, argrow, y,
-                                                                     parent, ao);
+  k_norm_act_maxpool8_fwd<false><<<FC_GRID(rows_launch(n_out, C), stream)>>>(x, seg, seg_stride, C, mean, var, eps, gamma, beta, act, nbr, n_out, out, argrow,
+                                                                            y, parent, nullptr, ao);
+  FC_CHECK_LAUNCH();
+  return FC_OK;
+}
+
+int fc_norm_act_maxpool8_mask_fwd(const float* x, const int* seg, int seg_stride, int C, const float* mean, const float* var, float eps,
+                                  const float* gamma, const float* beta, int act, const int* nbr, int64_t n_out, float* out,
+                                  int* argrow, float* y, int* parent, unsigned long long* mask, hipStream_t stream) {
+  unsigned* ao = take_amax_out();
+  if (n_out < 0 || C != 64 || act < 0 || act > 2 || !parent || !mask) return FC_EINVAL;
+  if (n_out == 0) return FC_OK;
+  k_norm_act_maxpool8_fwd<true><<<FC_GRID(rows_launch(n_out, C), stream)>>>(x, seg, seg_stride, C, mean, var, eps, gamma, beta, act, nbr, n_out, out, argrow,
+                                                                           y, parent, mask, ao);
   FC_CHECK_LAUNCH();
   return FC_OK;
 }
@@ -271,8 +294,17 @@
                              const float* gamma, const float* beta, int act, float* gx, float* sums, void* ws, int64_t ws_bytes,
                              hipStream_t stream) {
   if (!parent || !argrow) return FC_EINVAL;
-  return norm_bwd<true>(FC_NFORM_SEG, x, nullptr, gout, nullptr, parent, argrow, seg, seg_stride, n_in, C, nseg, mean, var, cnt, eps, gamma, beta, act, gx, nullptr,
+  return norm_bwd<POOL_ARG>(FC_NFORM_SEG, x, nullptr, gout, nullptr, parent, argrow, seg, seg_stride, n_in, C, nseg, mean, var, cnt, eps, gamma, beta, act, gx, nullptr,
                         sums, nullptr, 0, 0, ws, ws_bytes, stream, nullptr);
+}
+
+int fc_maxpool8_mask_norm_act_bwd(const float* x, const float* gout, const unsigned long long* mask, const int* parent, const int* seg,
+                                  int seg_stride, int64_t n_in, int C, int nseg, const float* mean, const float* var, const float* cnt, float eps,
+                                  const float* gamma, const float* beta, int act, float* gx, float* sums, void* ws, int64_t ws_bytes,
+                                  hipStream_t stream) {
+  if (!parent || !mask || C != 64) return FC_EINVAL;
+  return norm_bwd<POOL_MASK>(FC_NFORM_SEG, x, nullptr, gout, nullptr, parent, reinterpret_cast<const int*>(mask), seg, seg_stride, n_in, C, nseg, mean, var, cnt,
+                             eps, gamma, beta, act, gx, nullptr, sums, nullptr, 0, 0, ws, ws_bytes, stream, nullptr);
 }
 
 int fc_inverse_rows(const int* rows, int64_t n, int64_t n_inv, int* inv, hipStream_t stream) {
diff --git a/fcaf3d_amd/csrc/norm_bn.h b/fcaf3d_amd/csrc/norm_bn.h
--- a/fcaf3d_amd/csrc/norm_bn.h
+++ b/fcaf3d_amd/csrc/norm_bn.h
@@ -12,7 +12,7 @@
 #pragma unroll
     for (int u = 0; u < 4; ++u) {
       const int64_t r = rb + (int64_t)u * nrl;
-      v[u] = r < r1 ? *reinterpret_cast<const float4*>(x + r * C + cl * 4) : sh;
+      v[u] = *reinterpret_cast<const float4*>(x + (r < r1 ? r : 0) * C + cl * 4);
     }
 #pragma unroll
     for (int u = 0; u < 4; ++u) {
diff --git a/fcaf3d_amd/csrc/norm_rows.h b/fcaf3d_amd/csrc/norm_rows.h
--- a/fcaf3d_amd/csrc/norm_rows.h
+++ b/fcaf3d_amd/csrc/norm_rows.h
@@ -38,19 +38,23 @@
   if (amax_out) amax_commit(am, amax_out);
 }
 
-template <bool POOL>
-__global__ void k_norm_bwd_partial(const float* __restrict__ x, const float* __restrict__ y, const float* __restrict__ gy,
+enum { POOL_NONE, POOL_ARG, POOL_MASK };
+__device__ __forceinline__ unsigned pool_mask_nibble(const int* __restrict__ pool_mask, int64_t r, int cl) {
+  return (reinterpret_cast<const unsigned*>(pool_mask)[2 * r + (cl >> 3)] >> ((cl & 7) * 4)) & 15u;
+}
+__device__ __forceinline__ float keep_if(float v, bool keep) { return __uint_as_float(__float_as_uint(v) & (keep ? 0xffffffffu : 0u)); }
+template <int POOL, bool FROM_Y, bool GY2>
+__global__ __launch_bounds__(256) __attribute__((amdgpu_waves_per_eu(4))) void k_norm_bwd_partial(const float* __restrict__ x, const float* __restrict__ y, const float* __restrict__ gy,
                                    const float* __restrict__ gy2, const int* __restrict__ pool_parent,
-                                   const int* __restrict__ pool_arg, const int* __restrict__ seg, int seg_stride, int64_t n, int C, int nseg,
+                                   const int* __restrict__ pool_arg, const int* __restrict__ seg, int seg_stride, int64_t n, int C_rt, int nseg,
                                    const float* __restrict__ mean, const float* __restrict__ var, float eps, int act,
                                    const float* __restrict__ gamma, const float* __restrict__ beta,
                                    int64_t rpb, float* __restrict__ part) {
+  const int C = POOL == POOL_MASK ? 64 : C_rt;
   extern __shared__ float sm[];
   __shared__ int srange[2];
   const auto [cl, rl, nrl] = lane_coord(C / 4);
-  const int64_t r0 = (int64_t)blockIdx.x * rpb;
-  int64_t r1 = r0 + rpb;
-  if (r1 > n) r1 = n;
+  const auto [r0, r1] = row_span(rpb, n);
   int s_lo, s_hi;
   seg_range(seg, seg_stride, r0, r1, &s_lo, &s_hi, srange);
   const bool chk = seg && s_lo != s_hi;
@@ -65,10 +69,17 @@
                               1.f / sqrtf(va.w + eps));
       const float4 gm = gamma ? *reinterpret_cast<const float4*>(gamma + cl * 4) : make_float4(1.f, 1.f, 1.f, 1.f);
       const float4 bt = beta ? *reinterpret_cast<const float4*>(beta + cl * 4) : make_float4(0.f, 0.f, 0.f, 0.f);
-      const bool from_y = act && y;
       for (int64_t rb = r0 + rl; rb < r1; rb += 4 * nrl) {
         float4 xv[4], gv[4], yv[4], g2[4];
         bool ok[4];
+        int po[4];
+        if (POOL) {
+#pragma unroll
+          for (int u = 0; u < 4; ++u) {
+            const int64_t r = rb + (int64_t)u * nrl;
+            po[u] = pool_parent[r < r1 ? r : r0];
+          }
+        }
 #pragma unroll
         for (int u = 0; u < 4; ++u) {
           const int64_t r = rb + (int64_t)u * nrl;
@@ -76,24 +87,31 @@
           const int64_t rc = ok[u] ? r : r0;
           if (chk) ok[u] = ok[u] && seg[rc * seg_stride] == s;
           xv[u] = *reinterpret_cast<const float4*>(x + rc * C + cl * 4);
-          if (POOL) {
-            const int64_t o = pool_parent[rc];
+          if (POOL == POOL_MASK) {
+            const int64_t o = po[u];
+            const unsigned m = pool_mask_nibble(pool_arg, rc, cl);
+            gv[u] = *reinterpret_cast<const float4*>(gy + o * C + cl * 4);
+            gv[u].x = keep_if(gv[u].x, m & 1u); gv[u].y = keep_if(gv[u].y, m & 2u);
+            gv[u].z = keep_if(gv[u].z, m & 4u); gv[u].w = keep_if(gv[u].w, m & 8u);
+          } else if (POOL == POOL_ARG) {
+            const int64_t o = po[u];
             const int4 a = *reinterpret_cast<const int4*>(pool_arg + o * C + cl * 4);
             gv[u] = *reinterpret_cast<const float4*>(gy + o * C + cl * 4);
-            gv[u].x = a.x == rc ? gv[u].x : 0.f; gv[u].y = a.y == rc ? gv[u].y : 0.f;
-            gv[u].z = a.z == rc ? gv[u].z : 0.f; gv[u].w = a.w == rc ? gv[u].w : 0.f;
+            const int ri = (int)rc;
+            gv[u].x = keep_if(gv[u].x, a.x == ri); gv[u].y = keep_if(gv[u].y, a.y == ri);
+            gv[u].z = keep_if(gv[u].z, a.z == ri); gv[u].w = keep_if(gv[u].w, a.w == ri);
           } else {
             gv[u] = *reinterpret_cast<const float4*>(gy + rc * C + cl * 4);
           }
-          if (gy2) g2[u] = *reinterpret_cast<const float4*>(gy2 + rc * C + cl * 4);
-          if (from_y) yv[u] = *reinterpret_cast<const float4*>(y + rc * C + cl * 4);
+          if (GY2) g2[u] = *reinterpret_cast<const float4*>(gy2 + rc * C + cl * 4);
+          if (FROM_Y) yv[u] = *reinterpret_cast<const float4*>(y + rc * C + cl * 4);
         }
 #pragma unroll
         for (int u = 0; u < 4; ++u) {
           if (!ok[u]) continue;
           float4 g = gv[u];
-          if (gy2) { g.x += g2[u].x; g.y += g2[u].y; g.z += g2[u].z; g.w += g2[u].w; }
-          if (from_y) {
+          if (GY2) { g.x += g2[u].x; g.y += g2[u].y; g.z += g2[u].z; g.w += g2[u].w; }
+          if (FROM_Y) {
             g.x *= act_bwd_from_y(yv[u].x, act); g.y *= act_bwd_from_y(yv[u].y, act);
             g.z *= act_bwd_from_y(yv[u].z, act); g.w *= act_bwd_from_y(yv[u].w, act);
           } else if (act) {
@@ -131,15 +149,16 @@
   }
 }
 
-template <bool POOL>
+template <int POOL>
 __global__ void k_norm_bwd_apply(const float* __restrict__ x, const float* __restrict__ y, const float* __restrict__ gy,
                                  const float* __restrict__ gy2, const int* __restrict__ pool_parent,
-                                 const int* __restrict__ pool_arg, const int* __restrict__ seg, int seg_stride, int64_t n, int C,
+                                 const int* __restrict__ pool_arg, const int* __restrict__ seg, int seg_stride, int64_t n, int C_rt,
                                  const float* __restrict__ mean, const float* __restrict__ var, float eps,
                                  const float* __restrict__ gamma, const float* __restrict__ beta,
                                  const float* __restrict__ sums ,
                                  const float* __restrict__ cnt, int act, float* __restrict__ gx, float* __restrict__ gres,
                                  unsigned* __restrict__ amax_out) {
+  const int C = POOL == POOL_MASK ? 64 : C_rt;
   int64_t t = (int64_t)blockIdx.x * blockDim.x + threadIdx.x;
   const int c4n = C / 4;
   unsigned am = 0u;
@@ -150,7 +169,12 @@
   float inv_n = 1.f / cnt[s];
   float xv[4], gv[4], muv[4], vav[4], gam[4], bet[4] = {0.f, 0.f, 0.f, 0.f}, s1[4], s2[4], yv[4], o[4], gr[4];
   *reinterpret_cast<float4*>(xv) = *reinterpret_cast<const float4*>(x + r * C + c);
-  if (POOL) {
+  if (POOL == POOL_MASK) {
+    const int64_t o = pool_parent[r];
+    const unsigned m = pool_mask_nibble(pool_arg, r, c >> 2);
+    *reinterpret_cast<float4*>(gv) = *reinterpret_cast<const float4*>(gy + o * C + c);
+    gv[0] = (m & 1u) ? gv[0] : 0.f; gv[1] = (m & 2u) ? gv[1] : 0.f; gv[2] = (m & 4u) ? gv[2] : 0.f; gv[3] = (m & 8u) ? gv[3] : 0.f;
+  } else if (POOL == POOL_ARG) {
     const int64_t o = pool_parent[r];
     const int4 a = *reinterpret_cast<const int4*>(pool_arg + o * C + c);
     *reinterpret_cast<float4*>(gv) = *reinterpret_cast<const float4*>(gy + o * C + c);
diff --git a/fcaf3d_amd/csrc/norm_stats.h b/fcaf3d_amd/csrc/norm_stats.h
--- a/fcaf3d_amd/csrc/norm_stats.h
+++ b/fcaf3d_amd/csrc/norm_stats.h
@@ -1,8 +1,7 @@
 #pragma once
 
 __global__ void k_stats_partial(const float* __restrict__ x, const int* __restrict__ seg, int seg_stride, int64_t n, int C,
-                                int nseg, const float* __restrict__ mean, int mode, int64_t rpb, float* __restrict__ part,
-                                float* __restrict__ part_cnt) {
+                                int nseg, bool sq, int64_t rpb, float* __restrict__ part, float* __restrict__ part_cnt) {
   extern __shared__ float sm[];
   __shared__ int srange[2];
   const int c4n = C / 4;
@@ -13,13 +12,11 @@
   const bool chk = seg && s_lo != s_hi;
   for (int s = 0; s < nseg; ++s) {
     float4 acc[4];
-    float4 sq = make_float4(0.f, 0.f, 0.f, 0.f);
+    float4 sqs = make_float4(0.f, 0.f, 0.f, 0.f);
     float cnt = 0.f;
 #pragma unroll
     for (int u = 0; u < 4; ++u) acc[u] = make_float4(0.f, 0.f, 0.f, 0.f);
     if (s >= s_lo && s <= s_hi) {
-      float4 mu = make_float4(0.f, 0.f, 0.f, 0.f);
-      if (mode == 1) mu = *reinterpret_cast<const float4*>(mean + (int64_t)s * C + cl * 4);
       for (int64_t rb = r0 + rl; rb < r1; rb += 4 * nrl) {
         float4 vv[4];
         bool ok[4];
@@ -35,11 +32,7 @@
         for (int u = 0; u < 4; ++u) {
           if (!ok[u]) continue;
           float4 v = vv[u];
-          if (mode == 1) {
-            v.x -= mu.x; v.y -= mu.y; v.z -= mu.z; v.w -= mu.w;
-            v.x *= v.x; v.y *= v.y; v.z *= v.z; v.w *= v.w;
-          }
-          if (mode == 2) { sq.x += v.x * v.x; sq.y += v.y * v.y; sq.z += v.z * v.z; sq.w += v.w * v.w; }
+          if (sq) { sqs.x += v.x * v.x; sqs.y += v.y * v.y; sqs.z += v.z * v.z; sqs.w += v.w * v.w; }
           acc[u].x += v.x; acc[u].y += v.y; acc[u].z += v.z; acc[u].w += v.w;
           cnt += 1.f;
         }
@@ -56,7 +49,7 @@
     if (cl == 0) smc[rl] = cnt;
     __syncthreads();
     const int64_t slot = (int64_t)blockIdx.x * nseg + s;
-    float* dst = mode == 2 ? part + slot * 2 * C : part + slot * C;
+    float* dst = sq ? part + slot * 2 * C : part + slot * C;
     if (rl == 0) {
       float4 t = make_float4(0.f, 0.f, 0.f, 0.f);
       for (int j = 0; j < nrl; ++j) {
@@ -70,9 +63,9 @@
         part_cnt[slot] = c;
       }
     }
-    if (mode == 2) {
+    if (sq) {
       __syncthreads();
-      *reinterpret_cast<float4*>(&sm[(rl * c4n + cl) * 4]) = sq;
+      *reinterpret_cast<float4*>(&sm[(rl * c4n + cl) * 4]) = sqs;
       __syncthreads();
       if (rl == 0) {
         float4 t = make_float4(0.f, 0.f, 0.f, 0.f);
@@ -122,45 +115,29 @@
   }
 }
 
-__global__ __launch_bounds__(256) void k_stats_final(const float* __restrict__ part, const float* __restrict__ part_cnt,
-                                                      int64_t nblocks, int nseg, int C, int mode, float* __restrict__ out,
-                                                      float* __restrict__ cnt_io) {
+__global__ __launch_bounds__(256) void k_stats_final(const float* __restrict__ part, int64_t nblocks, int nseg, int C, float* __restrict__ out) {
   __shared__ float red[FIN_SL][FIN_CB + 1];
-  __shared__ float redc[FIN_SL];
   const int cgroups = (C + FIN_CB - 1) / FIN_CB;
   const int s = blockIdx.x / cgroups, cg = blockIdx.x % cgroups;
   const int cl = threadIdx.x & (FIN_CB - 1), j = threadIdx.x / FIN_CB;
   const int c = cg * FIN_CB + cl;
   float a0 = 0.f, a1 = 0.f, a2 = 0.f, a3 = 0.f;
   if (c < C) {
+    const float* p = part + (int64_t)s * C + c;
+    const int64_t st = (int64_t)nseg * C;
     int64_t b = j;
     for (; b + 3 * FIN_SL < nblocks; b += 4 * FIN_SL) {
-      const float v0 = fc_ld(&part[(b * nseg + s) * C + c]), v1 = fc_ld(&part[((b + FIN_SL) * nseg + s) * C + c]);
-      const float v2 = fc_ld(&part[((b + 2 * FIN_SL) * nseg + s) * C + c]), v3 = fc_ld(&part[((b + 3 * FIN_SL) * nseg + s) * C + c]);
+      const float v0 = fc_ld(&p[b * st]), v1 = fc_ld(&p[(b + FIN_SL) * st]);
+      const float v2 = fc_ld(&p[(b + 2 * FIN_SL) * st]), v3 = fc_ld(&p[(b + 3 * FIN_SL) * st]);
       a0 += v0; a1 += v1; a2 += v2; a3 += v3;
     }
-    for (; b < nblocks; b += FIN_SL) a0 += fc_ld(&part[(b * nseg + s) * C + c]);
+    for (; b < nblocks; b += FIN_SL) a0 += fc_ld(&p[b * st]);
   }
-  float acc = (a0 + a1) + (a2 + a3);
-  red[j][cl] = acc;
-  if (mode == 0 && cl == 0) {
-    float cc = 0.f;
-    for (int64_t b = j; b < nblocks; b += FIN_SL) cc += fc_ld(&part_cnt[b * nseg + s]);
-    redc[j] = cc;
-  }
+  red[j][cl] = (a0 + a1) + (a2 + a3);
   __syncthreads();
   if (j == 0 && c < C) {
     float t = 0.f;
     for (int q = 0; q < FIN_SL; ++q) t += red[q][cl];
-    float cnt = 1.f;
-    if (mode == 0) {
-      float cc = 0.f;
-      for (int q = 0; q < FIN_SL; ++q) cc += redc[q];
-      if (c == 0) cnt_io[s] = cc;
-      cnt = cc;
-    } else if (mode == 1) {
-      cnt = cnt_io[s];
-    }
-    out[(int64_t)s * C + c] = (mode == 2) ? t : (cnt > 0.f ? t / cnt : 0.f);
+    out[(int64_t)s * C + c] = t;
   }
 }
diff --git a/fcaf3d_amd/csrc/pool_rows.h b/fcaf3d_amd/csrc/pool_rows.h
--- a/fcaf3d_amd/csrc/pool_rows.h
+++ b/fcaf3d_amd/csrc/pool_rows.h
@@ -61,11 +61,13 @@
   if (i >= 0) gin[(int64_t)i * C + (t % C)] = gout[t];
 }
 
+template <bool MASK>
 __global__ void k_norm_act_maxpool8_fwd(const float* __restrict__ x, const int* __restrict__ seg, int seg_stride, int C,
                                         const float* __restrict__ mean, const float* __restrict__ var, float eps,
                                         const float* __restrict__ gamma, const float* __restrict__ beta, int act,
                                         const int* __restrict__ nbr, int64_t n_out, float* __restrict__ out, int* __restrict__ argrow,
-                                        float* __restrict__ y, int* __restrict__ parent, unsigned* __restrict__ amax_out) {
+                                        float* __restrict__ y, int* __restrict__ parent, unsigned long long* __restrict__ mask,
+                                        unsigned* __restrict__ amax_out) {
   const int c4n = C / 4;
   int64_t t = (int64_t)blockIdx.x * blockDim.x + threadIdx.x;
   unsigned am = 0u;
@@ -114,7 +116,24 @@
   }
   float4 ob = make_float4(arg[0] < 0 ? 0.f : best[0], arg[1] < 0 ? 0.f : best[1], arg[2] < 0 ? 0.f : best[2], arg[3] < 0 ? 0.f : best[3]);
   *reinterpret_cast<float4*>(out + o * C + c) = ob;
-  *reinterpret_cast<int4*>(argrow + o * C + c) = make_int4(arg[0], arg[1], arg[2], arg[3]);
+  if (!MASK || argrow) *reinterpret_cast<int4*>(argrow + o * C + c) = make_int4(arg[0], arg[1], arg[2], arg[3]);
+  if (MASK) {
+    unsigned won = 0u;
+#pragma unroll
+    for (int k = 0; k < 8; ++k) {
+      const unsigned nib = (unsigned)(arg[0] == idx[k]) | (unsigned)(arg[1] == idx[k]) << 1 | (unsigned)(arg[2] == idx[k]) << 2 |
+                           (unsigned)(arg[3] == idx[k]) << 3;
+      won |= (idx[k] < 0 ? 0u : nib) << (4 * k);
+    }
+    const int k = (c >> 2) & 7;
+    unsigned long long word = 0ull;
+#pragma unroll
+    for (int L = 0; L < 16; ++L) word |= (unsigned long long)((__shfl(won, L, 16) >> (4 * k)) & 15u) << (4 * L);
+    int mine = -1;
+#pragma unroll
+    for (int q = 0; q < 8; ++q) mine = (c == 4 * q) ? idx[q] : mine;
+    if (mine >= 0) mask[mine] = word;
+  }
   amax_fold(am, ob.x); amax_fold(am, ob.y); amax_fold(am, ob.z); amax_fold(am, ob.w);
   }
   if (amax_out) amax_commit(am, amax_out);
diff --git a/fcaf3d_amd/executor.py b/fcaf3d_amd/executor.py
--- a/fcaf3d_amd/executor.py
+++ b/fcaf3d_amd/executor.py
@@ -264,7 +264,7 @@
         maps[mn['stem']] = cm0.kernel_map(m1, 3).desc(conv=False)
         maps[mn['pool']] = m1.kernel_map(m2, 2).desc(conv=False)
         kms = {}
-        setd('n0', cm0.n); setd('n1', m1.n); setd('n2', m2.n); setd('B', batch_size); setd('one', 1)
+        setd('n0', cm0.n); setd('n1', m1.n); setd('n1w', 2 * m1.n); setd('n2', m2.n); setd('B', batch_size); setd('one', 1)
         prev, lv = m2, []
         for li in range(1, nl + 1):
             mi = prev.strided(2)
@@ -687,12 +687,14 @@
         t_in = p.T('n1', 64) if p.keep_state else -1
         if p.keep_state:
             p.relu_outs.append((t_in, 'n1', 64))
-        t_pool, arg = p.T('n2', 64), p.T('n2', 64)
+        t_pool = p.T('n2', 64)
+        arg = p.T('n2', 64) if (p.keep_state or not tr) else -1
         p.pool_arg = (arg, 'n2', 64)
         ap = self.folded(t_pool)
         pool_parent = p.T('n1', 1) if tr else -1
+        pool_mask = p.T('n1w', 1) if tr else -1
         p.emit(F, OP_NORM_POOL_FWD, S_MAIN, x=t_stem, seg=seg1, c=64, mean=mean_in, var=var_in, eps=_f(inorm.eps), gamma=p.S(inorm.weight),
-               beta=p.S(inorm.bias), act=relu, map=p.M('pool'), out=t_pool, arg=arg, y=t_in, amax_out=ap, parent=pool_parent)
+               beta=p.S(inorm.bias), act=relu, map=p.M('pool'), out=t_pool, arg=arg, y=t_in, amax_out=ap, parent=pool_parent, mask=pool_mask)
         if tr:
             p.in_sums = p.T('B', 2 * 64, 'b')
 
@@ -702,7 +704,7 @@
                 g_stem = p.T('n1', 64, 'b')
                 p.emit(self.Bk, OP_POOL_NORM_BWD, S_MAIN, x=t_stem, g_pool=g_pool, arg=arg, parent=pool_parent, seg=seg1, n=p.D('n1'), c=64,
                        nseg=p.D('B'), mean=mean_in, var=var_in, cnt=cnt_in, eps=_f(inorm.eps), gamma=p.S(inorm.weight),
-                       beta=p.S(inorm.bias), act=relu, gx=g_stem, sums=p.in_sums)
+                       beta=p.S(inorm.bias), act=relu, gx=g_stem, sums=p.in_sums, mask=pool_mask)
                 self.wgrad(S_MAIN, OP_STEM_WGRAD, col=col, gout=g_stem, map=p.M('stem'), gw=p.G(stem.kernel))
                 self.wrote(stem.kernel)
             self.tape.append(bwd)
diff --git a/include/fcaf3d_hip.h b/include/fcaf3d_hip.h
--- a/include/fcaf3d_hip.h
+++ b/include/fcaf3d_hip.h
@@ -10,7 +10,7 @@
 extern "C" {
 #endif
 
-#define FC_ABI_VERSION 14
+#define FC_ABI_VERSION 15
 #ifndef FC_AMAX_SLOT_BYTES
 #define FC_AMAX_SLOT_BYTES 2048
 #endif
@@ -228,6 +228,14 @@
                              const float* gamma, const float* beta, int act, float* gx, float* sums, void* ws, int64_t ws_bytes,
                              hipStream_t stream);
 
+int fc_norm_act_maxpool8_mask_fwd(const float* x, const int* seg, int seg_stride, int C, const float* mean, const float* var, float eps,
+                                  const float* gamma, const float* beta, int act, const int* nbr, int64_t n_out, float* out,
+                                  int* argrow, float* y, int* parent, unsigned long long* mask, hipStream_t stream);
+int fc_maxpool8_mask_norm_act_bwd(const float* x, const float* gout, const unsigned long long* mask, const int* parent, const int* seg,
+                                  int seg_stride, int64_t n_in, int C, int nseg, const float* mean, const float* var, const float* cnt,
+                                  float eps, const float* gamma, const float* beta, int act, float* gx, float* sums, void* ws,
+                                  int64_t ws_bytes, hipStream_t stream);
+
 int fc_inverse_rows(const int* rows, int64_t n, int64_t n_inv, int* inv, hipStream_t stream);
 int fc_norm_act_add_fwd(const float* x, const int* seg, int seg_stride, int64_t n, int C, const float* mean, const float* var,
                         float eps, const float* gamma, const float* beta, const float* residual, int act, const int* add_inv,
```

Measured after the change: 521.6, median of 6. 1.01x the previous value.
